# snap-research/MMVID

Hardware: AMD Instinct MI355X
Metric: video-tokens/sec training step, 8-frame 128px text-to-video (higher is better)
Workload: dtype bf16

## Files before the change

include/mmvid_hip.h:

```cpp
#ifndef MMVID_HIP_H
#define MMVID_HIP_H
#include <stdint.h>
#ifdef __cplusplus
extern "C" {
#endif

const char* mmvid_last_error(void);
int mmvid_abi_version(void);
int mmvid_device_count(void);

int mmvid_vq_sqnorm(const float* codebook, int n, int dim, float* ee, void* stream);
int mmvid_vq_argmin_l2(const float* z, const float* codebook, const float* ee, int64_t rows, int n, int dim,
                       int64_t* idx, float* dmin, void* stream);
int mmvid_gather_rows(const float* table, int64_t table_rows, const int64_t* idx, int64_t rows, int dim,
                      float* out_f32, void* out_bf16, void* stream);

int mmvid_gemm_bf16(int a_kmajor, int b_kmajor, int M, int N, int K, const void* A, int64_t lda, const void* B,
                    int64_t ldb, int batch, int64_t strideA, int64_t strideB, int64_t strideC, int splitk,
                    float alpha, const float* bias, const float* residual, int64_t ldr, const void* dact_pre,
                    void* save_pre, int64_t ldp, int act, int accumulate, float* out_f32, void* out_bf16,
                    int64_t ldc, float* out_colsum,
                    void* stream);

int mmvid_decode_trace(void* dev_buf);
int mmvid_decode_persistent_trace(void* dev_buf);

int mmvid_gemm_bf16_dw(int64_t M, int N, int K, const void* dY, int64_t ldy, const void* X, int64_t ldx, int splitk,
                       float* workspace, float* dW, int accumulate, void* stream);
int mmvid_gemm_dw_pick_splitk(int64_t M, int N, int K);
typedef struct {
    int N, K;
    const void* dY;
    int64_t ldy, strideY;
    const void* X;
    int64_t ldx, strideX;
    float* const* dW_list;
} mmvid_dw_kind_t;
int mmvid_gemm_bf16_dw_multi(int64_t M, int nkinds, const mmvid_dw_kind_t* kinds, int groups, int accumulate, void* stream);
int mmvid_gemm_bf16_dw_grouped(int64_t M, int N, int K, const void* dY, int64_t ldy, int64_t strideY, const void* X, int64_t ldx,
                               int64_t strideX, int groups, float* const* dW_list, int accumulate, void* stream);
double mmvid_gemm_dw_multi_fill(int nkinds, const mmvid_dw_kind_t* kinds, int groups);

int mmvid_layernorm_fwd(const float* x, int64_t ldx, int64_t rows, int E, const float* w, const float* b, float eps,
                        void* y_bf16, float* y_f32, int64_t ldy, float* mean, float* rstd, void* stream);
int mmvid_layernorm_bwd(const float* dy, int64_t lddy, const float* x, int64_t ldx, const float* mean,
                        const float* rstd, const float* w, int64_t rows, int E, float* dx, int64_t lddx,
                        int add_into_dx, void* dx_bf16, float* dw, float* db, float* dx_colsum, void* stream);
int mmvid_layernorm_bwd_ws(const float* dy, int64_t lddy, const float* x, int64_t ldx, const float* mean,
                           const float* rstd, const float* w, int64_t rows, int E, float* dx, int64_t lddx,
                           int add_into_dx, void* dx_bf16, float* dw, float* db, float* dx_colsum, float* workspace,
                           int64_t workspace_floats, void* stream);
int mmvid_layernorm_bwd_ex(const void* dy, int dy_is_bf16, int64_t lddy, const float* x, int64_t ldx, const float* mean,
                           const float* rstd, const float* w, int64_t rows, int E, float* dx, int64_t lddx, int add_into_dx,
                           void* dx_bf16, float* dw, float* db, float* dx_colsum, float* workspace, int64_t workspace_floats,
                           void* stream);
typedef struct {
    const float* partial;
    float *dw, *db, *dx_colsum;
} mmvid_ln_reduce_t;
int mmvid_layernorm_bwd_partial(const void* dy, int dy_is_bf16, int64_t lddy, const float* x, int64_t ldx, const float* mean,
                                const float* rstd, const float* w, int64_t rows, int E, float* dx, int64_t lddx, int add_into_dx,
                                void* dx_bf16, int want_dw, int want_db, int want_colsum, float* workspace,
                                int64_t workspace_floats, int* blocks_out, void* stream);
int mmvid_layernorm_bwd_reduce_multi(int n, const mmvid_ln_reduce_t* items, int blocks, int E, void* stream);
int mmvid_groupnorm_swish_nhwc(const void* x, int x_is_bf16, int N, int64_t hw, int C, const float* w,
                               const float* b, float eps, int swish, float* stats_scratch, int partial_blocks,
                               void* y_bf16, float* y_f32, void* stream);

int mmvid_attention_fwd(const void* qkv, int64_t ld, int B, int L, int H, int E, float scale, int mask_mode, int r0,
                        int c0, int r1, int c1, void* out, int64_t ldo, float* lse2, void* stream);
int mmvid_attention_bwd(const void* qkv, int64_t ld, const void* O, int64_t ldo, const void* dO, int64_t lddo,
                        const float* lse2, float* delta, int B, int L, int H, int E, float scale, int mask_mode,
                        int r0, int c0, int r1, int c1, void* dqkv, int64_t ldg, void* stream);
int mmvid_attention_bwd_bias(const void* qkv, int64_t ld, const void* O, int64_t ldo, const void* dO, int64_t lddo,
                             const float* lse2, float* delta, int B, int L, int H, int E, float scale, int mask_mode, int r0,
                             int c0, int r1, int c1, void* dqkv, int64_t ldg, float* dbias, void* stream);
int mmvid_assemble_sequence(const float* const* tables, const int64_t* table_rows, int ntables, const int64_t* ids,
                            const int32_t* seg, const float* pos, int64_t B, int L, int E, float* out, void* stream);
int mmvid_assemble_sequence_bwd(float* const* grad_tables, const int64_t* table_rows, int ntables,
                                const int64_t* ids, const int32_t* seg, const float* dx, int64_t B, int L, int E,
                                float* dpos, int accumulate_dpos, void* stream);
int mmvid_cross_entropy_fwd(const float* logits, int64_t ldl, const int64_t* target, const uint8_t* select,
                            int64_t rows, int V, float* lse, float* loss_sum, void* stream);
int mmvid_cross_entropy_bwd(const float* logits, int64_t ldl, const int64_t* target, const uint8_t* select,
                            const float* lse, const float* gscale, int64_t rows, int V, void* dlogits_bf16,
                            int64_t ldd, void* stream);
int mmvid_colsum_bf16(const void* dy, int64_t ld, int64_t M, int N, float* db, void* stream);
typedef struct {
    const float* w[3];
    float* gw[3];
    int32_t dst0, rows, naxes, src0;
    int32_t d[3];
    int32_t pad;
} mmvid_pos_segment_t;
int mmvid_pos_table_fwd(const mmvid_pos_segment_t* segs, int nseg, int L, int E, float* out, void* stream);
int mmvid_pos_table_bwd(const mmvid_pos_segment_t* segs, int nseg, int E, const float* g, void* stream);
int mmvid_lincomb3(const float* a, const float* b, const float* c, float wa, float wb, float wc, float* out, void* stream);
int mmvid_scale3(const float* g, float wa, float wb, float wc, float* ga, float* gb, float* gc, void* stream);
int mmvid_rows_pack(const float* W, int64_t V, int E, const int64_t* ids, int n, int64_t* uid, float* rows, void* stream);
int mmvid_rows_merge(float* W, int64_t V, int E, const int64_t* ids, const float* rows, int n, void* stream);

int mmvid_device_faults(int64_t* counts, int reset);

int mmvid_grad_sqnorm(const float* g, int64_t n, float* out_accum, void* stream);
int mmvid_adam_step(float* p, const float* g, float* m, float* v, void* shadow_bf16, int64_t n, float lr,
                    float beta1, float beta2, float eps, float weight_decay, int step, const float* step_dev,
                    float max_norm, const float* sqnorm, float grad_scale, void* stream);
int mmvid_grad_sqnorm_det(const float* g, int64_t n, float* partials, float* out_accum, void* stream);
int mmvid_adam_step_lr(float* p, const float* g, float* m, float* v, void* shadow_bf16, int64_t n, float lr,
                       const float* lr_dev, float beta1, float beta2, float eps, float weight_decay, int step,
                       const float* step_dev, float max_norm, const float* sqnorm, float grad_scale, void* stream);
int mmvid_grad_sqnorm_rows(const float* g, int64_t n, float* partials, float* out_accum, const uint8_t* row_flags,
                           int64_t table_lo, int64_t table_rows, int rowlen, void* stream);
int mmvid_adam_step_rows(float* p, const float* g, float* m, float* v, void* shadow_bf16, int64_t n, float lr,
                         const float* lr_dev, float beta1, float beta2, float eps, float weight_decay, int step,
                         const float* step_dev, float max_norm, const float* sqnorm, float grad_scale,
                         const uint8_t* row_flags, int64_t table_lo, int64_t table_rows, int rowlen, void* stream);
int mmvid_lr_schedule(const float* step_dev, int kind, float lr_min, float lr_max, int warmup_steps, int every,
                      float* lr_out, void* stream);
int mmvid_counter_add(float* counter, float value, void* stream);
int mmvid_cast_f32_to_bf16(const float* x, void* y, int64_t n, void* stream);

int mmvid_msm_masks(uint64_t seed, const float* step_dev, int B, int T, int f, const float* strategy_prob, float bern_lo,
                    float bern_hi, float pc_prob, uint8_t* mask1, float* not_fully_masked, int32_t* strategy_out,
                    void* stream);
int mmvid_msm_masks_inject(const int32_t* decisions, const uint8_t* bernoulli, int B, int T, int f, uint8_t* mask1,
                           float* not_fully_masked, void* stream);
int mmvid_warp_params_bytes(void);
int mmvid_vid_warp(uint64_t seed, const float* step_dev, const float* x, int B, int T, int C, int H, int W,
                   const float* strategy_prob, void* params_scratch, int draw_params, float* out, void* stream);
int mmvid_vid_warp_new_frames(uint64_t seed, const float* step_dev, const float* x, int B, int T, int C, int H, int W,
                              const float* strategy_prob, void* params_scratch, int draw_params, float* new_frames,
                              void* stream);
int mmvid_vid_warp_tokens(const int64_t* target_tok, const int64_t* new_frame_tok, const void* params, int B, int T, int n,
                          int64_t* out, void* stream);
int mmvid_frames_u8_to_f32(const uint8_t* frames_u8, int N, int H, int W, float* out, void* stream);
int mmvid_frames_to_u8(const float* img, int64_t N, int H, int W, uint8_t* out, void* stream);
int mmvid_frames_paste_u8(const float* img, const uint8_t* real, const uint8_t* given, int64_t N, int H, int W, int h, int w,
                          uint8_t* out, void* stream);
int mmvid_vid_warp_new_frames_u8(uint64_t seed, const float* step_dev, const uint8_t* x_u8, int B, int T, int H, int W,
                                 const float* strategy_prob, void* params_scratch, int draw_params, float* new_frames,
                                 void* stream);
int mmvid_vid_warp_draw(uint64_t seed, const float* step_dev, int B, int T, const float* strategy_prob, void* params_scratch,
                        void* stream);
int mmvid_token_rows_gather(const uint16_t* table, int64_t table_rows, const int64_t* frame_index, int64_t rows, int n,
                            int64_t* out, void* stream);
int mmvid_erase_tokens_choice(uint64_t seed, const float* step_dev, int nchoice, const float* cumprob, const int32_t* modes,
                              const int32_t* boxes, int frame0_full, int B, int Tv, int f, int64_t value, int64_t* tok,
                              void* stream);
int mmvid_random_erase_tokens(uint64_t seed, const float* step_dev, int B, int Tv, int f, float p, float scale_lo,
                              float scale_hi, float ratio_lo, float ratio_hi, int erase_half, int64_t value, int64_t* tok,
                              void* stream);

int mmvid_visual_color_jitter(uint64_t seed, const float* step_dev, float* x, int B, int Tv, int C, int H, int W, float p,
                              int first_frame, float* params_out, void* stream);

typedef struct {
    const float *ln1_w, *ln1_b, *ln2_w, *ln2_b;
    const void* in_w;
    const float* in_b;
    const void* out_w;
    const float* out_b;
    const void* fc_w;
    const float* fc_b;
    const void* pj_w;
    const float* pj_b;
    float *g_ln1_w, *g_ln1_b, *g_ln2_w, *g_ln2_b, *g_in_w, *g_in_b, *g_out_w, *g_out_b, *g_fc_w, *g_fc_b, *g_pj_w,
        *g_pj_b;
} mmvid_tower_layer_t;

typedef struct {
    int B, L, E, H, F, layers;
    int mask_mode, r0, c0, r1, c1;
    float ln_eps;
} mmvid_tower_cfg_t;

int mmvid_tower_workspace(const mmvid_tower_cfg_t* cfg, int64_t* saved_bytes, int64_t* scratch_bytes);
int mmvid_tower_forward(const mmvid_tower_cfg_t* cfg, const mmvid_tower_layer_t* layers, const float* x_in,
                        float* x_out, void* saved, void* scratch, void* stream);
int mmvid_tower_backward(const mmvid_tower_cfg_t* cfg, const mmvid_tower_layer_t* layers, float* g,
                         void* saved, void* scratch, void* stream);


int mmvid_tower_prefill(const mmvid_tower_cfg_t* cfg, const mmvid_tower_layer_t* layers, const float* x_in,
                        float* x_out, void* kv_cache, int Lmax, void* scratch, void* stream);
int mmvid_tower_decode(const mmvid_tower_cfg_t* cfg, const mmvid_tower_layer_t* layers, const float* x_in, float* x_out,
                       void* kv_cache, int Lmax, const int32_t* pos_dev, int pos, void* scratch, void* stream);
int mmvid_tower_decode_fused(const mmvid_tower_cfg_t* cfg, const mmvid_tower_layer_t* layers, const float* x_in,
                             float* x_out, void* kv_cache, int Lmax, const int32_t* pos_dev, int pos, void* scratch,
                             void* stream);
int mmvid_tower_decode_fused_slice(const mmvid_tower_cfg_t* cfg, const mmvid_tower_layer_t* layers, const float* x_in,
                                   float* x_out, void* kv_cache, int Lmax, int cache_batch, int32_t* pos_dev, int pos,
                                   int advance_pos, void* scratch, void* stream);
int mmvid_tower_decode_persistent_supported(const mmvid_tower_cfg_t* cfg, int Lmax);
int64_t mmvid_tower_decode_persistent_workspace_bytes(int B);
int mmvid_tower_decode_persistent(const mmvid_tower_cfg_t* cfg, const mmvid_tower_layer_t* layers, const float* x_in, float* x_out,
                                  void* kv_cache, int Lmax, int32_t* pos_dev, int pos, int advance_pos, void* workspace, void* stream);
typedef struct {
    int64_t* tok;
    const float* table;
    int64_t table_rows;
    const float* pos_rows;
    int32_t pos_off;
    int32_t record_pos0;
    int64_t* record;
    int64_t record_ld;
    const float *lnf_w, *lnf_b;
    const void* head_w;
    const float* head_b;
    const float* E;
    int64_t e_step_stride;
    int64_t tok_offset;
    float* logits_out;
    int32_t V, e_pos0;
    float lnf_eps, temperature;
} mmvid_decode_token_t;
int mmvid_artv_token_step_persistent(const mmvid_tower_cfg_t* cfg, const mmvid_tower_layer_t* layers, const mmvid_decode_token_t* t,
                                     float* x_out, void* kv_cache, int Lmax, int32_t* pos_dev, void* workspace, void* stream);
int mmvid_gemv_rows(const float* x, int64_t ldx, int NB, int K, const float* ln_w, const float* ln_b, float eps, const void* W,
                    const float* bias, int N, int act, const float* residual, int64_t ldr, int round_in, int round_out,
                    float* out, int64_t ldo, void* stream);
int mmvid_decode_embed(const int64_t* tok, const float* table, int64_t table_rows, const float* pos_rows,
                       const int32_t* pos_dev, int pos_off, int B, int E, float* x, void* stream);
int mmvid_decode_embed_record(const int64_t* tok, const float* table, int64_t table_rows, const float* pos_rows,
                              const int32_t* pos_dev, int pos_off, int B, int E, float* x, int64_t* record, int64_t record_ld,
                              int record_pos0, void* stream);
int mmvid_kv_store(const void* qkv, int64_t ldq, int B, int L, int E, const int32_t* pos_dev, int pos0, int Lmax,
                   void* cache, void* stream);
int mmvid_attention_decode(const void* qkv, int64_t ldq, const void* cache, int B, int Lmax, int H, int E,
                           const int32_t* pos_dev, int pos0, float scale, void* out, int64_t ldo, void* stream);

int mmvid_conv2d_nhwc(int mode, const void* x, int N, int Hin, int Win, int Cin, const void* w, const float* bias,
                      int Cout, const void* residual_bf16, const float* residual_f32, int clamp01, void* out_bf16,
                      float* out_f32, float* gn_partial, void* stream);
int mmvid_conv2d_nhwc_splitk(int mode, const void* x, int N, int Hin, int Win, int Cin, const void* w, const float* bias,
                             int Cout, const void* residual_bf16, const float* residual_f32, int clamp01, void* out_bf16,
                             float* out_f32, float* gn_partial, int splitk, float* workspace, void* stream);
int mmvid_conv3x3_strip_supported(int H, int W, int Cin, int Cout);
int mmvid_conv3x3_strip_nhwc(const void* x, int N, int H, int W, int Cin, const void* w, const float* bias, int Cout,
                             const void* residual_bf16, const float* residual_f32, void* out_bf16, float* out_f32,
                             float* gn_partial64, void* stream);
int mmvid_image_to_nhwc8(const float* img, int N, int H, int W, void* out_bf16, void* stream);
int mmvid_nhwc_to_nchw_f32(const float* x, int N, int H, int W, int C, int Cuse, float* out, void* stream);
int mmvid_spatial_attention(const void* q, const void* k, const void* v, int N, int HW, int C, float scale,
                            float* scores_scratch, void* out_bf16, void* stream);
int mmvid_spatial_attention_ld(const void* q, const void* k, const void* v, int64_t ld, int N, int HW, int C, float scale,
                               float* scores_scratch, void* out_bf16, void* stream);

int mmvid_sample_race(const float* logits, int64_t ld, const float* E, const float* noise_u, float temperature,
                      float logit_div, int64_t R, int V, int64_t tok_offset, int64_t* tok, float* y, void* stream);
int mmvid_sample_race_at(const float* logits, int64_t ld, const float* E, const int32_t* step_dev, int step0, int64_t e_step_stride,
                         const float* noise_u, float temperature, float logit_div, int64_t R, int V, int64_t tok_offset, int64_t* tok,
                         float* y, void* stream);
int mmvid_mp_select_keep(const float* Y, const float* E, const uint8_t* preserve, int b, int Bm, int TS, int k,
                         uint8_t* mask1, void* stream);
int mmvid_mp_select_keep_rows(const float* Y, const float* E, const uint8_t* given, const int32_t* k_rows, int b, int Bm, int TS,
                              uint8_t* mask1, void* stream);
int mmvid_mp_build_input(const float* control_emb, const float* image_emb, int64_t table_rows, const float* tpos,
                         const int64_t* I_tok, const uint8_t* mask1, int b, int Bm, int csl, int TS, int E, int64_t mask_id,
                         float* out, void* stream);
int mmvid_mp_update(const uint8_t* mask1, const float* Ynew, const int64_t* Inew, const float* rel_logit,
                    const float* vid_logit, int b, int Bm, int TS, int t, int dynamic, float* Y, int64_t* I_tok,
                    int64_t* Imax, float* Smax, int32_t* tmax, uint8_t* active, float* S_out, int32_t* jmax_out,
                    void* stream);
int mmvid_head_bce_fwd(const float* x, int64_t ldx, const int64_t* rows, int R, int E, const float* ln_w, const float* ln_b,
                       float eps, const float* w, const float* b, const float* label, const float* row_weight,
                       const float* den_from, int nden, float den_const, float* z, float* mean, float* rstd, float* loss,
                       void* stream);
int mmvid_head_bce_bwd(const float* x, int64_t ldx, const int64_t* rows, int R, int E, const float* ln_w, const float* ln_b,
                       const float* w, const float* z, const float* mean, const float* rstd, const float* label,
                       const float* row_weight, const float* den_from, int nden, float den_const, const float* gloss,
                       float* dx, int64_t lddx, float* dw, float* db, float* dln_w, float* dln_b, void* stream);
int mmvid_bert_build_ids(const int64_t* text, const int64_t* text_neg, const int64_t* visual_tok, const int64_t* target,
                         const int64_t* target_warp, const uint8_t* mask1, int B, int Ttxt, int Nvis, int TS,
                         int64_t pad_base, int64_t mask_id, int has_rel, int has_vid, int64_t* ids, uint8_t* select_full,
                         int64_t* target_full, float* select_count, void* stream);

int mmvid_gemm_f32(int b_kmajor, int M, int N, int K, const float* A, int64_t lda, const float* B, int64_t ldb,
                   int batch, int64_t strideA, int64_t strideB, int64_t strideC, float alpha, const float* bias,
                   const float* residual, float* C, int64_t ldc, void* stream);
int mmvid_conv2d_nhwc_f32(int mode, const float* x, int N, int Hin, int Win, int Cin, const float* w,
                          const float* bias, int Cout, const float* residual, int clamp01, float* out, void* stream);
int mmvid_image_to_nhwc4_f32(const float* img, int N, int H, int W, float* out, void* stream);
int mmvid_groupnorm_swish_nhwc_f32(const float* x, int N, int64_t hw, int C, const float* w, const float* b, float eps,
                                   int swish, float* stats_scratch, float* y, void* stream);
int mmvid_spatial_attention_f32(const float* q, const float* k, const float* v, int N, int HW, int C, float scale,
                                float* scratch, float* out, void* stream);

int mmvid_conv2d_nhwc_split3(int mode, const void* x_planes, int N, int Hin, int Win, int Cin, const void* w3, const float* bias,
                             int Cout, const float* residual_f32, int clamp01, float* out_f32, float* gn_partial, int splitk,
                             float* workspace, void* stream);
int mmvid_conv3x3_strip_nhwc_split3(const void* x_planes, int N, int H, int W, int Cin, const void* w3, const float* bias,
                                    int Cout, const float* residual_f32, float* out_f32, float* gn_partial64, void* out_planes,
                                    void* stream);
int mmvid_split_f32_bf16x2(const float* x, int64_t n, void* planes_bf16, void* stream);
int mmvid_image_to_nhwc8_split(const float* img, int N, int H, int W, void* planes_bf16, void* stream);
int mmvid_groupnorm_swish_nhwc_split(const float* x, int N, int64_t hw, int C, const float* w, const float* b, float eps,
                                     int swish, float* stats_scratch, int partial_blocks, void* planes_bf16, void* stream);
int mmvid_conv3x3_strip_nhwc_f16(const void* x_f16, int N, int H, int W, int Cin, const void* w_f16, const float* bias, int Cout,
                                 const float* residual_f32, float* out_f32, float* gn_partial64, void* out_planes, void* stream);
int mmvid_groupnorm_swish_nhwc_f16out(const float* x, int N, int64_t hw, int C, const float* w, const float* b, float eps,
                                      int swish, float* stats_scratch, int partial_blocks, void* y_f16, void* stream);

enum {
    MMVID_VQOP_IMG2NHWC8 = 0,
    MMVID_VQOP_CONV = 1,
    MMVID_VQOP_GROUPNORM = 2,
    MMVID_VQOP_CAST = 3,
    MMVID_VQOP_SPATIAL_ATTN = 4,
    MMVID_VQOP_VQ_ARGMIN = 5,
    MMVID_VQOP_GATHER = 6,
    MMVID_VQOP_NHWC2NCHW = 7,
    MMVID_VQOP_EXT_CAST = 8
};
#define MMVID_VQFLAG_STRICT 16
#define MMVID_VQFLAG_SPLIT 64
#define MMVID_VQFLAG_F16 128
typedef struct {
    int32_t op, mode;
    int32_t N, H, W, C;
    int32_t Cout, flags;
    int64_t in0, in1, in2;
    int64_t out_bf16, out_f32, scratch;
    const void* w;
    const float* b;
    const void* ext_in;
    void* ext_out;
    float eps;
    int32_t pad;
} mmvid_vqgan_op_t;
int mmvid_vqgan_run(const mmvid_vqgan_op_t* ops, int nops, void* arena, void* stream);

int mmvid_probe(int which, const void* in, void* out, void* stream);

// ... 86 lines not shown
```

mmvid_amd/_lib.py:

```python
import ctypes
import os
from ctypes import POINTER, Structure, c_char_p, c_float, c_int, c_int32, c_int64, c_uint8, c_uint64, c_void_p

HERE = os.path.dirname(os.path.abspath(__file__))
LIB_PATH = os.environ.get('MMVID_LIB') or os.path.join(HERE, 'libmmvid_hip.so')

P = c_void_p
I, I64, F, U64 = c_int, c_int64, c_float, c_uint64


class TowerLayer(Structure):
    _fields_ = [(n, P) for n in (
        'ln1_w', 'ln1_b', 'ln2_w', 'ln2_b', 'in_w', 'in_b', 'out_w', 'out_b', 'fc_w', 'fc_b', 'pj_w', 'pj_b',
        'g_ln1_w', 'g_ln1_b', 'g_ln2_w', 'g_ln2_b', 'g_in_w', 'g_in_b', 'g_out_w', 'g_out_b', 'g_fc_w', 'g_fc_b',
        'g_pj_w', 'g_pj_b')]


class TowerCfg(Structure):
    _fields_ = [('B', I), ('L', I), ('E', I), ('H', I), ('F', I), ('layers', I), ('mask_mode', I), ('r0', I),
                ('c0', I), ('r1', I), ('c1', I), ('ln_eps', F)]


class DecodeToken(Structure):
    _fields_ = [('tok', c_void_p), ('table', c_void_p), ('table_rows', c_int64), ('pos_rows', c_void_p), ('pos_off', c_int32),
                ('record_pos0', c_int32), ('record', c_void_p), ('record_ld', c_int64), ('lnf_w', c_void_p), ('lnf_b', c_void_p),
                ('head_w', c_void_p), ('head_b', c_void_p), ('E', c_void_p), ('e_step_stride', c_int64), ('tok_offset', c_int64),
                ('logits_out', c_void_p), ('V', c_int32), ('e_pos0', c_int32), ('lnf_eps', c_float), ('temperature', c_float)]


class PostLnLayer(Structure):
    _fields_ = [(n, P) for n in ('qkv_w', 'qkv_b', 'out_w', 'out_b', 'ln1_w', 'ln1_b', 'fc_w', 'fc_b', 'pj_w', 'pj_b', 'ln2_w', 'ln2_b')]


class PostLnCfg(Structure):
    _fields_ = [('B', I), ('L', I), ('E', I), ('H', I), ('F', I), ('layers', I), ('ln_eps', F)]


class Conv3dCfg(Structure):
    _fields_ = [(n, I) for n in ('N', 'T', 'H', 'W', 'Cin', 'Cout', 'kt', 'kh', 'kw', 'st', 'sh', 'sw', 'pt0', 'pt1', 'ph0', 'ph1',
                                 'pw0', 'pw1', 'relu', 'nseg')] + [('seg_end', I * 3), ('ldo', I * 3), ('c_off', I * 3), ('out', P * 3)]


class VqganOp(Structure):
    _fields_ = [('op', c_int32), ('mode', c_int32), ('N', c_int32), ('H', c_int32), ('W', c_int32), ('C', c_int32),
                ('Cout', c_int32), ('flags', c_int32), ('in0', I64), ('in1', I64), ('in2', I64), ('out_bf16', I64),
                ('out_f32', I64), ('scratch', I64), ('w', P), ('b', P), ('ext_in', P), ('ext_out', P), ('eps', F),
                ('pad', c_int32)]


SIGNATURES = {
    'mmvid_vq_sqnorm': [P, I, I, P, P],
    'mmvid_vq_argmin_l2': [P, P, P, I64, I, I, P, P, P],
    'mmvid_gather_rows': [P, I64, P, I64, I, P, P, P],
    'mmvid_gemm_bf16': [I, I, I, I, I, P, I64, P, I64, I, I64, I64, I64, I, F, P, P, I64, P, P, I64, I, I, P, P, I64, P, P],
    'mmvid_gemm_bf16_dw': [I64, I, I, P, I64, P, I64, I, P, P, I, P],
    'mmvid_gemm_dw_pick_splitk': [I64, I, I],
    'mmvid_gemm_bf16_dw_grouped': [I64, I, I, P, I64, I64, P, I64, I64, I, P, I, P],
    'mmvid_gemm_bf16_dw_multi': [I64, I, P, I, I, P],
    'mmvid_layernorm_fwd': [P, I64, I64, I, P, P, F, P, P, I64, P, P, P],
    'mmvid_layernorm_bwd': [P, I64, P, I64, P, P, P, I64, I, P, I64, I, P, P, P, P, P],
    'mmvid_layernorm_bwd_ws': [P, I64, P, I64, P, P, P, I64, I, P, I64, I, P, P, P, P, P, I64, P],
    'mmvid_layernorm_bwd_partial': [P, I, I64, P, I64, P, P, P, I64, I, P, I64, I, P, I, I, I, P, I64, P, P],
    'mmvid_layernorm_bwd_reduce_multi': [I, P, I, I, P],
    'mmvid_layernorm_bwd_ex': [P, I, I64, P, I64, P, P, P, I64, I, P, I64, I, P, P, P, P, P, I64, P],
    'mmvid_groupnorm_swish_nhwc': [P, I, I, I64, I, P, P, F, I, P, I, P, P, P],
    'mmvid_attention_fwd': [P, I64, I, I, I, I, F, I, I, I, I, I, P, I64, P, P],
    'mmvid_attention_bwd': [P, I64, P, I64, P, I64, P, P, I, I, I, I, F, I, I, I, I, I, P, I64, P],
    'mmvid_attention_bwd_bias': [P, I64, P, I64, P, I64, P, P, I, I, I, I, F, I, I, I, I, I, P, I64, P, P],
    'mmvid_assemble_sequence': [POINTER(P), POINTER(I64), I, P, P, P, I64, I, I, P, P],
    'mmvid_assemble_sequence_bwd': [POINTER(P), POINTER(I64), I, P, P, P, I64, I, I, P, I, P],
    'mmvid_cross_entropy_fwd': [P, I64, P, P, I64, I, P, P, P],
    'mmvid_cross_entropy_bwd': [P, I64, P, P, P, P, I64, I, P, I64, P],
    'mmvid_colsum_bf16': [P, I64, I64, I, P, P],
    'mmvid_grad_sqnorm': [P, I64, P, P],
    'mmvid_adam_step': [P, P, P, P, P, I64, F, F, F, F, F, I, P, F, P, F, P],
    'mmvid_cast_f32_to_bf16': [P, P, I64, P],
    'mmvid_tower_workspace': [POINTER(TowerCfg), POINTER(I64), POINTER(I64)],
    'mmvid_tower_forward': [POINTER(TowerCfg), POINTER(TowerLayer), P, P, P, P, P],
    'mmvid_tower_backward': [POINTER(TowerCfg), POINTER(TowerLayer), P, P, P, P],
    'mmvid_tower_prefill': [POINTER(TowerCfg), POINTER(TowerLayer), P, P, P, I, P, P],
    'mmvid_tower_decode': [POINTER(TowerCfg), POINTER(TowerLayer), P, P, P, I, P, I, P, P],
    'mmvid_tower_decode_fused': [POINTER(TowerCfg), POINTER(TowerLayer), P, P, P, I, P, I, P, P],
    'mmvid_tower_decode_persistent': [POINTER(TowerCfg), POINTER(TowerLayer), P, P, P, I, P, I, I, P, P],
    'mmvid_artv_token_step_persistent': [POINTER(TowerCfg), POINTER(TowerLayer), POINTER(DecodeToken), P, P, I, P, P, P],
    'mmvid_tower_decode_fused_slice': [POINTER(TowerCfg), POINTER(TowerLayer), P, P, P, I, I, P, I, I, P, P],
    'mmvid_gemv_rows': [P, I64, I, I, P, P, F, P, P, I, I, P, I64, I, I, P, I64, P],
    'mmvid_decode_embed': [P, P, I64, P, P, I, I, I, P, P],
    'mmvid_decode_embed_record': [P, P, I64, P, P, I, I, I, P, P, I64, I, P],
    'mmvid_kv_store': [P, I64, I, I, I, P, I, I, P, P],
    'mmvid_attention_decode': [P, I64, P, I, I, I, I, P, I, F, P, I64, P],
    'mmvid_conv2d_nhwc': [I, P, I, I, I, I, P, P, I, P, P, I, P, P, P, P],
    'mmvid_conv2d_nhwc_splitk': [I, P, I, I, I, I, P, P, I, P, P, I, P, P, P, I, P, P],
    'mmvid_conv3x3_strip_supported': [I, I, I, I],
    'mmvid_conv3x3_strip_nhwc': [P, I, I, I, I, P, P, I, P, P, P, P, P, P],
    'mmvid_image_to_nhwc8': [P, I, I, I, P, P],
    'mmvid_nhwc_to_nchw_f32': [P, I, I, I, I, I, P, P],
    'mmvid_spatial_attention': [P, P, P, I, I, I, F, P, P, P],
    'mmvid_spatial_attention_ld': [P, P, P, I64, I, I, I, F, P, P, P],
    'mmvid_conv2d_nhwc_split3': [I, P, I, I, I, I, P, P, I, P, I, P, P, I, P, P],
    'mmvid_conv3x3_strip_nhwc_split3': [P, I, I, I, I, P, P, I, P, P, P, P, P],
    'mmvid_conv3x3_strip_nhwc_f16': [P, I, I, I, I, P, P, I, P, P, P, P, P],
    'mmvid_split_f32_bf16x2': [P, I64, P, P],
    'mmvid_image_to_nhwc8_split': [P, I, I, I, P, P],
    'mmvid_groupnorm_swish_nhwc_split': [P, I, I64, I, P, P, F, I, P, I, P, P],
    'mmvid_groupnorm_swish_nhwc_f16out': [P, I, I64, I, P, P, F, I, P, I, P, P],
    'mmvid_decode_trace': [P],
    'mmvid_decode_persistent_trace': [P],
    'mmvid_vqgan_run': [POINTER(VqganOp), I, P, P],
    'mmvid_sample_race': [P, I64, P, P, F, F, I64, I, I64, P, P, P],
    'mmvid_sample_race_at': [P, I64, P, P, I, I64, P, F, F, I64, I, I64, P, P, P],
    'mmvid_mp_select_keep': [P, P, P, I, I, I, I, P, P],
    'mmvid_mp_build_input': [P, P, I64, P, P, P, I, I, I, I, I, I64, P, P],
    'mmvid_mp_update': [P, P, P, P, P, I, I, I, I, I, P, P, P, P, P, P, P, P, P],
    'mmvid_head_bce_fwd': [P, I64, P, I, I, P, P, F, P, P, P, P, P, I, F, P, P, P, P, P],
    'mmvid_head_bce_bwd': [P, I64, P, I, I, P, P, P, P, P, P, P, P, P, I, F, P, P, I64, P, P, P, P, P],
    'mmvid_bert_build_ids': [P, P, P, P, P, P, I, I, I, I, I64, I64, I, I, P, P, P, P, P],
    'mmvid_grad_sqnorm_det': [P, I64, P, P, P],
    'mmvid_adam_step_lr': [P, P, P, P, P, I64, F, P, F, F, F, F, I, P, F, P, F, P],
    'mmvid_lr_schedule': [P, I, F, F, I, I, P, P],
    'mmvid_grad_sqnorm_rows': [P, I64, P, P, P, I64, I64, I, P],
    'mmvid_adam_step_rows': [P, P, P, P, P, I64, F, P, F, F, F, F, I, P, F, P, F, P, I64, I64, I, P],
    'mmvid_counter_add': [P, F, P],
    'mmvid_msm_masks': [U64, P, I, I, I, P, F, F, F, P, P, P, P],
    'mmvid_msm_masks_inject': [P, P, I, I, I, P, P, P],
    'mmvid_vid_warp': [U64, P, P, I, I, I, I, I, P, P, I, P, P],
    'mmvid_vid_warp_new_frames': [U64, P, P, I, I, I, I, I, P, P, I, P, P],
    'mmvid_vid_warp_tokens': [P, P, P, I, I, I, P, P],
    'mmvid_frames_u8_to_f32': [P, I, I, I, P, P],
    'mmvid_vid_warp_new_frames_u8': [U64, P, P, I, I, I, I, P, P, I, P, P],
    'mmvid_vid_warp_draw': [U64, P, I, I, P, P, P],
    'mmvid_token_rows_gather': [P, I64, P, I64, I, P, P],
    'mmvid_erase_tokens_choice': [U64, P, I, P, P, P, I, I, I, I, I64, P, P],
    'mmvid_random_erase_tokens': [U64, P, I, I, I, F, F, F, F, F, I, I64, P, P],
    'mmvid_visual_color_jitter': [U64, P, P, I, I, I, I, I, F, I, P, P],
    'mmvid_gemm_f32': [I, I, I, I, P, I64, P, I64, I, I64, I64, I64, F, P, P, P, I64, P],
    'mmvid_conv2d_nhwc_f32': [I, P, I, I, I, I, P, P, I, P, I, P, P],
    'mmvid_image_to_nhwc4_f32': [P, I, I, I, P, P],
    'mmvid_groupnorm_swish_nhwc_f32': [P, I, I64, I, P, P, F, I, P, P, P],
    'mmvid_spatial_attention_f32': [P, P, P, I, I, I, F, P, P, P],
    'mmvid_probe': [I, P, P, P],
    'mmvid_prof_begin': [I],
    'mmvid_prof_enable': [I],
    'mmvid_graph_stats': [P],
    'mmvid_set_option': [c_char_p, I],
    'mmvid_get_option': [c_char_p, POINTER(I)],
    'mmvid_colsum_bf16_det': [P, I64, I64, I, P, P, I64, P],
    'mmvid_cross_entropy_fwd_det': [P, I64, P, P, I64, I, P, P, P, I64, P],
    'mmvid_assemble_sequence_bwd_det': [POINTER(P), POINTER(I64), I, P, P, P, I64, I, I, P, I, P, I64, P],
    'mmvid_gemm_bf16_det': [I, I, I, I, I, P, I64, P, I64, I, I64, I64, I64, I, F, P, P, I64, P, P, I64, I, I, P, P, I64, P, P, I64, P],
    'mmvid_attention_bwd_bias_det': [P, I64, P, I64, P, I64, P, P, I, I, I, I, F, I, I, I, I, I, P, I64, P, P, I64, P],
    'mmvid_device_faults': [P, I],
    'mmvid_pos_table_fwd': [P, I, I, I, P, P],
    'mmvid_pos_table_bwd': [P, I, I, P, P],
    'mmvid_lincomb3': [P, P, P, F, F, F, P, P],
    'mmvid_scale3': [P, F, F, F, P, P, P, P],
    'mmvid_prof_end': [P, P, P, P, I],
    'mmvid_rows_pack': [P, I64, I, P, I, P, P, P],
    'mmvid_rows_merge': [P, I64, I, P, P, I, P],
    'mmvid_clip_patchify': [P, I, I, I, I, I, P, P],
    'mmvid_clip_image_assemble': [P, P, P, P, P, F, I, I, I, P, P],
    'mmvid_clip_text_embed': [P, I, I, P, I64, P, I, P, P, P],
    'mmvid_clip_pool_project': [P, I, I, I, P, P, P, F, P, I, I, P, P],
    'mmvid_clip_pair_scores': [P, P, I, I, I, P, P],
    'mmvid_roberta_embed': [P, P, I, I, P, I64, P, I64, P, P, P, F, I, I64, P, P, P, P],
    'mmvid_attention_fwd_keylen': [P, I64, I, I, I, I, F, P, P, I64, P, P],
    'mmvid_postln_encoder_workspace': [POINTER(PostLnCfg), POINTER(I64)],
    'mmvid_postln_encoder_forward': [POINTER(PostLnCfg), POINTER(PostLnLayer), P, P, P, P, P, P],
    'mmvid_masked_mean_pool': [P, P, I, I, I, P, P],
    'mmvid_conv3d_ndhwc': [POINTER(Conv3dCfg), P, P, P, P],
    'mmvid_maxpool3d_ndhwc': [P, I, I, I, I, I, I, I, I, I, I, I, I, I, I, I, I, I, P, I, I, P],
    'mmvid_i3d_preprocess': [P, I, I, I, I, I, P, P],
    'mmvid_i3d_fold': [P, I, I, P, P],
    'mmvid_i3d_head': [P, I, I, I, P, P, I, P, P],
    'mmvid_frames_to_u8': [P, I64, I, I, P, P],
    'mmvid_mp_select_keep_rows': [P, P, P, P, I, I, I, P, P],
    'mmvid_frames_paste_u8': [P, P, P, I64, I, I, I, I, P, P],
}
OTHER = {'mmvid_last_error': ([], c_char_p), 'mmvid_abi_version': ([], I), 'mmvid_device_count': ([], I),
         'mmvid_warp_params_bytes': ([], I), 'mmvid_gemm_dw_multi_fill': ([I, P, I], ctypes.c_double),
         'mmvid_tower_decode_persistent_supported': ([POINTER(TowerCfg), I], I),
         'mmvid_tower_decode_persistent_workspace_bytes': ([I], I64),
         'mmvid_colsum_bf16_det_workspace_bytes': ([I64, I], I64), 'mmvid_cross_entropy_fwd_det_workspace_bytes': ([I64], I64),
         'mmvid_assemble_sequence_bwd_det_workspace_bytes': ([I64, I, I, I, POINTER(I64)], I64),
         'mmvid_gemm_bf16_det_workspace_bytes': ([I, I, I, I], I64),
         'mmvid_attention_bwd_bias_det_workspace_bytes': ([I, I, I], I64)}

class DwKind(ctypes.Structure):
    _fields_ = [('N', ctypes.c_int32), ('K', ctypes.c_int32), ('dY', ctypes.c_void_p), ('ldy', ctypes.c_int64), ('strideY', ctypes.c_int64),
                ('X', ctypes.c_void_p), ('ldx', ctypes.c_int64), ('strideX', ctypes.c_int64), ('dW_list', ctypes.c_void_p)]


class LnReduce(ctypes.Structure):
    _fields_ = [('partial', ctypes.c_void_p), ('dw', ctypes.c_void_p), ('db', ctypes.c_void_p), ('dx_colsum', ctypes.c_void_p)]


class PosSegment(ctypes.Structure):
    _fields_ = [('w', ctypes.c_void_p * 3), ('gw', ctypes.c_void_p * 3), ('dst0', ctypes.c_int32), ('rows', ctypes.c_int32),
                ('naxes', ctypes.c_int32), ('src0', ctypes.c_int32), ('d', ctypes.c_int32 * 3), ('pad', ctypes.c_int32)]


ABI_VERSION = 3
_lib = None


class MMVIDError(RuntimeError):
    pass


def load():
    global _lib
    if _lib is None:
        import torch
        if not os.path.exists(LIB_PATH):
            raise MMVIDError(f'{LIB_PATH} is missing: run `python -m mmvid_amd.build` (hipcc, gfx950). '
                             'There is no CPU/PyTorch fallback for the kernels.')
        lib = ctypes.CDLL(LIB_PATH)
        ver = getattr(lib, 'mmvid_abi_version', None)
        have = ver() if ver is not None else None
        if have != ABI_VERSION:
            raise MMVIDError(f'{LIB_PATH} has ABI version {have}, this package needs {ABI_VERSION}: '
                             'rebuild with `python -m mmvid_amd.build --force`')
        missing = []

        def bind(name, args, res):
            fn = getattr(lib, name, None)
            if fn is None:
                missing.append(name)
            else:
                fn.argtypes, fn.restype = args, res

        for name, args in SIGNATURES.items():
            bind(name, args, I)
        for name, (args, res) in OTHER.items():
            bind(name, args, res)
        if missing and not os.environ.get('MMVID_LIB'):
            raise MMVIDError(f'{LIB_PATH} lacks {missing[:4]}: rebuild with `python -m mmvid_amd.build --force`')
        lib._mmvid_missing = frozenset(missing)
        _lib = lib
    return _lib


def call(name, *args):
    lib = load()
    if name in lib._mmvid_missing:
        raise MMVIDError(f'{name} is not in {LIB_PATH} (an older build loaded through MMVID_LIB)')
    rc = getattr(lib, name)(*args)
    if rc != 0:
        raise MMVIDError(f'{name} failed (rc={rc}): {lib.mmvid_last_error().decode()}')


def is_deterministic():
    if 'mmvid_get_option' in load()._mmvid_missing:
        return False
    v = c_int(0)
    call('mmvid_get_option', b'deterministic', ctypes.byref(v))
    return v.value != 0


def set_deterministic(flag):
    prev = is_deterministic()
    call('mmvid_set_option', b'deterministic', int(bool(flag)))
    return prev


class deterministic:

    def __init__(self, flag=True):
        self.flag = bool(flag)

    def __enter__(self):
        self.prev = set_deterministic(self.flag)
        return self

    def __exit__(self, *exc):
        set_deterministic(self.prev)
        return False


FAULT_NAMES = ('embedding id outside its table', 'cross-entropy target outside [0, V)', 'token-table row outside its table', 'reserved')


def device_faults(reset=True):
    arr = (ctypes.c_int64 * 4)()
    call('mmvid_device_faults', arr, int(reset))
    return list(arr)


def check_device_faults():
    counts = device_faults(reset=True)
    bad = [f'{n} x {FAULT_NAMES[i]}' for i, n in enumerate(counts) if n]
    if bad:
        raise MMVIDError('kernels met out-of-range indices: ' + '; '.join(bad))
```

mmvid_amd/clip_tower.py:

```python
import ctypes
import os
import math

import torch
from torch import nn

from . import _lib, ops
from .functional import _note_params, _with_param_zeros

TOWER_SHAPES = {
    'openai_clip_visual': (768, 12, 12),
    'openai_clip_text': (512, 12, 8),
}
MATRIX_KEYS = ('attn.in_proj_weight', 'attn.out_proj.weight', 'mlp.c_fc.weight', 'mlp.c_proj.weight')


class _Holder(nn.Module):
    """Parameter container (no forward): gives parameters their reference names."""


def _linear_params(out_f, in_f, std):
    h = _Holder()
    h.weight = nn.Parameter(torch.randn(out_f, in_f) * std)
    h.bias = nn.Parameter(torch.zeros(out_f))
    return h


def _ln_params(e):
    h = _Holder()
    h.weight = nn.Parameter(torch.ones(e))
    h.bias = nn.Parameter(torch.zeros(e))
    return h


class ResidualAttentionBlockParams(_Holder):
    def __init__(self, width, layers):
        super().__init__()
        proj_std = (width**-0.5) * ((2 * layers)**-0.5)
        attn_std = width**-0.5
        fc_std = (2 * width)**-0.5
        self.attn = _Holder()
        self.attn.in_proj_weight = nn.Parameter(torch.randn(3 * width, width) * attn_std)
        self.attn.in_proj_bias = nn.Parameter(torch.zeros(3 * width))
        self.attn.out_proj = _linear_params(width, width, proj_std)
        self.ln_1 = _ln_params(width)
        self.mlp = _Holder()
        self.mlp.c_fc = _linear_params(4 * width, width, fc_std)
        self.mlp.c_proj = _linear_params(width, 4 * width, proj_std)
        self.ln_2 = _ln_params(width)


class _TowerParams(_Holder):
    def __init__(self, width, layers):
        super().__init__()
        self.resblocks = nn.ModuleList([ResidualAttentionBlockParams(width, layers) for _ in range(layers)])


class _TowerFn(torch.autograd.Function):
    @staticmethod
    def forward(ctx, x, tower, keep, *params):
        _note_params(ctx, (x, tower, keep) + params)
        ctx.tower = tower
        y, saved = tower._run_forward(x, keep=keep)
        ctx.saved_arena = saved
        ctx.shape = x.shape
        return y

    @staticmethod
    def backward(ctx, gy):
        g = gy.contiguous().clone()
        ctx.tower._run_backward(g, ctx.saved_arena, ctx.shape)
        ctx.saved_arena = None
        return _with_param_zeros(ctx, (g.view(ctx.shape), None, None) + (None, ) * (len(ctx.needs_input_grad) - 3))


class DecodeSession:

    def __init__(self, tower, kv_cache, first_pos, graph, fused=True):
        self.tower, self.cache, self.fused = tower, kv_cache, fused
        B, dev = kv_cache.shape[1], kv_cache.device
        self.cfg = tower._cfg(B, kv_cache.shape[2])
        self.layers, self._keep = tower._layer_structs(False)
        _, self.scratch = tower._workspace(self.cfg, dev, False)
        self.x = torch.zeros(B, tower.width, device=dev, dtype=torch.float32)
        self.y = torch.zeros_like(self.x)
        self.pos = torch.tensor([first_pos], dtype=torch.int32, device=dev)
        self.host_pos = int(first_pos)
        self.graph, self.want_graph, self.calls = None, graph, 0
        self._slice_cfgs = {}
        lib = _lib.load()
        self.persistent = bool(fused is True and os.environ.get('MMVID_DECODE_PERSISTENT', '1') != '0'
                               and lib.mmvid_tower_decode_persistent_supported(ctypes.byref(self.cfg), kv_cache.shape[2]))
        self.ws = torch.zeros(lib.mmvid_tower_decode_persistent_workspace_bytes(B) // 8, dtype=torch.int64, device=dev) if self.persistent else None

    def _enqueue(self):
        B, E = self.x.shape[0], self.x.shape[-1]
        if self.persistent:
            _lib.call('mmvid_tower_decode_persistent', ctypes.byref(self.cfg), self.layers, ops._p(self.x), ops._p(self.y),
                      ops._p(self.cache), self.cache.shape[2], ops._p(self.pos), 0, 1, ops._p(self.ws), ops._stream())
            return
        Lmax = self.cache.shape[2]
        if self.fused and E <= 768:
            per = 64 if E in (512, 768) else 16
            for b0 in range(0, B, per):
                nb = min(per, B - b0)
                cfg = self.cfg if nb == B else self._slice_cfgs.setdefault(nb, self.tower._cfg(nb, Lmax))
                _lib.call('mmvid_tower_decode_fused_slice', ctypes.byref(cfg), self.layers, self.x[b0:].data_ptr(), self.y[b0:].data_ptr(),
                          self.cache[0, b0].data_ptr(), Lmax, B, ops._p(self.pos), 0, int(b0 + per >= B), ops._p(self.scratch), ops._stream())
            return
        _lib.call('mmvid_tower_decode', ctypes.byref(self.cfg), self.layers, ops._p(self.x), ops._p(self.y),
                  ops._p(self.cache), Lmax, ops._p(self.pos), 0, ops._p(self.scratch), ops._stream())
        self.pos.add_(1)

    def token_step(self, tk):
        assert self.persistent
        _lib.call('mmvid_artv_token_step_persistent', ctypes.byref(self.cfg), self.layers, ctypes.byref(tk), ops._p(self.y), ops._p(self.cache),
                  self.cache.shape[2], ops._p(self.pos), ops._p(self.ws), ops._stream())
        self.host_pos += 1

    def failed(self):
        return bool(self.persistent and int(self.ws[1]) != 0)

    def fall_back(self, pos):
        self.persistent, self.graph = False, None
        self.fell_back = getattr(self, 'fell_back', 0) + 1
        self.pos.fill_(int(pos))
        self.host_pos = int(pos)

    def check(self):
        if self.failed():
            raise _lib.MMVIDError('persistent decode step: a poll timed out (the device was shared while it ran); results are invalid. '
                                  'Set MMVID_DECODE_PERSISTENT=0 to use the five-launch step.')

    @torch.no_grad()
    def step(self, x_new, verify=False):
        self.x.copy_(x_new)
        self.calls += 1
        if self.want_graph and self.graph is None and self.calls == 2:
            g = torch.cuda.CUDAGraph()
            side = torch.cuda.Stream()
            side.wait_stream(torch.cuda.current_stream())
            with torch.cuda.stream(side):
                with torch.cuda.graph(g, stream=side):
                    self._enqueue()
            torch.cuda.current_stream().wait_stream(side)
            self.graph = g
        if self.graph is not None:
            self.graph.replay()
        else:
            self._enqueue()
        if verify and self.persistent and self.failed():
            self.fall_back(self.host_pos)
            self._enqueue()
        self.host_pos += 1
        return self.y


class OpenAICLIPTransformer(nn.Module):
    def __init__(self, seq_len=0, which_model='openai_clip_text', model_path=None, causal=True, mask_type='causal',
                 mask_kwargs=None, layers=None, width=None, heads=None):
        super().__init__()
        if not which_model.startswith('openai_clip'):
            raise NotImplementedError(which_model)
        w, l, h = TOWER_SHAPES[which_model]
        self.width, self.layers, self.heads = width or w, layers or l, heads or h
        self.debug_keep_saved = False
        assert self.width == 64 * self.heads, 'head_dim must be 64 (CLIP towers)'
        self.context_length = seq_len
        self.causal = causal
        self.transformer = _TowerParams(self.width, self.layers)
        self.mask_spec = self.build_attention_mask(seq_len, mask_type, **(mask_kwargs or {})) if causal else None
        if model_path is not None:
            self.load_clip_checkpoint(model_path, which_model)
        self._shadow = None
        self._shadow_key = None
        self._scratch = None
        self._scratch_retired = []
        self.backward_chunk_layers = int(os.environ.get('MMVID_BWD_CHUNK', 0))
        self.on_layers_done = None

    @staticmethod
    def build_attention_mask(context_length, mask_type='causal', **kwargs):
        if mask_type == 'causal':
            return 'causal'
        if mask_type == 'mask_prev':
            idx = list(kwargs['index'])
            assert len(idx) <= 2, 'the kernels carry at most two restricted rows (BERT uses [ST1],[VID])'
            return ('rows', [(int(i), int(i)) for i in idx])
        raise NotImplementedError(mask_type)

    def dense_attention_mask(self, L=None):
        L = L or self.context_length
        if self.mask_spec is None:
            return None
        if self.mask_spec == 'causal':
            return torch.full((L, L), float('-inf')).triu_(1)
        m = torch.zeros(L, L)
        for r, c in self.mask_spec[1]:
            m[r, :c] = float('-inf')
        return m

    def load_clip_checkpoint(self, path, which_model):
        sd = torch.jit.load(path, map_location='cpu').state_dict()
        prefix = 'transformer.' if which_model == 'openai_clip_text' else 'visual.transformer.'
        own = {k[len(prefix):]: v.float() for k, v in sd.items() if k.startswith(prefix + 'resblocks.')}
        self.transformer.load_state_dict(own)

    def forward(self, x, **kwargs):
        assert x.dim() == 3 and x.shape[-1] == self.width
        keep = torch.is_grad_enabled() and (x.requires_grad or self._any_trainable())
        return _TowerFn.apply(x, self, keep, *self.parameters())

    def new_kv_cache(self, B, max_len, device):
        assert self.mask_spec == 'causal', 'incremental decoding needs the causal mask'
        return torch.empty(self.layers, B, max_len, 2 * self.width, device=device, dtype=torch.bfloat16)

    @torch.no_grad()
    def prefill(self, x, kv_cache):
        x = ops._chk(x.contiguous(), torch.float32, 'tower input')
        B, L, _ = x.shape
        cfg = self._cfg(B, L)
        layers, _keep = self._layer_structs(False)
        _, scratch = self._workspace(cfg, x.device, False)
        y = torch.empty_like(x)
        _lib.call('mmvid_tower_prefill', ctypes.byref(cfg), layers, ops._p(x), ops._p(y), ops._p(kv_cache),
                  kv_cache.shape[2], ops._p(scratch), ops._stream())
        return y

    @torch.no_grad()
    def decode_step(self, x_new, kv_cache, pos, pos_dev=None):
        x_new = ops._chk(x_new.contiguous(), torch.float32, 'tower input')
        B = x_new.shape[0]
        cfg = self._cfg(B, kv_cache.shape[2])
        layers, _keep = self._layer_structs(False)
        _, scratch = self._workspace(cfg, x_new.device, False)
        y = torch.empty_like(x_new)
        _lib.call('mmvid_tower_decode', ctypes.byref(cfg), layers, ops._p(x_new), ops._p(y), ops._p(kv_cache),
                  kv_cache.shape[2], ops._p(pos_dev), int(pos), ops._p(scratch), ops._stream())
        return y

    def decode_session(self, kv_cache, first_pos, graph=True, fused=True):
        return DecodeSession(self, kv_cache, first_pos, graph, fused)

    def _any_trainable(self):
        return any(p.requires_grad for p in self.parameters())

    def _matrix_params(self):
        for blk in self.transformer.resblocks:
            yield blk.attn.in_proj_weight
            yield blk.attn.out_proj.weight
            yield blk.mlp.c_fc.weight
            yield blk.mlp.c_proj.weight

    def attach_shadow(self, views):
        self._shadow = list(views)
        self.mark_shadow_fresh()

    def mark_shadow_fresh(self):
        self._shadow_key = tuple((p._version, p.data_ptr()) for p in self._matrix_params())

    def _sync_shadow(self):
        ps = list(self._matrix_params())
        key = tuple((p._version, p.data_ptr()) for p in ps)
        if self._shadow is None or self._shadow[0].device != ps[0].device:
            self._shadow = [torch.empty(p.shape, device=p.device, dtype=torch.bfloat16) for p in ps]
            self._shadow_key = None
        if key != self._shadow_key:
            for p, s in zip(ps, self._shadow):
                ops.cast_bf16(p.detach().contiguous(), s)
            self._shadow_key = key
        return self._shadow

    def _cfg(self, B, L):
        c = _lib.TowerCfg()
        c.B, c.L, c.E, c.H, c.F, c.layers = B, L, self.width, self.heads, 4 * self.width, self.layers
        c.mask_mode, c.r0, c.c0, c.r1, c.c1 = ops._mask_args(self.mask_spec)
        c.ln_eps = 1e-5
        return c

    def _layer_structs(self, with_grads):
        sh = self._sync_shadow()
        arr = (_lib.TowerLayer * self.layers)()
        keep = []

        def ptr(t):
            keep.append(t)
            return t.data_ptr()

        def gptr(p):
            if not with_grads or not p.requires_grad:
                return None
            if p.grad is None:
                p.grad = torch.zeros_like(p)
            return p.grad.data_ptr()

        for i, blk in enumerate(self.transformer.resblocks):
            a = arr[i]
            a.ln1_w, a.ln1_b = ptr(blk.ln_1.weight), ptr(blk.ln_1.bias)
            a.ln2_w, a.ln2_b = ptr(blk.ln_2.weight), ptr(blk.ln_2.bias)
            a.in_w, a.in_b = ptr(sh[4 * i]), ptr(blk.attn.in_proj_bias)
            a.out_w, a.out_b = ptr(sh[4 * i + 1]), ptr(blk.attn.out_proj.bias)
            a.fc_w, a.fc_b = ptr(sh[4 * i + 2]), ptr(blk.mlp.c_fc.bias)
            a.pj_w, a.pj_b = ptr(sh[4 * i + 3]), ptr(blk.mlp.c_proj.bias)
            a.g_ln1_w, a.g_ln1_b = gptr(blk.ln_1.weight), gptr(blk.ln_1.bias)
            a.g_ln2_w, a.g_ln2_b = gptr(blk.ln_2.weight), gptr(blk.ln_2.bias)
            a.g_in_w, a.g_in_b = gptr(blk.attn.in_proj_weight), gptr(blk.attn.in_proj_bias)
            a.g_out_w, a.g_out_b = gptr(blk.attn.out_proj.weight), gptr(blk.attn.out_proj.bias)
            a.g_fc_w, a.g_fc_b = gptr(blk.mlp.c_fc.weight), gptr(blk.mlp.c_fc.bias)
            a.g_pj_w, a.g_pj_b = gptr(blk.mlp.c_proj.weight), gptr(blk.mlp.c_proj.bias)
        return arr, keep

    def _workspace(self, cfg, device, keep):
        sb, cb = ctypes.c_int64(), ctypes.c_int64()
        _lib.call('mmvid_tower_workspace', ctypes.byref(cfg), ctypes.byref(sb), ctypes.byref(cb))
        if self._scratch is None or self._scratch.device != torch.device(device) or self._scratch.numel() < cb.value:
            if self._scratch is not None:
                self._scratch_retired.append(self._scratch)
            self._scratch = torch.empty(cb.value, device=device, dtype=torch.uint8)
        saved = torch.empty(sb.value, device=device, dtype=torch.uint8) if keep else None
        return saved, self._scratch

    def _run_forward(self, x, keep):
        x = ops._chk(x.contiguous(), torch.float32, 'tower input')
        B, L, _ = x.shape
        cfg = self._cfg(B, L)
        layers, _keep = self._layer_structs(False)
        saved, scratch = self._workspace(cfg, x.device, keep)
        y = torch.empty_like(x)
        _lib.call('mmvid_tower_forward', ctypes.byref(cfg), layers, ops._p(x), ops._p(y), ops._p(saved), ops._p(scratch),
                  ops._stream())
        if self.debug_keep_saved:
            self._last_saved = saved
        return y, saved

    def backward_chunks(self):
        if self.on_layers_done is None:
            return [(0, self.layers)]
        if self.backward_chunk_layers <= 0:
            return self._planned_chunks()
        step = self.backward_chunk_layers
        out, hi = [], self.layers
        while hi > 0:
            lo = max(0, hi - step)
            out.append((lo, hi))
            hi = lo
        return out

    def _planned_chunks(self):
        if getattr(self, '_chunk_plan', None) is None or self._chunk_plan[0] != self.layers:
            E = self.width
            F = 4 * E
            t = sum(-(-n // 256) * -(-k // 128) for n, k in ((3 * E, E), (E, E), (F, E), (E, F)))
            waste = lambda n: (-(-n * t // 256)) - n * t / 256.0
            best, plan = None, [(0, self.layers)]
            for a in range(3, self.layers - 2):
                w = waste(a) + waste(self.layers - a) + 0.02 * abs(a - 0.6 * self.layers)
                if best is None or w < best:
                    best, plan = w, [(self.layers - a, self.layers), (0, self.layers - a)]
            self._chunk_plan = (self.layers, plan)
        return self._chunk_plan[1]

    def _run_backward(self, g, saved, shape):
        if saved is None:
            raise _lib.MMVIDError('tower backward without saved activations (forward ran under no_grad)')
        B, L, _ = shape
        cfg = self._cfg(B, L)
        layers, _keep = self._layer_structs(True)
        _, scratch = self._workspace(cfg, g.device, False)
        sb = ctypes.c_int64()
        _lib.call('mmvid_tower_workspace', ctypes.byref(cfg), ctypes.byref(sb), None)
        if sb.value != saved.numel():
            raise _lib.MMVIDError(f'tower backward: the saved arena holds {saved.numel()} bytes, the current layout needs {sb.value} '
                                  '(the library changed between forward and backward)')
        per_layer = saved.numel() // self.layers
        for lo, hi in self.backward_chunks():
            sub = self._cfg(B, L)
            sub.layers = hi - lo
            lp = ctypes.cast(ctypes.byref(layers, lo * ctypes.sizeof(_lib.TowerLayer)), ctypes.POINTER(_lib.TowerLayer))
            _lib.call('mmvid_tower_backward', ctypes.byref(sub), lp, ops._p(g),
                      ctypes.c_void_p(saved.data_ptr() + lo * per_layer), ops._p(scratch), ops._stream())
            if self.on_layers_done is not None:
                self.on_layers_done(lo)
```

mmvid_amd/csrc/norm.hip:

```cpp
#include "../../include/mmvid_hip.h"
#include "common.h"
#include <type_traits>

namespace {

constexpr int LN_MAXV = 4;

__global__ __launch_bounds__(256) void layernorm_fwd_kernel(const float* __restrict__ x, long ldx, long rows, int E,
                                                            const float* __restrict__ w,
                                                            const float* __restrict__ b, float eps,
                                                            bf16_t* __restrict__ y_bf16, float* __restrict__ y_f32,
                                                            long ldy, float* __restrict__ mean_out,
                                                            float* __restrict__ rstd_out) {
    const long half = (rows + 1) >> 1;
    const long r0 = (long)blockIdx.x * 4 + (threadIdx.x >> 6);
    if (r0 >= half) return;
    const long rr[2] = {r0, r0 + half};
    const bool live1 = rr[1] < rows;
    const int lane = threadIdx.x & 63;
    const int nv = E >> 2;
    float4 v[2][LN_MAXV];
    float s[2] = {0.f, 0.f};
#pragma unroll
    for (int k = 0; k < 2; ++k) {
        const float4* xr = reinterpret_cast<const float4*>(x + (k == 0 || live1 ? rr[k] : rr[0]) * ldx);
#pragma unroll
        for (int i = 0; i < LN_MAXV; ++i) {
            const int c = lane + 64 * i;
            v[k][i] = c < nv ? xr[c] : make_float4(0, 0, 0, 0);
        }
    }
#pragma unroll
    for (int k = 0; k < 2; ++k)
#pragma unroll
        for (int i = 0; i < LN_MAXV; ++i) s[k] += (v[k][i].x + v[k][i].y) + (v[k][i].z + v[k][i].w);
    const float mean[2] = {wave_sum_fast(s[0]) / (float)E, wave_sum_fast(s[1]) / (float)E};
    float q[2] = {0.f, 0.f};
#pragma unroll
    for (int k = 0; k < 2; ++k)
#pragma unroll
        for (int i = 0; i < LN_MAXV; ++i) {
            const int c = lane + 64 * i;
            if (c < nv) {
                const float a = v[k][i].x - mean[k], b2 = v[k][i].y - mean[k], c2 = v[k][i].z - mean[k], d = v[k][i].w - mean[k];
                q[k] += (a * a + b2 * b2) + (c2 * c2 + d * d);
            }
        }
    const float rstd[2] = {rsqrtf(wave_sum_fast(q[0]) / (float)E + eps), rsqrtf(wave_sum_fast(q[1]) / (float)E + eps)};
#pragma unroll
    for (int k = 0; k < 2; ++k) {
        if (k == 1 && !live1) break;
        const long r = rr[k];
        if (lane == 0) {
            if (mean_out) mean_out[r] = mean[k];
            if (rstd_out) rstd_out[r] = rstd[k];
        }
#pragma unroll
        for (int i = 0; i < LN_MAXV; ++i) {
            const int c = lane + 64 * i;
            if (c < nv) {
                const float4 w4 = reinterpret_cast<const float4*>(w)[c];
                const float4 b4 = reinterpret_cast<const float4*>(b)[c];
                float4 o;
                o.x = (v[k][i].x - mean[k]) * rstd[k] * w4.x + b4.x;
                o.y = (v[k][i].y - mean[k]) * rstd[k] * w4.y + b4.y;
                o.z = (v[k][i].z - mean[k]) * rstd[k] * w4.z + b4.z;
                o.w = (v[k][i].w - mean[k]) * rstd[k] * w4.w + b4.w;
                if (y_f32) reinterpret_cast<float4*>(y_f32 + r * ldy)[c] = o;
                if (y_bf16) reinterpret_cast<uint2*>(y_bf16 + r * ldy)[c] = make_uint2(pack_bf2(o.x, o.y), pack_bf2(o.z, o.w));
            }
        }
    }
}

template <typename DY>
__global__ __launch_bounds__(256) void layernorm_bwd_kernel(const DY* __restrict__ dy, long lddy,
                                                            const float* __restrict__ x, long ldx,
                                                            const float* __restrict__ mean,
                                                            const float* __restrict__ rstd,
                                                            const float* __restrict__ w, long rows, int E,
                                                            float* __restrict__ dx, long lddx, int add,
                                                            bf16_t* __restrict__ dx_bf16,
                                                            float* __restrict__ dw, float* __restrict__ db,
                                                            float* __restrict__ dx_colsum, float* __restrict__ partial) {
    __shared__ float red[2][4][LN_MAXV * 64 * 4];
    const int lane = threadIdx.x & 63, wave = threadIdx.x >> 6;
    const int nv = E >> 2;
    float4 pw[LN_MAXV], pb[LN_MAXV], pc[LN_MAXV], w4[LN_MAXV];
#pragma unroll
    for (int i = 0; i < LN_MAXV; ++i) {
        pw[i] = pb[i] = pc[i] = make_float4(0, 0, 0, 0);
        const int c = lane + 64 * i;
        w4[i] = (c < nv) ? reinterpret_cast<const float4*>(w)[c] : make_float4(0, 0, 0, 0);
    }
    for (long r = (long)blockIdx.x * 4 + wave; r < rows; r += (long)gridDim.x * 4) {
        const float mu = mean[r], rs = rstd[r];
        float4 g[LN_MAXV], xh[LN_MAXV], prev[LN_MAXV];
        float s1 = 0.f, s2 = 0.f;
#pragma unroll
        for (int i = 0; i < LN_MAXV; ++i) {
            const int c = lane + 64 * i;
            if (c < nv) {
                prev[i] = add ? reinterpret_cast<const float4*>(dx + r * lddx)[c] : make_float4(0.f, 0.f, 0.f, 0.f);
                float4 d4;
                if constexpr (sizeof(DY) == 4) {
                    d4 = reinterpret_cast<const float4*>(dy + r * lddy)[c];
                } else {
                    const uint2 u = reinterpret_cast<const uint2*>(dy + r * lddy)[c];
                    d4 = make_float4(bf_lo(u.x), bf_hi(u.x), bf_lo(u.y), bf_hi(u.y));
                }
                const float4 x4 = reinterpret_cast<const float4*>(x + r * ldx)[c];
                xh[i] = make_float4((x4.x - mu) * rs, (x4.y - mu) * rs, (x4.z - mu) * rs, (x4.w - mu) * rs);
                g[i] = make_float4(d4.x * w4[i].x, d4.y * w4[i].y, d4.z * w4[i].z, d4.w * w4[i].w);
                s1 += (g[i].x + g[i].y) + (g[i].z + g[i].w);
                s2 += (g[i].x * xh[i].x + g[i].y * xh[i].y) + (g[i].z * xh[i].z + g[i].w * xh[i].w);
                pw[i].x += d4.x * xh[i].x, pw[i].y += d4.y * xh[i].y, pw[i].z += d4.z * xh[i].z, pw[i].w += d4.w * xh[i].w;
                pb[i].x += d4.x, pb[i].y += d4.y, pb[i].z += d4.z, pb[i].w += d4.w;
            }
        }
        const float m1 = wave_sum_fast(s1) / (float)E, m2 = wave_sum_fast(s2) / (float)E;
#pragma unroll
        for (int i = 0; i < LN_MAXV; ++i) {
            const int c = lane + 64 * i;
            if (c < nv) {
                float4 o;
                o.x = rs * (g[i].x - m1 - xh[i].x * m2);
                o.y = rs * (g[i].y - m1 - xh[i].y * m2);
                o.z = rs * (g[i].z - m1 - xh[i].z * m2);
                o.w = rs * (g[i].w - m1 - xh[i].w * m2);
                float4* d = reinterpret_cast<float4*>(dx + r * lddx) + c;
                o.x += prev[i].x, o.y += prev[i].y, o.z += prev[i].z, o.w += prev[i].w;
                *d = o;
                pc[i].x += o.x, pc[i].y += o.y, pc[i].z += o.z, pc[i].w += o.w;
                if (dx_bf16)
                    reinterpret_cast<uint2*>(dx_bf16 + r * lddx)[c] = make_uint2(pack_bf2(o.x, o.y), pack_bf2(o.z, o.w));
            }
        }
    }
    if (dw || db) {
#pragma unroll
        for (int i = 0; i < LN_MAXV; ++i) {
            const int c = lane + 64 * i;
            if (c < nv) {
                reinterpret_cast<float4*>(red[0][wave])[c] = pw[i];
                reinterpret_cast<float4*>(red[1][wave])[c] = pb[i];
            }
        }
        __syncthreads();
        for (int e = threadIdx.x; e < E; e += 256) {
            const float sw = (red[0][0][e] + red[0][1][e]) + (red[0][2][e] + red[0][3][e]);
            const float sb = (red[1][0][e] + red[1][1][e]) + (red[1][2][e] + red[1][3][e]);
            if (partial) {
                partial[((long)blockIdx.x * 3 + 0) * E + e] = sw;
                partial[((long)blockIdx.x * 3 + 1) * E + e] = sb;
            } else {
                if (dw) unsafeAtomicAdd(dw + e, sw);
                if (db) unsafeAtomicAdd(db + e, sb);
            }
        }
    }
    if (dx_colsum) {
        __syncthreads();
#pragma unroll
        for (int i = 0; i < LN_MAXV; ++i) {
            const int c = lane + 64 * i;
            if (c < nv) reinterpret_cast<float4*>(red[0][wave])[c] = pc[i];
        }
        __syncthreads();
        for (int e = threadIdx.x; e < E; e += 256) {
            const float sc = (red[0][0][e] + red[0][1][e]) + (red[0][2][e] + red[0][3][e]);
            if (partial)
                partial[((long)blockIdx.x * 3 + 2) * E + e] = sc;
            else
                unsafeAtomicAdd(dx_colsum + e, sc);
        }
    }
}

template <typename DY, int NVI>
__global__ __launch_bounds__(256) void layernorm_bwd_fast_kernel(const DY* __restrict__ dy, long lddy, const float* __restrict__ x,
                                                                 long ldx, const float* __restrict__ mean,
                                                                 const float* __restrict__ rstd, const float* __restrict__ w, long rows,
                                                                 float* __restrict__ dx, long lddx, int add,
                                                                 bf16_t* __restrict__ dx_bf16, float* __restrict__ dw,
                                                                 float* __restrict__ db, float* __restrict__ dx_colsum,
                                                                 float* __restrict__ partial) {
    constexpr int E = 256 * NVI;
    __shared__ float red[2][4][E];
    typedef typename std::conditional<sizeof(DY) == 4, float4, uint2>::type dy_raw_t;
    const int lane = threadIdx.x & 63, wave = __builtin_amdgcn_readfirstlane(threadIdx.x >> 6);
    float4 pw[NVI], pb[NVI], pc[NVI], w4[NVI];
#pragma unroll
    for (int i = 0; i < NVI; ++i) {
        pw[i] = pb[i] = pc[i] = make_float4(0, 0, 0, 0);
        w4[i] = reinterpret_cast<const float4*>(w)[lane + 64 * i];
    }
    struct RowIn {
        float4 prev[NVI], x4[NVI];
        dy_raw_t d[NVI];
        float mu, rs;
    };
    const long rstep = (long)gridDim.x * 4;
    auto load_row = [&](RowIn& in, long r) {
        in.mu = mean[r], in.rs = rstd[r];
#pragma unroll
        for (int i = 0; i < NVI; ++i) {
            const int c = lane + 64 * i;
            in.prev[i] = reinterpret_cast<const float4*>(dx + r * lddx)[c];
            in.d[i] = reinterpret_cast<const dy_raw_t*>(dy + r * lddy)[c];
            in.x4[i] = reinterpret_cast<const float4*>(x + r * ldx)[c];
        }
    };
    RowIn cur, nxt;
    long r = (long)blockIdx.x * 4 + wave;
    if (r < rows) load_row(nxt, r);
    for (; r < rows; r += rstep) {
        cur = nxt;
        load_row(nxt, r + rstep < rows ? r + rstep : r);
        const float mu = cur.mu, rs = cur.rs;
        float4 g[NVI], xh[NVI];
        float s1 = 0.f, s2 = 0.f;
#pragma unroll
        for (int i = 0; i < NVI; ++i) {
            float4 d4;
            if constexpr (sizeof(DY) == 4) {
                d4 = cur.d[i];
            } else {
                const uint2 u = cur.d[i];
                d4 = make_float4(bf_lo(u.x), bf_hi(u.x), bf_lo(u.y), bf_hi(u.y));
            }
            const float4 x4 = cur.x4[i];
            xh[i] = make_float4((x4.x - mu) * rs, (x4.y - mu) * rs, (x4.z - mu) * rs, (x4.w - mu) * rs);
            g[i] = make_float4(d4.x * w4[i].x, d4.y * w4[i].y, d4.z * w4[i].z, d4.w * w4[i].w);
            s1 += (g[i].x + g[i].y) + (g[i].z + g[i].w);
            s2 += (g[i].x * xh[i].x + g[i].y * xh[i].y) + (g[i].z * xh[i].z + g[i].w * xh[i].w);
            pw[i].x += d4.x * xh[i].x, pw[i].y += d4.y * xh[i].y, pw[i].z += d4.z * xh[i].z, pw[i].w += d4.w * xh[i].w;
            pb[i].x += d4.x, pb[i].y += d4.y, pb[i].z += d4.z, pb[i].w += d4.w;
        }
        const float m1 = wave_sum_fast(s1) / (float)E, m2 = wave_sum_fast(s2) / (float)E;
#pragma unroll
        for (int i = 0; i < NVI; ++i) {
            const int c = lane + 64 * i;
            float4 o;
            o.x = rs * (g[i].x - m1 - xh[i].x * m2);
            o.y = rs * (g[i].y - m1 - xh[i].y * m2);
            o.z = rs * (g[i].z - m1 - xh[i].z * m2);
            o.w = rs * (g[i].w - m1 - xh[i].w * m2);
            if (add) o.x += cur.prev[i].x, o.y += cur.prev[i].y, o.z += cur.prev[i].z, o.w += cur.prev[i].w;
            reinterpret_cast<float4*>(dx + r * lddx)[c] = o;
            pc[i].x += o.x, pc[i].y += o.y, pc[i].z += o.z, pc[i].w += o.w;
            if (dx_bf16) reinterpret_cast<uint2*>(dx_bf16 + r * lddx)[c] = make_uint2(pack_bf2(o.x, o.y), pack_bf2(o.z, o.w));
        }
    }
    if (dw || db) {
#pragma unroll
        for (int i = 0; i < NVI; ++i) {
            reinterpret_cast<float4*>(red[0][wave])[lane + 64 * i] = pw[i];
            reinterpret_cast<float4*>(red[1][wave])[lane + 64 * i] = pb[i];
        }
        __syncthreads();
        for (int e = threadIdx.x; e < E; e += 256) {
            const float sw = (red[0][0][e] + red[0][1][e]) + (red[0][2][e] + red[0][3][e]);
            const float sb = (red[1][0][e] + red[1][1][e]) + (red[1][2][e] + red[1][3][e]);
            if (partial) {
                partial[((long)blockIdx.x * 3 + 0) * E + e] = sw;
                partial[((long)blockIdx.x * 3 + 1) * E + e] = sb;
            } else {
                if (dw) unsafeAtomicAdd(dw + e, sw);
                if (db) unsafeAtomicAdd(db + e, sb);
            }
        }
    }
    if (dx_colsum) {
        __syncthreads();
#pragma unroll
        for (int i = 0; i < NVI; ++i) reinterpret_cast<float4*>(red[0][wave])[lane + 64 * i] = pc[i];
        __syncthreads();
        for (int e = threadIdx.x; e < E; e += 256) {
            const float sc = (red[0][0][e] + red[0][1][e]) + (red[0][2][e] + red[0][3][e]);
            if (partial)
                partial[((long)blockIdx.x * 3 + 2) * E + e] = sc;
            else
                unsafeAtomicAdd(dx_colsum + e, sc);
        }
    }
}

__global__ __launch_bounds__(1024) void layernorm_bwd_reduce_kernel(const float* __restrict__ partial, int nblocks, int E,
                                                                    float* __restrict__ dw, float* __restrict__ db,
                                                                    float* __restrict__ dx_colsum) {
    __shared__ float sh[32][33];
    const int which = blockIdx.y;
    float* out = which == 0 ? dw : (which == 1 ? db : dx_colsum);
    if (!out) return;
    const int lane = threadIdx.x & 31, rg = threadIdx.x >> 5;
    const int col = blockIdx.x * 32 + lane;
    float a = 0.f;
    if (col < E) {
        const float* src = partial + (long)which * E + col;
        int b = rg;
        for (; b + 15 * 32 < nblocks; b += 16 * 32) {
            float v[16];
#pragma unroll
            for (int i = 0; i < 16; ++i) v[i] = src[(long)(b + i * 32) * 3 * E];
#pragma unroll
            for (int i = 0; i < 16; ++i) a += v[i];
        }
        for (; b < nblocks; b += 32) a += src[(long)b * 3 * E];
    }
    sh[rg][lane] = a;
    __syncthreads();
    if (rg == 0 && col < E) {
        float t = 0.f;
#pragma unroll
        for (int i = 0; i < 32; ++i) t += sh[i][lane];
        out[col] += t;
    }
}

constexpr int LN_MULTI_MAX = 32;
struct LnReduceTable {
    mmvid_ln_reduce_t item[LN_MULTI_MAX];
};
__global__ __launch_bounds__(1024) void layernorm_bwd_reduce_multi_kernel(LnReduceTable t, int nblocks, int E) {
    __shared__ float sh[32][33];
    const int which = blockIdx.y;
    const float* partial = t.item[blockIdx.z].partial;
    float* out = which == 0 ? t.item[blockIdx.z].dw : (which == 1 ? t.item[blockIdx.z].db : t.item[blockIdx.z].dx_colsum);
    if (!out) return;
    const int lane = threadIdx.x & 31, rg = threadIdx.x >> 5;
    const int col = blockIdx.x * 32 + lane;
    float a = 0.f;
    if (col < E) {
        const float* src = partial + (long)which * E + col;
        int b = rg;
        for (; b + 15 * 32 < nblocks; b += 16 * 32) {
            float v[16];
#pragma unroll
            for (int i = 0; i < 16; ++i) v[i] = src[(long)(b + i * 32) * 3 * E];
#pragma unroll
            for (int i = 0; i < 16; ++i) a += v[i];
        }
        for (; b < nblocks; b += 32) a += src[(long)b * 3 * E];
    }
    sh[rg][lane] = a;
    __syncthreads();
    if (rg == 0 && col < E) {
        float s = 0.f;
#pragma unroll
        for (int i = 0; i < 32; ++i) s += sh[i][lane];
        out[col] += s;
    }
}

template <typename T>
__device__ __forceinline__ void load8(const T* p, float (&f)[8]);
template <>
__device__ __forceinline__ void load8<bf16_t>(const bf16_t* p, float (&f)[8]) {
    const uint4 u = *reinterpret_cast<const uint4*>(p);
    f[0] = bf_lo(u.x), f[1] = bf_hi(u.x), f[2] = bf_lo(u.y), f[3] = bf_hi(u.y);
    f[4] = bf_lo(u.z), f[5] = bf_hi(u.z), f[6] = bf_lo(u.w), f[7] = bf_hi(u.w);
// ... 139 lines not shown
        float a = 0.f;
        for (int r = 0; r < pstep; ++r) a += red[which][r * CB + ch];
        sh[which][ch] = a;
    }
    __syncthreads();
    const int cpg = C / 32;
    if (threadIdx.x < CB / cpg) {
        const int grp = threadIdx.x;
        float sm = 0.f, sq = 0.f;
        for (int e = 0; e < cpg; ++e) sm += sh[0][grp * cpg + e];
        for (int e = 0; e < cpg; ++e) sq += sh[1][grp * cpg + e];
        const float mu = sm / cnt;
        float var = sq / cnt - mu * mu;
        var = var < 0.f ? 0.f : var;
        const float rstd = rsqrtf(var + eps);
        for (int e = 0; e < cpg; ++e) {
            const int ch = grp * cpg + e;
            const float a = rstd * w[c0 + ch];
            ab[ch][0] = a, ab[ch][1] = b[c0 + ch] - mu * a;
        }
    }
    __syncthreads();
    float av[8], bv[8];
#pragma unroll
    for (int e = 0; e < 8; ++e) av[e] = ab[cc * 8 + e][0], bv[e] = ab[cc * 8 + e][1];
    for (long p = prow; p < hw; p += pstep) {
        float f[8], o[8];
        load8<T>(base + p * C, f);
#pragma unroll
        for (int e = 0; e < 8; ++e) {
            float v = f[e] * av[e] + bv[e];
            if (swish) v = v * __builtin_amdgcn_rcpf(1.0f + __builtin_amdgcn_exp2f(-1.4426950408889634f * v));
            o[e] = v;
        }
        const long at = ((long)n * hw + p) * C + c0 + cc * 8;
        if (y_bf16)
            *reinterpret_cast<uint4*>(y_bf16 + at) = make_uint4(pack_bf2(o[0], o[1]), pack_bf2(o[2], o[3]), pack_bf2(o[4], o[5]), pack_bf2(o[6], o[7]));
        if (y_f32) {
            float4* d = reinterpret_cast<float4*>(y_f32 + at);
            d[0] = make_float4(o[0], o[1], o[2], o[3]);
            d[1] = make_float4(o[4], o[5], o[6], o[7]);
        }
    }
}

__global__ __launch_bounds__(256) void groupnorm_finalize_f64_kernel(const float* __restrict__ partial, int nblk, int N, int C,
                                                                     double cnt, float eps, float* __restrict__ mr) {
    const int item = blockIdx.x * 4 + (threadIdx.x >> 6);
    if (item >= N * 32) return;
    const int lane = threadIdx.x & 63;
    const int n = item >> 5, grp = item & 31;
    double sm = 0.0, sq = 0.0;
    for (int k = lane; k < nblk; k += 64) {
        const float2 v = *reinterpret_cast<const float2*>(partial + (((long)n * nblk + k) * 32 + grp) * 2);
        sm += (double)v.x, sq += (double)v.y;
    }
    for (int o = 32; o > 0; o >>= 1) sm += __shfl_xor(sm, o, 64), sq += __shfl_xor(sq, o, 64);
    const double mu = sm / cnt;
    double var = sq / cnt - mu * mu;
    var = var < 0.0 ? 0.0 : var;
    const double rstd = 1.0 / sqrt(var + (double)eps);
    const int cpg = C >> 5;
    if (lane < cpg) *reinterpret_cast<float2*>(mr + ((long)n * C + grp * cpg + lane) * 2) = make_float2((float)mu, (float)rstd);
}

template <bool F16>
__global__ __launch_bounds__(256) void groupnorm_apply_split_kernel(const float* __restrict__ x, long hw, int C,
                                                                    const float* __restrict__ mr, const float* __restrict__ w,
                                                                    const float* __restrict__ b, int swish,
                                                                    bf16_t* __restrict__ planes, long total_chunks) {
    const long t = (long)blockIdx.x * 256 + threadIdx.x;
    if (t >= total_chunks) return;
    const int cchunks = C >> 3;
    const int cc = (int)(t % cchunks);
    const long pix = t / cchunks;
    const int n = (int)(pix / hw);
    float f[8], wv[8], bv[8];
    load8<float>(x + pix * C + cc * 8, f);
    load8<float>(w + cc * 8, wv);
    load8<float>(b + cc * 8, bv);
    const float4* q = reinterpret_cast<const float4*>(mr + ((long)n * C + cc * 8) * 2);
    const float4 q0 = q[0], q1 = q[1], q2 = q[2], q3 = q[3];
    const float mu[8] = {q0.x, q0.z, q1.x, q1.z, q2.x, q2.z, q3.x, q3.z};
    const float rs[8] = {q0.y, q0.w, q1.y, q1.w, q2.y, q2.w, q3.y, q3.w};
    uint32_t h[4], l[4];
    float o[8];
#pragma unroll
    for (int e = 0; e < 8; ++e) {
        float v = ((f[e] - mu[e]) * rs[e]) * wv[e] + bv[e];
        if (swish) v = v * (1.0f / (1.0f + expf(-v)));
        o[e] = v;
    }
    if constexpr (F16) {
#pragma unroll
        for (int e = 0; e < 4; ++e) {
            typedef __attribute__((ext_vector_type(2))) _Float16 h2_t;
            const h2_t p2 = {(_Float16)o[2 * e], (_Float16)o[2 * e + 1]};
            h[e] = __builtin_bit_cast(uint32_t, p2);
        }
        *reinterpret_cast<uint4*>(planes + t * 8) = make_uint4(h[0], h[1], h[2], h[3]);
        return;
    }
#pragma unroll
    for (int e = 0; e < 4; ++e) {
        h[e] = pack_bf2(o[2 * e], o[2 * e + 1]);
        l[e] = pack_bf2(o[2 * e] - bf_lo(h[e]), o[2 * e + 1] - bf_hi(h[e]));
    }
    *reinterpret_cast<uint4*>(planes + t * 8) = make_uint4(h[0], h[1], h[2], h[3]);
    *reinterpret_cast<uint4*>(planes + (total_chunks + t) * 8) = make_uint4(l[0], l[1], l[2], l[3]);
}

}

extern "C" int mmvid_layernorm_fwd(const float* x, int64_t ldx, int64_t rows, int E, const float* w, const float* b,
                                   float eps, void* y_bf16, float* y_f32, int64_t ldy, float* mean, float* rstd,
                                   void* stream) {
    MMVID_REQUIRE(x && w && b && (y_bf16 || y_f32), "layernorm_fwd: null pointer");
    MMVID_REQUIRE(E % 4 == 0 && E <= 64 * 4 * LN_MAXV && ldx % 4 == 0 && ldy % 4 == 0,
                  "layernorm_fwd: E=%d must be a multiple of 4 and <= %d; row strides multiples of 4", E,
                  64 * 4 * LN_MAXV);
    if (rows == 0) return MMVID_OK;
    hipLaunchKernelGGL(layernorm_fwd_kernel, dim3(cdiv((rows + 1) / 2, 4)), dim3(256), 0, (hipStream_t)stream, x, (long)ldx,
                       (long)rows, E, w, b, eps, (bf16_t*)y_bf16, y_f32, (long)ldy, mean, rstd);
    MMVID_LAUNCH_CHECK("layernorm_fwd");
    return MMVID_OK;
}

extern "C" int mmvid_layernorm_bwd_ws(const float* dy, int64_t lddy, const float* x, int64_t ldx, const float* mean,
                                      const float* rstd, const float* w, int64_t rows, int E, float* dx, int64_t lddx,
                                      int add_into_dx, void* dx_bf16, float* dw, float* db, float* dx_colsum,
                                      float* workspace, int64_t workspace_floats, void* stream);
extern "C" int mmvid_layernorm_bwd_ex(const void* dy, int dy_is_bf16, int64_t lddy, const float* x, int64_t ldx, const float* mean,
                                      const float* rstd, const float* w, int64_t rows, int E, float* dx, int64_t lddx,
                                      int add_into_dx, void* dx_bf16, float* dw, float* db, float* dx_colsum,
                                      float* workspace, int64_t workspace_floats, void* stream);

extern "C" int mmvid_layernorm_bwd(const float* dy, int64_t lddy, const float* x, int64_t ldx, const float* mean,
                                   const float* rstd, const float* w, int64_t rows, int E, float* dx, int64_t lddx,
                                   int add_into_dx, void* dx_bf16, float* dw, float* db, float* dx_colsum,
                                   void* stream) {
    return mmvid_layernorm_bwd_ws(dy, lddy, x, ldx, mean, rstd, w, rows, E, dx, lddx, add_into_dx, dx_bf16, dw, db, dx_colsum,
                                  nullptr, 0, stream);
}

extern "C" int mmvid_layernorm_bwd_ws(const float* dy, int64_t lddy, const float* x, int64_t ldx, const float* mean,
                                      const float* rstd, const float* w, int64_t rows, int E, float* dx, int64_t lddx,
                                      int add_into_dx, void* dx_bf16, float* dw, float* db, float* dx_colsum,
                                      float* workspace, int64_t workspace_floats, void* stream) {
    return mmvid_layernorm_bwd_ex(dy, 0, lddy, x, ldx, mean, rstd, w, rows, E, dx, lddx, add_into_dx, dx_bf16, dw, db, dx_colsum,
                                  workspace, workspace_floats, stream);
}

static int layernorm_bwd_impl(const void* dy, int dy_is_bf16, int64_t lddy, const float* x, int64_t ldx, const float* mean,
                              const float* rstd, const float* w, int64_t rows, int E, float* dx, int64_t lddx, int add_into_dx,
                              void* dx_bf16, float* dw, float* db, float* dx_colsum, float* workspace, int64_t workspace_floats,
                              int* blocks_out, void* stream) {
    MMVID_REQUIRE(dy && x && mean && rstd && w && dx, "layernorm_bwd: null pointer");
    MMVID_REQUIRE(E % 4 == 0 && E <= 64 * 4 * LN_MAXV && lddy % 4 == 0 && ldx % 4 == 0 && lddx % 4 == 0,
                  "layernorm_bwd: bad E/strides");
    if (rows == 0) return MMVID_OK;
    int blocks = cdiv(rows, 4);
    const bool any_red = dw || db || dx_colsum;
    float* partial = nullptr;
    if (workspace && any_red) {
        int cap = (int)(workspace_floats / (3 * (int64_t)E));
        if (cap > 2048) cap = 2048;
        if (cap >= 64) {
            if (blocks > cap) blocks = cap;
            partial = workspace;
        }
    }
    MMVID_REQUIRE(partial || !any_red || !mmvid_option(MMVID_OPT_DETERMINISTIC),
                  "layernorm_bwd: deterministic mode refuses the atomic dw / db / dx_colsum sums: pass a workspace of at least 64 * 3 * E "
                  "floats (mmvid_layernorm_bwd_ws / mmvid_layernorm_bwd_ex / mmvid_layernorm_bwd_partial)");
    if (!partial) {
        if (blocks > 512) blocks = 512;
    }
    float* const a_dw = partial ? (dw ? dw : workspace) : dw;
    float* const a_db = partial ? (db ? db : workspace) : db;
    float* const a_cs = partial ? (dx_colsum ? dx_colsum : nullptr) : dx_colsum;
    if (E == 768 || E == 512) {
#define MMVID_LN_FAST(DYT, NVI)                                                                                                            \
    hipLaunchKernelGGL((layernorm_bwd_fast_kernel<DYT, NVI>), dim3(blocks), dim3(256), 0, (hipStream_t)stream, (const DYT*)dy, (long)lddy, x, \
                       (long)ldx, mean, rstd, w, (long)rows, dx, (long)lddx, add_into_dx, (bf16_t*)dx_bf16, a_dw, a_db, a_cs, partial)
        if (dy_is_bf16) {
            if (E == 768) MMVID_LN_FAST(bf16_t, 3); else MMVID_LN_FAST(bf16_t, 2);
        } else {
            if (E == 768) MMVID_LN_FAST(float, 3); else MMVID_LN_FAST(float, 2);
        }
#undef MMVID_LN_FAST
    } else if (dy_is_bf16)
        hipLaunchKernelGGL(layernorm_bwd_kernel<bf16_t>, dim3(blocks), dim3(256), 0, (hipStream_t)stream, (const bf16_t*)dy, (long)lddy, x,
                           (long)ldx, mean, rstd, w, (long)rows, E, dx, (long)lddx, add_into_dx, (bf16_t*)dx_bf16,
                           partial ? (dw ? dw : workspace) : dw, partial ? (db ? db : workspace) : db,
                           partial ? (dx_colsum ? dx_colsum : nullptr) : dx_colsum, partial);
    else
        hipLaunchKernelGGL(layernorm_bwd_kernel<float>, dim3(blocks), dim3(256), 0, (hipStream_t)stream, (const float*)dy, (long)lddy, x,
                           (long)ldx, mean, rstd, w, (long)rows, E, dx, (long)lddx, add_into_dx, (bf16_t*)dx_bf16,
                           partial ? (dw ? dw : workspace) : dw, partial ? (db ? db : workspace) : db,
                           partial ? (dx_colsum ? dx_colsum : nullptr) : dx_colsum, partial);
    if (blocks_out) {
        MMVID_REQUIRE(partial || !any_red, "layernorm_bwd_partial: needs a workspace of at least 64 * 3 * E floats");
        *blocks_out = blocks;
    } else if (partial) {
        hipLaunchKernelGGL(layernorm_bwd_reduce_kernel, dim3(cdiv(E, 32), 3), dim3(1024), 0, (hipStream_t)stream, partial, blocks, E,
                           dw, db, dx_colsum);
    }
    MMVID_LAUNCH_CHECK("layernorm_bwd");
    return MMVID_OK;
}

extern "C" int mmvid_layernorm_bwd_ex(const void* dy, int dy_is_bf16, int64_t lddy, const float* x, int64_t ldx, const float* mean,
                                      const float* rstd, const float* w, int64_t rows, int E, float* dx, int64_t lddx,
                                      int add_into_dx, void* dx_bf16, float* dw, float* db, float* dx_colsum,
                                      float* workspace, int64_t workspace_floats, void* stream) {
    return layernorm_bwd_impl(dy, dy_is_bf16, lddy, x, ldx, mean, rstd, w, rows, E, dx, lddx, add_into_dx, dx_bf16, dw, db, dx_colsum,
                              workspace, workspace_floats, nullptr, stream);
}

extern "C" int mmvid_layernorm_bwd_partial(const void* dy, int dy_is_bf16, int64_t lddy, const float* x, int64_t ldx, const float* mean,
                                           const float* rstd, const float* w, int64_t rows, int E, float* dx, int64_t lddx,
                                           int add_into_dx, void* dx_bf16, int want_dw, int want_db, int want_colsum,
                                           float* workspace, int64_t workspace_floats, int* blocks_out, void* stream) {
    MMVID_REQUIRE(workspace && blocks_out, "layernorm_bwd_partial: null workspace / blocks_out");
    return layernorm_bwd_impl(dy, dy_is_bf16, lddy, x, ldx, mean, rstd, w, rows, E, dx, lddx, add_into_dx, dx_bf16,
                              want_dw ? workspace : nullptr, want_db ? workspace : nullptr, want_colsum ? workspace : nullptr, workspace,
                              workspace_floats, blocks_out, stream);
}

extern "C" int mmvid_layernorm_bwd_reduce_multi(int n, const mmvid_ln_reduce_t* items, int blocks, int E, void* stream) {
    MMVID_REQUIRE(n >= 0 && (n == 0 || items) && blocks > 0 && E > 0, "layernorm_bwd_reduce_multi: bad arguments");
    for (int i0 = 0; i0 < n; i0 += LN_MULTI_MAX) {
        const int m = n - i0 < LN_MULTI_MAX ? n - i0 : LN_MULTI_MAX;
        LnReduceTable t;
        for (int i = 0; i < LN_MULTI_MAX; ++i) {
            if (i < m) {
                MMVID_REQUIRE(items[i0 + i].partial, "layernorm_bwd_reduce_multi: entry %d has no partial rows", i0 + i);
                t.item[i] = items[i0 + i];
            } else {
                t.item[i].partial = nullptr, t.item[i].dw = t.item[i].db = t.item[i].dx_colsum = nullptr;
            }
        }
        hipLaunchKernelGGL(layernorm_bwd_reduce_multi_kernel, dim3(cdiv(E, 32), 3, m), dim3(1024), 0, (hipStream_t)stream, t, blocks, E);
    }
    MMVID_LAUNCH_CHECK("layernorm_bwd_reduce_multi");
    return MMVID_OK;
}

extern "C" int mmvid_groupnorm_swish_nhwc(const void* x, int x_is_bf16, int N, int64_t hw, int C, const float* w,
                                          const float* b, float eps, int swish, float* stats_scratch,
                                          int partial_blocks, void* y_bf16, float* y_f32, void* stream) {
    MMVID_REQUIRE(x && w && b && stats_scratch && (y_bf16 || y_f32), "groupnorm: null pointer");
    MMVID_REQUIRE(C % 32 == 0 && C <= 512 && 256 % (C / 8) == 0, "groupnorm: C=%d unsupported", C);
    MMVID_REQUIRE(partial_blocks >= 0 && partial_blocks <= cdiv(hw, 64), "groupnorm: partial_blocks %d", partial_blocks);
    if (N == 0 || hw == 0) return MMVID_OK;
    hipStream_t s = (hipStream_t)stream;
    const int pix_per_block = 256;
    int nblk = partial_blocks;
    float* ab = stats_scratch;
    float* partial = stats_scratch + (long)N * C * 2;
    const long chunks = (long)N * hw * (C / 8);
    if (partial_blocks == 0 && hw <= pix_per_block && (C & (C - 1)) == 0) {
        if (x_is_bf16)
            hipLaunchKernelGGL(groupnorm_small_fused_kernel<bf16_t>, dim3(N, C < 64 ? 1 : C / 64), dim3(256), 0, s, (const bf16_t*)x, (long)hw, C,
                               (float)hw * (float)(C / 32), eps, w, b, swish, (bf16_t*)y_bf16, y_f32);
        else
            hipLaunchKernelGGL(groupnorm_small_fused_kernel<float>, dim3(N, C < 64 ? 1 : C / 64), dim3(256), 0, s, (const float*)x, (long)hw, C,
                               (float)hw * (float)(C / 32), eps, w, b, swish, (bf16_t*)y_bf16, y_f32);
        MMVID_LAUNCH_CHECK("groupnorm");
        return MMVID_OK;
    }
    if (partial_blocks == 0) {
        nblk = cdiv(hw, pix_per_block);
        dim3 g1(nblk, N);
        if (x_is_bf16)
            hipLaunchKernelGGL(groupnorm_stats_kernel<bf16_t>, g1, dim3(256), 0, s, (const bf16_t*)x, (long)hw, C,
                               pix_per_block, partial);
        else
            hipLaunchKernelGGL(groupnorm_stats_kernel<float>, g1, dim3(256), 0, s, (const float*)x, (long)hw, C,
                               pix_per_block, partial);
    }
    hipLaunchKernelGGL(groupnorm_finalize_kernel, dim3(cdiv((long)N * 32, 4)), dim3(256), 0, s, partial, nblk, N, C,
                       (float)hw * (float)(C / 32), eps, w, b, ab);
    if (x_is_bf16)
        hipLaunchKernelGGL(groupnorm_apply_kernel<bf16_t>, dim3(cdiv(chunks, 256)), dim3(256), 0, s,
                           (const bf16_t*)x, (long)hw, C, ab, swish, (bf16_t*)y_bf16, y_f32, chunks);
    else
        hipLaunchKernelGGL(groupnorm_apply_kernel<float>, dim3(cdiv(chunks, 256)), dim3(256), 0, s, (const float*)x,
                           (long)hw, C, ab, swish, (bf16_t*)y_bf16, y_f32, chunks);
    MMVID_LAUNCH_CHECK("groupnorm");
    return MMVID_OK;
}

static int groupnorm_split_launch(const float* x, int N, int64_t hw, int C, const float* w, const float* b, float eps, int swish,
                                  float* stats_scratch, int partial_blocks, void* planes_bf16, void* stream, bool f16);

extern "C" int mmvid_groupnorm_swish_nhwc_split(const float* x, int N, int64_t hw, int C, const float* w, const float* b, float eps,
                                                int swish, float* stats_scratch, int partial_blocks, void* planes_bf16, void* stream) {
    return groupnorm_split_launch(x, N, hw, C, w, b, eps, swish, stats_scratch, partial_blocks, planes_bf16, stream, false);
}
extern "C" int mmvid_groupnorm_swish_nhwc_f16out(const float* x, int N, int64_t hw, int C, const float* w, const float* b, float eps,
                                                 int swish, float* stats_scratch, int partial_blocks, void* y_f16, void* stream) {
    return groupnorm_split_launch(x, N, hw, C, w, b, eps, swish, stats_scratch, partial_blocks, y_f16, stream, true);
}

static int groupnorm_split_launch(const float* x, int N, int64_t hw, int C, const float* w, const float* b, float eps, int swish,
                                  float* stats_scratch, int partial_blocks, void* planes_bf16, void* stream, bool f16) {
    MMVID_REQUIRE(x && w && b && stats_scratch && planes_bf16, "groupnorm_split: null pointer");
    MMVID_REQUIRE(C % 32 == 0 && C <= 512 && 256 % (C / 8) == 0, "groupnorm_split: C=%d unsupported", C);
    MMVID_REQUIRE(partial_blocks >= 0 && partial_blocks <= cdiv(hw, 64), "groupnorm_split: partial_blocks %d", partial_blocks);
    if (N == 0 || hw == 0) return MMVID_OK;
    hipStream_t s = (hipStream_t)stream;
    const int pix_per_block = 256;
    int nblk = partial_blocks;
    float* mr = stats_scratch;
    float* partial = stats_scratch + (long)N * C * 2;
    if (partial_blocks == 0) {
        nblk = cdiv(hw, pix_per_block);
        hipLaunchKernelGGL(groupnorm_stats_kernel<float>, dim3(nblk, N), dim3(256), 0, s, x, (long)hw, C, pix_per_block, partial);
    }
    hipLaunchKernelGGL(groupnorm_finalize_f64_kernel, dim3(cdiv((long)N * 32, 4)), dim3(256), 0, s, partial, nblk, N, C,
                       (double)hw * (double)(C / 32), eps, mr);
    const long chunks = (long)N * hw * (C / 8);
    if (f16)
        hipLaunchKernelGGL(groupnorm_apply_split_kernel<true>, dim3(cdiv(chunks, 256)), dim3(256), 0, s, x, (long)hw, C, mr, w, b, swish,
                           (bf16_t*)planes_bf16, chunks);
    else
        hipLaunchKernelGGL(groupnorm_apply_split_kernel<false>, dim3(cdiv(chunks, 256)), dim3(256), 0, s, x, (long)hw, C, mr, w, b, swish,
                           (bf16_t*)planes_bf16, chunks);
    MMVID_LAUNCH_CHECK("groupnorm_split");
    return MMVID_OK;
}
```

mmvid_amd/csrc/optim.hip:

```cpp
#include "../../include/mmvid_hip.h"
#include "common.h"

namespace {

__global__ __launch_bounds__(256) void grad_sqnorm_kernel(const float* __restrict__ g, long n,
                                                          float* __restrict__ out) {
    float a = 0.f;
    const long stride = (long)gridDim.x * 256 * 4;
    for (long i = ((long)blockIdx.x * 256 + threadIdx.x) * 4; i < n; i += stride) {
        if (i + 3 < n) {
            const float4 v = *reinterpret_cast<const float4*>(g + i);
            a += (v.x * v.x + v.y * v.y) + (v.z * v.z + v.w * v.w);
        } else {
            for (long k = i; k < n; ++k) a += g[k] * g[k];
        }
    }
    a = wave_sum(a);
    __shared__ float sh[4];
    if ((threadIdx.x & 63) == 0) sh[threadIdx.x >> 6] = a;
    __syncthreads();
    if (threadIdx.x == 0) unsafeAtomicAdd(out, (sh[0] + sh[1]) + (sh[2] + sh[3]));
}

struct AdamArgs {
    float lr, beta1, beta2, eps, weight_decay, bc1, bc2_sqrt, max_norm, grad_scale;
};
struct LazyRows {
    const unsigned char* flags;
    long lo, hi;
    int rowlen;
};
__device__ __forceinline__ bool lazy_skip(const LazyRows& z, long i) {
    return z.flags && i >= z.lo && i < z.hi && z.flags[(i - z.lo) / z.rowlen] == 0;
}

__global__ __launch_bounds__(256) void adam_kernel(float* __restrict__ p, const float* __restrict__ g,
                                                   float* __restrict__ m, float* __restrict__ v,
                                                   bf16_t* __restrict__ shadow, long n, AdamArgs a,
                                                   const float* __restrict__ sqnorm,
                                                   const float* __restrict__ step_dev,
                                                   const float* __restrict__ lr_dev, LazyRows z) {
    if (lr_dev) a.lr = *lr_dev;
    if (step_dev) {
        const float t = *step_dev;
        a.bc1 = 1.0f - powf(a.beta1, t);
        a.bc2_sqrt = sqrtf(1.0f - powf(a.beta2, t));
    }
    float coef = a.grad_scale;
    if (sqnorm && a.max_norm > 0.f) {
        const float c = a.max_norm / (sqrtf(*sqnorm) * a.grad_scale + 1e-6f);
        coef *= c < 1.f ? c : 1.f;
    }
    const float step = a.lr / a.bc1;
    const long stride = (long)gridDim.x * 256 * 4;
    for (long i = ((long)blockIdx.x * 256 + threadIdx.x) * 4; i < n; i += stride) {
        if (lazy_skip(z, i)) continue;
        if (i + 3 < n) {
            float4 pp = *reinterpret_cast<float4*>(p + i);
            const float4 gg = *reinterpret_cast<const float4*>(g + i);
            float4 mm = *reinterpret_cast<float4*>(m + i), vv = *reinterpret_cast<float4*>(v + i);
            float pe[4] = {pp.x, pp.y, pp.z, pp.w}, ge[4] = {gg.x, gg.y, gg.z, gg.w};
            float me[4] = {mm.x, mm.y, mm.z, mm.w}, ve[4] = {vv.x, vv.y, vv.z, vv.w};
#pragma unroll
            for (int e = 0; e < 4; ++e) {
                float gr = ge[e] * coef + a.weight_decay * pe[e];
                me[e] = a.beta1 * me[e] + (1.f - a.beta1) * gr;
                ve[e] = a.beta2 * ve[e] + (1.f - a.beta2) * gr * gr;
                pe[e] -= step * me[e] / (sqrtf(ve[e]) / a.bc2_sqrt + a.eps);
            }
            *reinterpret_cast<float4*>(p + i) = make_float4(pe[0], pe[1], pe[2], pe[3]);
            *reinterpret_cast<float4*>(m + i) = make_float4(me[0], me[1], me[2], me[3]);
            *reinterpret_cast<float4*>(v + i) = make_float4(ve[0], ve[1], ve[2], ve[3]);
            if (shadow) *reinterpret_cast<uint2*>(shadow + i) = make_uint2(pack_bf2(pe[0], pe[1]), pack_bf2(pe[2], pe[3]));
        } else {
            for (long k = i; k < n; ++k) {
                float gr = g[k] * coef + a.weight_decay * p[k];
                float mk = a.beta1 * m[k] + (1.f - a.beta1) * gr;
                float vk = a.beta2 * v[k] + (1.f - a.beta2) * gr * gr;
                float pk = p[k] - step * mk / (sqrtf(vk) / a.bc2_sqrt + a.eps);
                p[k] = pk, m[k] = mk, v[k] = vk;
                if (shadow) shadow[k] = f2bf(pk);
            }
        }
    }
}

__global__ __launch_bounds__(256) void cast_bf16_kernel(const float* __restrict__ x, bf16_t* __restrict__ y, long n) {
    const long stride = (long)gridDim.x * 256 * 4;
    for (long i = ((long)blockIdx.x * 256 + threadIdx.x) * 4; i < n; i += stride) {
        if (i + 3 < n) {
            const float4 v = *reinterpret_cast<const float4*>(x + i);
            *reinterpret_cast<uint2*>(y + i) = make_uint2(pack_bf2(v.x, v.y), pack_bf2(v.z, v.w));
        } else {
            for (long k = i; k < n; ++k) y[k] = f2bf(x[k]);
        }
    }
}

static int grid_for(long n) {
    long b = (n + 1023) / 1024;
    if (b > 2048) b = 2048;
    if (b < 1) b = 1;
    return (int)b;
}

}

extern "C" int mmvid_grad_sqnorm(const float* g, int64_t n, float* out_accum, void* stream) {
    MMVID_REQUIRE(g && out_accum && n >= 0, "grad_sqnorm: bad arguments");
    MMVID_REQUIRE(((uintptr_t)g & 15) == 0, "grad_sqnorm: buffer must be 16-byte aligned");
    if (n == 0) return MMVID_OK;
    hipLaunchKernelGGL(grad_sqnorm_kernel, dim3(grid_for(n)), dim3(256), 0, (hipStream_t)stream, g, (long)n, out_accum);
    MMVID_LAUNCH_CHECK("grad_sqnorm");
    return MMVID_OK;
}

__global__ __launch_bounds__(256) void grad_sqnorm_partial_kernel(const float* __restrict__ g, long n, float* __restrict__ part,
                                                                  LazyRows z) {
    float a = 0.f;
    const long stride = (long)gridDim.x * 256 * 4;
    for (long i = ((long)blockIdx.x * 256 + threadIdx.x) * 4; i < n; i += stride) {
        if (lazy_skip(z, i)) continue;
        if (i + 3 < n) {
            const float4 v = *reinterpret_cast<const float4*>(g + i);
            a += (v.x * v.x + v.y * v.y) + (v.z * v.z + v.w * v.w);
        } else {
            for (long k = i; k < n; ++k) a += g[k] * g[k];
        }
    }
    a = wave_sum(a);
    __shared__ float sh[4];
    if ((threadIdx.x & 63) == 0) sh[threadIdx.x >> 6] = a;
    __syncthreads();
    if (threadIdx.x == 0) part[blockIdx.x] = (sh[0] + sh[1]) + (sh[2] + sh[3]);
}
__global__ __launch_bounds__(256) void sum_partials_kernel(const float* __restrict__ part, int nb, float* __restrict__ out) {
    __shared__ float sh[256];
    float a = 0.f;
    for (int i = threadIdx.x; i < nb; i += 256) a += part[i];
    sh[threadIdx.x] = a;
    __syncthreads();
    for (int o = 128; o > 0; o >>= 1) {
        if ((int)threadIdx.x < o) sh[threadIdx.x] += sh[threadIdx.x + o];
        __syncthreads();
    }
    if (threadIdx.x == 0) out[0] += sh[0];
}

static int make_lazy(LazyRows& z, const uint8_t* flags, int64_t lo, int64_t rows, int rowlen, int64_t n) {
    z.flags = nullptr, z.lo = z.hi = 0, z.rowlen = 1;
    if (!flags) return MMVID_OK;
    MMVID_REQUIRE(lo >= 0 && rows >= 0 && rowlen > 0 && rowlen % 4 == 0 && lo % 4 == 0 && lo + rows * rowlen <= n,
                  "lazy rows: the table [%lld, +%lld x %d) must lie inside the buffer and be 4-element aligned", (long long)lo,
                  (long long)rows, rowlen);
    z.flags = flags, z.lo = lo, z.hi = lo + rows * rowlen, z.rowlen = rowlen;
    return MMVID_OK;
}

extern "C" int mmvid_grad_sqnorm_det(const float* g, int64_t n, float* partials, float* out_accum, void* stream) {
    return mmvid_grad_sqnorm_rows(g, n, partials, out_accum, nullptr, 0, 0, 0, stream);
}

extern "C" int mmvid_grad_sqnorm_rows(const float* g, int64_t n, float* partials, float* out_accum, const uint8_t* row_flags,
                                      int64_t table_lo, int64_t table_rows, int rowlen, void* stream) {
    MMVID_REQUIRE(g && partials && out_accum && n >= 0, "grad_sqnorm_det: bad arguments");
    MMVID_REQUIRE(((uintptr_t)g & 15) == 0, "grad_sqnorm_det: buffer must be 16-byte aligned");
    if (n == 0) return MMVID_OK;
    LazyRows z;
    if (int rc = make_lazy(z, row_flags, table_lo, table_rows, rowlen, n)) return rc;
    const int nb = grid_for(n);
    hipLaunchKernelGGL(grad_sqnorm_partial_kernel, dim3(nb), dim3(256), 0, (hipStream_t)stream, g, (long)n, partials, z);
    hipLaunchKernelGGL(sum_partials_kernel, dim3(1), dim3(256), 0, (hipStream_t)stream, partials, nb, out_accum);
    MMVID_LAUNCH_CHECK("grad_sqnorm_det");
    return MMVID_OK;
}

extern "C" int mmvid_adam_step_lr(float* p, const float* g, float* m, float* v, void* shadow_bf16, int64_t n, float lr,
                                  const float* lr_dev, float beta1, float beta2, float eps, float weight_decay, int step,
                                  const float* step_dev, float max_norm, const float* sqnorm, float grad_scale, void* stream);

extern "C" int mmvid_adam_step(float* p, const float* g, float* m, float* v, void* shadow_bf16, int64_t n, float lr,
                               float beta1, float beta2, float eps, float weight_decay, int step,
                               const float* step_dev, float max_norm, const float* sqnorm, float grad_scale,
                               void* stream) {
    return mmvid_adam_step_lr(p, g, m, v, shadow_bf16, n, lr, nullptr, beta1, beta2, eps, weight_decay, step, step_dev, max_norm,
                              sqnorm, grad_scale, stream);
}

extern "C" int mmvid_adam_step_lr(float* p, const float* g, float* m, float* v, void* shadow_bf16, int64_t n, float lr,
                                  const float* lr_dev, float beta1, float beta2, float eps, float weight_decay, int step,
                                  const float* step_dev, float max_norm, const float* sqnorm, float grad_scale, void* stream) {
    return mmvid_adam_step_rows(p, g, m, v, shadow_bf16, n, lr, lr_dev, beta1, beta2, eps, weight_decay, step, step_dev, max_norm,
                                sqnorm, grad_scale, nullptr, 0, 0, 0, stream);
}

extern "C" int mmvid_adam_step_rows(float* p, const float* g, float* m, float* v, void* shadow_bf16, int64_t n, float lr,
                                    const float* lr_dev, float beta1, float beta2, float eps, float weight_decay, int step,
                                    const float* step_dev, float max_norm, const float* sqnorm, float grad_scale,
                                    const uint8_t* row_flags, int64_t table_lo, int64_t table_rows, int rowlen, void* stream) {
    MMVID_REQUIRE(p && g && m && v && n >= 0 && (step >= 1 || step_dev), "adam_step: bad arguments");
    MMVID_REQUIRE(!row_flags || weight_decay == 0.f, "adam_step: lazy rows are exact only without weight decay");
    LazyRows z;
    if (int rc = make_lazy(z, row_flags, table_lo, table_rows, rowlen, n)) return rc;
    MMVID_REQUIRE((((uintptr_t)p | (uintptr_t)g | (uintptr_t)m | (uintptr_t)v) & 15) == 0 && ((uintptr_t)shadow_bf16 & 7) == 0,
                  "adam_step: buffers must be 16-byte aligned");
    if (n == 0) return MMVID_OK;
    AdamArgs a;
    a.lr = lr, a.beta1 = beta1, a.beta2 = beta2, a.eps = eps, a.weight_decay = weight_decay;
    a.bc1 = 1.0f - powf(beta1, (float)(step >= 1 ? step : 1));
    a.bc2_sqrt = sqrtf(1.0f - powf(beta2, (float)(step >= 1 ? step : 1)));
    a.max_norm = max_norm, a.grad_scale = grad_scale;
    hipLaunchKernelGGL(adam_kernel, dim3(grid_for(n)), dim3(256), 0, (hipStream_t)stream, p, g, m, v, (bf16_t*)shadow_bf16,
                       (long)n, a, sqnorm, step_dev, lr_dev, z);
    MMVID_LAUNCH_CHECK("adam_step");
    return MMVID_OK;
}

extern "C" int mmvid_cast_f32_to_bf16(const float* x, void* y, int64_t n, void* stream) {
    MMVID_REQUIRE(x && y && n >= 0, "cast_f32_to_bf16: bad arguments");
    MMVID_REQUIRE(((uintptr_t)x & 15) == 0 && ((uintptr_t)y & 7) == 0, "cast_f32_to_bf16: alignment");
    if (n == 0) return MMVID_OK;
    hipLaunchKernelGGL(cast_bf16_kernel, dim3(grid_for(n)), dim3(256), 0, (hipStream_t)stream, x, (bf16_t*)y, (long)n);
    MMVID_LAUNCH_CHECK("cast_f32_to_bf16");
    return MMVID_OK;
}
```

mmvid_amd/csrc/tower.hip:

```cpp
#include "../../include/mmvid_hip.h"
#include "common.h"
#include <vector>

#include "graphs.h"

namespace {

inline int64_t align256(int64_t x) { return (x + 255) & ~(int64_t)255; }
constexpr int kMaxSplitK = 16;
constexpr int kLnBwdBlocks = 512;

struct Dims {
    int B, L, E, H, F, layers;
    int64_t M;
};
Dims dims_of(const mmvid_tower_cfg_t& c) {
    Dims d;
    d.B = c.B, d.L = c.L, d.E = c.E, d.H = c.H, d.F = c.F, d.layers = c.layers;
    d.M = (int64_t)c.B * c.L;
    return d;
}

struct SavedLayer {
    int64_t x_in, x_mid, mean1, rstd1, mean2, rstd2, h1, qkv, o, lse2, h2, pre, act, k_gpj, k_dpre, k_gout, k_dqkv, k_ln1, k_ln2, total;
};
SavedLayer saved_layout(const Dims& d) {
    SavedLayer s;
    int64_t off = 0;
    auto take = [&](int64_t bytes) {
        int64_t o = off;
        off += align256(bytes);
        return o;
    };
    s.x_in = take(d.M * d.E * 4);
    s.x_mid = take(d.M * d.E * 4);
    s.mean1 = take(d.M * 4), s.rstd1 = take(d.M * 4), s.mean2 = take(d.M * 4), s.rstd2 = take(d.M * 4);
    s.h1 = take(d.M * d.E * 2);
    s.qkv = take(d.M * 3 * d.E * 2);
    s.o = take(d.M * d.E * 2);
    s.lse2 = take((int64_t)d.B * d.H * d.L * 4);
    s.h2 = take(d.M * d.E * 2);
    s.pre = take(d.M * d.F * 2);
    s.act = take(d.M * d.F * 2);
    const int64_t keep = 1;
    s.k_gpj = take(keep * d.M * d.E * 2), s.k_dpre = take(keep * d.M * d.F * 2);
    s.k_gout = take(keep * d.M * d.E * 2), s.k_dqkv = take(keep * d.M * 3 * d.E * 2);
    s.k_ln1 = take(keep * (int64_t)kLnBwdBlocks * 3 * d.E * 4), s.k_ln2 = take(keep * (int64_t)kLnBwdBlocks * 3 * d.E * 4);
    s.total = off;
    return s;
}

struct Scratch {
    int64_t delta, d_h, d_o, splitk_ws, infer, total;
};
Scratch scratch_layout(const Dims& d) {
    Scratch s;
    int64_t off = 0;
    auto take = [&](int64_t bytes) {
        int64_t o = off;
        off += align256(bytes);
        return o;
    };
    s.delta = take((int64_t)d.B * d.H * d.L * 4);
    s.d_h = take(d.M * d.E * 2);
    s.d_o = take(d.M * d.E * 2);
    s.splitk_ws = take((int64_t)kMaxSplitK * d.F * d.E * 4);
    s.infer = take(saved_layout(d).total);
    s.total = off;
    return s;
}

int64_t det_slab_bytes(const Dims& d) {
    const int64_t a = mmvid_gemm_bf16_det_workspace_bytes((int)d.M, d.F, 1, 1);
    const int64_t b = mmvid_attention_bwd_bias_det_workspace_bytes(d.B, d.L, d.E);
    const int64_t c = mmvid_colsum_bf16_det_workspace_bytes(d.M, d.E);
    return a > b ? (a > c ? a : c) : (b > c ? b : c);
}

#define TRY(call)                   \
    do {                            \
        int rc__ = (call);          \
        if (rc__ != 0) return rc__; \
    } while (0)

int check_cfg(const mmvid_tower_cfg_t* c) {
    MMVID_REQUIRE(c, "tower: null config");
    MMVID_REQUIRE(c->B > 0 && c->L > 0 && c->layers > 0, "tower: bad B/L/layers");
    MMVID_REQUIRE(c->E == c->H * 64 && c->E % 8 == 0 && c->F % 8 == 0 && c->E <= 1024,
                  "tower: need E == 64*H <= 1024 and F %% 8 == 0 (E=%d H=%d F=%d)", c->E, c->H, c->F);
    return 0;
}

int linear_fwd(int64_t M, int N, int K, const void* X, const void* W, const float* bias, const float* residual,
               void* save_pre, int act, float* out_f32, void* out_bf16, void* st) {
    return mmvid_gemm_bf16(0, 0, (int)M, N, K, X, K, W, K, 1, 0, 0, 0, 1, 1.0f, bias, residual, N, nullptr, save_pre, N,
                           act, 0, out_f32, out_bf16, N, nullptr, st);
}
int linear_dx(int64_t M, int N, int K, const void* dY, const void* W, const void* dact_pre, float* out_f32,
              void* out_bf16, void* st, float* out_colsum = nullptr, void* det_ws = nullptr, int64_t det_bytes = 0) {
    if (out_colsum && det_ws)
        return mmvid_gemm_bf16_det(0, 1, (int)M, K, N, dY, N, W, K, 1, 0, 0, 0, 1, 1.0f, nullptr, nullptr, 0, dact_pre, nullptr, K,
                                   0, 0, out_f32, out_bf16, K, out_colsum, det_ws, det_bytes, st);
    return mmvid_gemm_bf16(0, 1, (int)M, K, N, dY, N, W, K, 1, 0, 0, 0, 1, 1.0f, nullptr, nullptr, 0, dact_pre, nullptr, K,
                           0, 0, out_f32, out_bf16, K, out_colsum, st);
}
int linear_dw(int64_t M, int N, int K, const void* dY, const void* X, float* dW, float* db, float* ws, void* st) {
    if (dW) {
        const int sk = mmvid_gemm_dw_pick_splitk(M, N, K);
        TRY(mmvid_gemm_bf16_dw(M, N, K, dY, N, X, K, sk, ws, dW, 1, st));
    }
    if (db) TRY(mmvid_colsum_bf16(dY, N, M, N, db, st));
    return 0;
}

}

extern "C" int mmvid_tower_workspace(const mmvid_tower_cfg_t* cfg, int64_t* saved_bytes, int64_t* scratch_bytes) {
    TRY(check_cfg(cfg));
    const Dims d = dims_of(*cfg);
    if (saved_bytes) *saved_bytes = saved_layout(d).total * d.layers;
    if (scratch_bytes) *scratch_bytes = scratch_layout(d).total;
    return MMVID_OK;
}

static int tower_forward_enqueue(const mmvid_tower_cfg_t* cfg, const mmvid_tower_layer_t* layers, const float* x_in,
                                 float* x_out, void* saved, void* scratch, void* stream, void* kv_cache = nullptr,
                                 int kv_lmax = 0);
static int tower_backward_enqueue(const mmvid_tower_cfg_t* cfg, const mmvid_tower_layer_t* layers, float* g,
                                  void* saved, void* scratch, void* stream);

static uint64_t tower_key(uint64_t seed, const mmvid_tower_cfg_t* cfg, const mmvid_tower_layer_t* layers, const void* a,
                          const void* b, const void* c, const void* d, const void* stream) {
    uint64_t k = mmvid_hash_bytes(cfg, sizeof(*cfg), 0xcbf29ce484222325ull ^ seed);
    k = mmvid_hash_bytes(layers, sizeof(mmvid_tower_layer_t) * (size_t)cfg->layers, k);
    return mmvid_hash_ptr(stream, mmvid_hash_ptr(d, mmvid_hash_ptr(c, mmvid_hash_ptr(b, mmvid_hash_ptr(a, k)))));
}

extern "C" int mmvid_tower_forward(const mmvid_tower_cfg_t* cfg, const mmvid_tower_layer_t* layers,
                                   const float* x_in, float* x_out, void* saved, void* scratch, void* stream) {
    TRY(check_cfg(cfg));
    MMVID_REQUIRE(layers && x_in && x_out && scratch, "tower_forward: null pointer");
    const uint64_t key = tower_key(2, cfg, layers, x_in, x_out, saved, scratch, stream);
    return mmvid_run_cached(key, (hipStream_t)stream, [=](hipStream_t s) {
        return tower_forward_enqueue(cfg, layers, x_in, x_out, saved, scratch, (void*)s);
    });
}

static int tower_forward_enqueue(const mmvid_tower_cfg_t* cfg, const mmvid_tower_layer_t* layers, const float* x_in,
                                 float* x_out, void* saved, void* scratch, void* stream, void* kv_cache, int kv_lmax) {
    const Dims d = dims_of(*cfg);
    const SavedLayer sl = saved_layout(d);
    const Scratch sc = scratch_layout(d);
    char* scr = (char*)scratch;
    const float scale = 0.125f;
    const float* x = x_in;
    for (int i = 0; i < d.layers; ++i) {
        const mmvid_tower_layer_t& ly = layers[i];
        char* sv = saved ? (char*)saved + (int64_t)i * sl.total : scr + sc.infer;
        float* xin_s = (float*)(sv + sl.x_in);
        float* xmid = (float*)(sv + sl.x_mid);
        if (saved && i == 0) {
            if (hipMemcpyAsync(xin_s, x_in, d.M * d.E * 4, hipMemcpyDeviceToDevice, (hipStream_t)stream) != hipSuccess) {
                mmvid_set_error("tower_forward: memcpy failed");
                return MMVID_ERR_HIP;
            }
            x = xin_s;
        }
        float* xnext;
        if (i == d.layers - 1)
            xnext = x_out;
        else if (saved)
            xnext = (float*)((char*)saved + (int64_t)(i + 1) * sl.total + sl.x_in);
        else
            xnext = x_out;
        TRY(mmvid_layernorm_fwd(x, d.E, d.M, d.E, ly.ln1_w, ly.ln1_b, cfg->ln_eps, sv + sl.h1, nullptr, d.E,
                                (float*)(sv + sl.mean1), (float*)(sv + sl.rstd1), stream));
        TRY(linear_fwd(d.M, 3 * d.E, d.E, sv + sl.h1, ly.in_w, ly.in_b, nullptr, nullptr, 0, nullptr, sv + sl.qkv, stream));
        if (kv_cache)
            TRY(mmvid_kv_store(sv + sl.qkv, 3 * d.E, d.B, d.L, d.E, nullptr, 0, kv_lmax,
                               (char*)kv_cache + (int64_t)i * d.B * kv_lmax * 2 * d.E * 2, stream));
        TRY(mmvid_attention_fwd(sv + sl.qkv, 3 * d.E, d.B, d.L, d.H, d.E, scale, cfg->mask_mode, cfg->r0, cfg->c0, cfg->r1,
                                cfg->c1, sv + sl.o, d.E, (float*)(sv + sl.lse2), stream));
        TRY(linear_fwd(d.M, d.E, d.E, sv + sl.o, ly.out_w, ly.out_b, x, nullptr, 0, xmid, nullptr, stream));
        TRY(mmvid_layernorm_fwd(xmid, d.E, d.M, d.E, ly.ln2_w, ly.ln2_b, cfg->ln_eps, sv + sl.h2, nullptr, d.E,
                                (float*)(sv + sl.mean2), (float*)(sv + sl.rstd2), stream));
        TRY(linear_fwd(d.M, d.F, d.E, sv + sl.h2, ly.fc_w, ly.fc_b, nullptr, saved ? sv + sl.pre : nullptr, 1, nullptr,
                       sv + sl.act, stream));
        TRY(linear_fwd(d.M, d.E, d.F, sv + sl.act, ly.pj_w, ly.pj_b, xmid, nullptr, 0, xnext, nullptr, stream));
        x = xnext;
    }
    return MMVID_OK;
}

extern "C" int mmvid_tower_backward(const mmvid_tower_cfg_t* cfg, const mmvid_tower_layer_t* layers, float* g,
                                    void* saved, void* scratch, void* stream) {
    TRY(check_cfg(cfg));
    MMVID_REQUIRE(layers && g && saved && scratch, "tower_backward: null pointer");
    const uint64_t key = tower_key(mmvid_option(MMVID_OPT_DETERMINISTIC) ? 5 : 3, cfg, layers, g, saved, scratch, nullptr, stream);
    return mmvid_run_cached(key, (hipStream_t)stream, [=](hipStream_t s) {
        return tower_backward_enqueue(cfg, layers, g, saved, scratch, (void*)s);
    });
}

static int tower_backward_enqueue(const mmvid_tower_cfg_t* cfg, const mmvid_tower_layer_t* layers, float* g, void* saved,
                                  void* scratch, void* stream) {
    const Dims d = dims_of(*cfg);
    const SavedLayer sl = saved_layout(d);
    const Scratch sc = scratch_layout(d);
    char* scr = (char*)scratch;
    char* keep = (char*)saved;
    struct { int64_t g_pj, d_pre, g_out, dqkv, total; } kl = {sl.k_gpj, sl.k_dpre, sl.k_gout, sl.k_dqkv, sl.total};
    const float scale = 0.125f;
    void* d_h = scr + sc.d_h;
    float* ws = (float*)(scr + sc.splitk_ws);
    void* det_ws = nullptr;
    const int64_t det_bytes = det_slab_bytes(d);
    if (mmvid_option(MMVID_OPT_DETERMINISTIC)) {
        MMVID_REQUIRE(det_bytes <= sc.total - sc.infer, "tower_backward: the deterministic slabs do not fit the scratch arena");
        det_ws = scr + sc.infer;
    }
    const int64_t ln_ws_floats = (int64_t)kLnBwdBlocks * 3 * d.E;
    std::vector<mmvid_ln_reduce_t> ln_items;
    int ln_blocks = 0;
    for (int i = d.layers - 1; i >= 0; --i) {
        const mmvid_tower_layer_t& ly = layers[i];
        const char* sv = (const char*)saved + (int64_t)i * sl.total;
        char* kp = keep + (int64_t)i * kl.total;
        void* g_pj = kp + kl.g_pj;
        if (i == d.layers - 1) {
            TRY(mmvid_cast_f32_to_bf16(g, g_pj, d.M * d.E, stream));
            if (ly.g_pj_b && det_ws) TRY(mmvid_colsum_bf16_det(g_pj, d.E, d.M, d.E, ly.g_pj_b, det_ws, det_bytes, stream));
            if (ly.g_pj_b && !det_ws) TRY(mmvid_colsum_bf16(g_pj, d.E, d.M, d.E, ly.g_pj_b, stream));
        }
        TRY(linear_dx(d.M, d.E, d.F, g_pj, ly.pj_w, sv + sl.pre, nullptr, kp + kl.d_pre, stream, ly.g_fc_b, det_ws, det_bytes));
        TRY(linear_dx(d.M, d.F, d.E, kp + kl.d_pre, ly.fc_w, nullptr, nullptr, d_h, stream));
        {
            mmvid_ln_reduce_t r = {(const float*)(kp + sl.k_ln2), ly.g_ln2_w, ly.g_ln2_b, ly.g_out_b};
            int nb = 0;
            TRY(mmvid_layernorm_bwd_partial(d_h, 1, d.E, (const float*)(sv + sl.x_mid), d.E, (const float*)(sv + sl.mean2),
                                            (const float*)(sv + sl.rstd2), ly.ln2_w, d.M, d.E, g, d.E, 1, kp + kl.g_out, r.dw != nullptr,
                                            r.db != nullptr, r.dx_colsum != nullptr, (float*)(kp + sl.k_ln2), ln_ws_floats, &nb, stream));
            if (r.dw || r.db || r.dx_colsum) ln_items.push_back(r), ln_blocks = nb;
        }
        TRY(linear_dx(d.M, d.E, d.E, kp + kl.g_out, ly.out_w, nullptr, nullptr, scr + sc.d_o, stream));
        if (det_ws)
            TRY(mmvid_attention_bwd_bias_det(sv + sl.qkv, 3 * d.E, sv + sl.o, d.E, scr + sc.d_o, d.E, (const float*)(sv + sl.lse2),
                                             (float*)(scr + sc.delta), d.B, d.L, d.H, d.E, scale, cfg->mask_mode, cfg->r0, cfg->c0,
                                             cfg->r1, cfg->c1, kp + kl.dqkv, 3 * d.E, ly.g_in_b, det_ws, det_bytes, stream));
        else
            TRY(mmvid_attention_bwd_bias(sv + sl.qkv, 3 * d.E, sv + sl.o, d.E, scr + sc.d_o, d.E, (const float*)(sv + sl.lse2),
                                         (float*)(scr + sc.delta), d.B, d.L, d.H, d.E, scale, cfg->mask_mode, cfg->r0, cfg->c0,
                                         cfg->r1, cfg->c1, kp + kl.dqkv, 3 * d.E, ly.g_in_b, stream));
        TRY(linear_dx(d.M, 3 * d.E, d.E, kp + kl.dqkv, ly.in_w, nullptr, nullptr, d_h, stream));
        {
            mmvid_ln_reduce_t r = {(const float*)(kp + sl.k_ln1), ly.g_ln1_w, ly.g_ln1_b, i > 0 ? layers[i - 1].g_pj_b : nullptr};
            int nb = 0;
            TRY(mmvid_layernorm_bwd_partial(d_h, 1, d.E, (const float*)(sv + sl.x_in), d.E, (const float*)(sv + sl.mean1),
                                            (const float*)(sv + sl.rstd1), ly.ln1_w, d.M, d.E, g, d.E, 1,
                                            i > 0 ? (void*)(keep + (int64_t)(i - 1) * kl.total + kl.g_pj) : nullptr, r.dw != nullptr,
                                            r.db != nullptr, r.dx_colsum != nullptr, (float*)(kp + sl.k_ln1), ln_ws_floats, &nb, stream));
            if (r.dw || r.db || r.dx_colsum) ln_items.push_back(r), ln_blocks = nb;
        }
    }
    if (!ln_items.empty()) TRY(mmvid_layernorm_bwd_reduce_multi((int)ln_items.size(), ln_items.data(), ln_blocks, d.E, stream));
    struct Kind {
        int N, K;
        int64_t dy_off, x_off;
        float* mmvid_tower_layer_t::*gw;
    };
    const Kind kinds[4] = {{d.E, d.F, kl.g_pj, sl.act, &mmvid_tower_layer_t::g_pj_w},
                           {d.F, d.E, kl.d_pre, sl.h2, &mmvid_tower_layer_t::g_fc_w},
                           {d.E, d.E, kl.g_out, sl.o, &mmvid_tower_layer_t::g_out_w},
                           {3 * d.E, d.E, kl.dqkv, sl.h1, &mmvid_tower_layer_t::g_in_w}};
    std::vector<float*> outs((size_t)d.layers * 4);
    mmvid_dw_kind_t kd[4];
    int nk = 0;
    for (const Kind& k : kinds) {
        float** o = outs.data() + (size_t)nk * d.layers;
        bool any = false;
        for (int i = 0; i < d.layers; ++i) o[i] = layers[i].*(k.gw), any = any || o[i];
        if (!any) continue;
        kd[nk].N = k.N, kd[nk].K = k.K;
        kd[nk].dY = keep + k.dy_off, kd[nk].ldy = k.N, kd[nk].strideY = kl.total / 2;
        kd[nk].X = (const char*)saved + k.x_off, kd[nk].ldx = k.K, kd[nk].strideX = sl.total / 2;
        kd[nk].dW_list = o;
        ++nk;
    }
    if (nk == 0) return MMVID_OK;
    if (mmvid_gemm_dw_multi_fill(nk, kd, d.layers) >= 0.7) return mmvid_gemm_bf16_dw_multi(d.M, nk, kd, d.layers, 1, stream);
    for (int k = 0; k < nk; ++k)
        for (int i = d.layers - 1; i >= 0; --i)
            TRY(linear_dw(d.M, kd[k].N, kd[k].K, (const char*)kd[k].dY + (int64_t)i * kl.total, (const char*)kd[k].X + (int64_t)i * sl.total,
                          kd[k].dW_list[i], nullptr, ws, stream));
    return MMVID_OK;
}

extern "C" int mmvid_tower_prefill(const mmvid_tower_cfg_t* cfg, const mmvid_tower_layer_t* layers, const float* x_in,
                                   float* x_out, void* kv_cache, int Lmax, void* scratch, void* stream) {
    TRY(check_cfg(cfg));
    MMVID_REQUIRE(layers && x_in && x_out && kv_cache && scratch, "tower_prefill: null pointer");
    MMVID_REQUIRE(cfg->mask_mode == 1 && cfg->L <= Lmax, "tower_prefill: needs the causal mask and L (%d) <= Lmax (%d)", cfg->L,
                  Lmax);
    return tower_forward_enqueue(cfg, layers, x_in, x_out, nullptr, scratch, stream, kv_cache, Lmax);
}

extern "C" int mmvid_tower_decode(const mmvid_tower_cfg_t* cfg, const mmvid_tower_layer_t* layers, const float* x_in,
                                  float* x_out, void* kv_cache, int Lmax, const int32_t* pos_dev, int pos, void* scratch,
                                  void* stream) {
    TRY(check_cfg(cfg));
    MMVID_REQUIRE(layers && x_in && x_out && kv_cache && scratch, "tower_decode: null pointer");
    MMVID_REQUIRE(cfg->mask_mode == 1, "tower_decode: incremental decoding needs the causal mask");
    const int B = cfg->B, E = cfg->E, F = cfg->F, H = cfg->H;
    char* p = (char*)scratch;
    auto take = [&](int64_t bytes) {
        char* o = p;
        p += align256(bytes);
        return o;
    };
    void* h = take((int64_t)B * E * 2);
    void* qkv = take((int64_t)B * 3 * E * 2);
    void* o = take((int64_t)B * E * 2);
    float* xmid = (float*)take((int64_t)B * E * 4);
    void* act = take((int64_t)B * F * 2);
    float* xa = (float*)take((int64_t)B * E * 4);
    float* xb = (float*)take((int64_t)B * E * 4);
    const float* x = x_in;
    for (int i = 0; i < cfg->layers; ++i) {
        const mmvid_tower_layer_t& ly = layers[i];
        void* cache = (char*)kv_cache + (int64_t)i * B * Lmax * 2 * E * 2;
        float* xnext = (i == cfg->layers - 1) ? x_out : ((i & 1) ? xb : xa);
        TRY(mmvid_layernorm_fwd(x, E, B, E, ly.ln1_w, ly.ln1_b, cfg->ln_eps, h, nullptr, E, nullptr, nullptr, stream));
        TRY(linear_fwd(B, 3 * E, E, h, ly.in_w, ly.in_b, nullptr, nullptr, 0, nullptr, qkv, stream));
        TRY(mmvid_kv_store(qkv, 3 * E, B, 1, E, pos_dev, pos, Lmax, cache, stream));
        TRY(mmvid_attention_decode(qkv, 3 * E, cache, B, Lmax, H, E, pos_dev, pos, 0.125f, o, E, stream));
        TRY(linear_fwd(B, E, E, o, ly.out_w, ly.out_b, x, nullptr, 0, xmid, nullptr, stream));
        TRY(mmvid_layernorm_fwd(xmid, E, B, E, ly.ln2_w, ly.ln2_b, cfg->ln_eps, h, nullptr, E, nullptr, nullptr, stream));
        TRY(linear_fwd(B, F, E, h, ly.fc_w, ly.fc_b, nullptr, nullptr, 1, nullptr, act, stream));
        TRY(linear_fwd(B, E, F, act, ly.pj_w, ly.pj_b, xmid, nullptr, 0, xnext, nullptr, stream));
        x = xnext;
    }
    return MMVID_OK;
}
```

mmvid_amd/engine.py:

```python
import os

import torch
import torch.distributed as dist

from . import _lib, ops

ALIGN = 128


def _round_up(x, m):
    return (x + m - 1) // m * m


class WarmupLR:

    def __init__(self, warmup_min_lr=1e-6, warmup_max_lr=1e-4, warmup_num_steps=5000, every=1):
        self.min_lr, self.max_lr = float(warmup_min_lr), float(warmup_max_lr)
        self.warmup = max(2, int(warmup_num_steps))
        self.every = max(1, int(every))

    def lr_at(self, iteration):
        import math
        ns = iteration // self.every
        if ns == 0:
            return self.max_lr
        k = ns - 1
        gamma = math.log(k + 1) / math.log(self.warmup) if k < self.warmup else 1.0
        return self.min_lr + (self.max_lr - self.min_lr) * gamma


class FlatTrainer:
    def __init__(self, model, lr=1e-4, betas=(0.9, 0.999), eps=1e-8, weight_decay=0.0, max_grad_norm=1.0,
                 process_group=None, bucket_mb=64, order=None, lr_schedule=None, force_exchange=False, sparse_tables=True,
                 lazy_rows=True, exchange=None):
        self.model = model
        self.exchange = os.environ.get('MMVID_EXCHANGE', exchange or 'allreduce')
        assert self.exchange in ('allreduce', 'direct'), self.exchange
        self._direct_buf = None
        self.sparse_tables = bool(sparse_tables) and os.environ.get('MMVID_SPARSE_TABLES', '1') != '0'
        self.lr_schedule = lr_schedule
        self.force_exchange = bool(force_exchange) and dist.is_available() and dist.is_initialized()
        self.exchange_enabled = True
        params = [(n, p) for n, p in model.named_parameters() if p.requires_grad]
        if order is not None:
            params = order(params)
        self.names = [n for n, _ in params]
        self.params = [p for _, p in params]
        dev = self.params[0].device
        offs, tot = [], 0
        for p in self.params:
            offs.append(tot)
            tot += _round_up(p.numel(), ALIGN)
        self.offsets, self.numel = offs, tot
        self.P = torch.zeros(tot, device=dev, dtype=torch.float32)
        self.G = torch.zeros(tot, device=dev, dtype=torch.float32)
        self.M = torch.zeros(tot, device=dev, dtype=torch.float32)
        self.V = torch.zeros(tot, device=dev, dtype=torch.float32)
        self.S = torch.zeros(tot, device=dev, dtype=torch.bfloat16) if dev.type == 'cuda' else None
        for p, o in zip(self.params, offs):
            n = p.numel()
            self.P[o:o + n].copy_(p.detach().reshape(-1))
            p.data = self.P[o:o + n].view(p.shape)
            p.grad = self.G[o:o + n].view(p.shape)
        if self.S is not None:
            ops.cast_bf16(self.P, self.S)
            self._attach_shadows()
        self.lr, self.betas, self.eps, self.wd, self.max_norm = lr, betas, eps, weight_decay, max_grad_norm
        self.step_count = 0
        self.pg = process_group
        self.world = dist.get_world_size(process_group) if (dist.is_available() and dist.is_initialized()) else 1
        self.bucket_elems = max(ALIGN, int(bucket_mb * (1 << 20) / 4) // ALIGN * ALIGN)
        self._sq = torch.zeros(1, device=dev, dtype=torch.float32)
        self._sq_partials = torch.zeros(2048, device=dev, dtype=torch.float32) if dev.type == 'cuda' else None
        self._step_dev = torch.zeros(1, device=dev, dtype=torch.float32) if dev.type == 'cuda' else None
        self._lr_dev = torch.full((1, ), float(lr), device=dev, dtype=torch.float32) if dev.type == 'cuda' else None
        self._comm_stream = torch.cuda.Stream(device=dev) if dev.type == 'cuda' else None
        self._works = []
        self._sent_from = tot
        self._layer_start = {}
        for n, o in zip(self.names, offs):
            if n.startswith('transformer.transformer.resblocks.'):
                i = int(n.split('.')[3])
                self._layer_start[i] = min(o, self._layer_start.get(i, tot))
        tw = getattr(model, 'transformer', None)
        if tw is not None and hasattr(tw, 'on_layers_done') and self._layer_start and (self.world > 1 or self.force_exchange):
            tw.on_layers_done = self.layers_done
        self._init_lazy_rows(lazy_rows and os.environ.get('MMVID_LAZY_ROWS', '1') != '0')

    def _init_lazy_rows(self, enabled):
        self._lazy = None
        fn = getattr(self.model, 'sparse_grad_rows', None)
        if not enabled or fn is None or self.S is None or self.wd != 0.0:
            return
        names = [n for n in fn() if n in self.names]
        if len(names) != 1:
            return
        i = self.names.index(names[0])
        p = self.params[i]
        if p.dim() != 2 or p.shape[1] % 4 != 0:
            return
        dev = p.device
        self._lazy = {'name': names[0], 'lo': self.offsets[i], 'rows': p.shape[0], 'rowlen': p.shape[1],
                      'flags': torch.zeros(p.shape[0], device=dev, dtype=torch.uint8),
                      'dirty': None, 'dirty_n': 0, 'all_dirty': True}

    def _lazy_arg(self):
        z = self._lazy
        return None if z is None else (z['flags'], z['lo'], z['rows'], z['rowlen'])

    def _lazy_mark(self, ids):
        z = self._lazy
        if z is None:
            return
        if ids is None:
            z['flags'].fill_(1)
            z['all_dirty'] = True
            return
        ids = ids.reshape(-1).clamp_min(0)
        z['flags'].index_fill_(0, ids, 1)
        if z['all_dirty']:
            return
        n = ids.numel()
        if z['dirty'] is None or z['dirty_n'] + n > z['dirty'].numel():
            if z['dirty'] is not None and z['dirty_n'] > 0 or torch.cuda.is_current_stream_capturing():
                z['all_dirty'] = True
                return
            z['dirty'] = torch.zeros(max(4 * n, 1024), device=ids.device, dtype=torch.int64)
            z['dirty_n'] = 0
        z['dirty'][z['dirty_n']:z['dirty_n'] + n].copy_(ids)
        z['dirty_n'] += n

    def _shadow_view(self, p):
        i = next(k for k, q in enumerate(self.params) if q is p)
        o = self.offsets[i]
        return self.S[o:o + p.numel()].view(p.shape)

    def _attach_shadows(self):
        m = self.model
        self._tower_shadow_attached = False
        tw = getattr(m, 'transformer', None)
        if tw is not None and hasattr(tw, 'attach_shadow') and all(p.requires_grad for p in tw._matrix_params()):
            tw.attach_shadow([self._shadow_view(p) for p in tw._matrix_params()])
            self._tower_shadow_attached = True
        if hasattr(m, 'attach_head_shadow') and hasattr(m, 'head_shadow_targets'):
            for lin in m.head_shadow_targets():
                if lin.weight.requires_grad:
                    m.attach_head_shadow(lin, self._shadow_view(lin.weight))

    def _check_bindings(self):
        for p, o in zip(self.params, self.offsets):
            if p.data_ptr() != self.P.data_ptr() + 4 * o:
                raise RuntimeError('a parameter no longer lives in FlatTrainer.P (moved by .to() / load_state_dict(assign=True)); '
                                   'rebuild the trainer after moving the model')
            if p.grad is None or p.grad.data_ptr() != self.G.data_ptr() + 4 * o:
                stray = p.grad
                p.grad = self.G[o:o + p.numel()].view(p.shape)
                if stray is not None:
                    p.grad.add_(stray)
                    if self._lazy is not None and o == self._lazy['lo']:
                        self._lazy_mark(None)

    def state_dict(self):
        state = {}
        for i, (p, o) in enumerate(zip(self.params, self.offsets)):
            n = p.numel()
            state[i] = {'step': torch.tensor(float(self.step_count)), 'exp_avg': self.M[o:o + n].view(p.shape).clone(),
                        'exp_avg_sq': self.V[o:o + n].view(p.shape).clone()}
        group = {'lr': self.lr, 'betas': self.betas, 'eps': self.eps, 'weight_decay': self.wd, 'amsgrad': False,
                 'params': list(range(len(self.params)))}
        out = {'state': state, 'param_groups': [group], 'names': list(self.names)}
        fe = getattr(self.model, 'frontend', None)
        if fe is not None and hasattr(fe, 'state_dict'):
            out['frontend'] = fe.state_dict()
        return out

    def load_state_dict(self, sd):
        if 'names' in sd:
            names = list(sd['names'])
        else:
            names = [n for n, p in self.model.named_parameters() if p.requires_grad]
        if sorted(names) != sorted(self.names):
            raise ValueError('optimizer state was saved for a different set of parameters: '
                             f'{sorted(set(names) ^ set(self.names))[:6]} ...')
        at = {n: i for i, n in enumerate(self.names)}
        steps, loaded = set(), []
        for j, name in enumerate(names):
            st = sd['state'].get(j, sd['state'].get(str(j)))
            if st is None:
                continue
            i = at[name]
            p, o, n = self.params[i], self.offsets[i], self.params[i].numel()
            for k in ('exp_avg', 'exp_avg_sq'):
                if tuple(st[k].shape) != tuple(p.shape):
                    raise ValueError(f'optimizer state entry {j} ({name}): {k} has shape {tuple(st[k].shape)}, the parameter '
                                     f'{tuple(p.shape)}')
            loaded.append((o, n, st))
            steps.add(int(float(st['step'])))
        if len(steps) > 1:
            raise ValueError('per-parameter step counts differ')
        for o, n, st in loaded:
            self.M[o:o + n].copy_(st['exp_avg'].reshape(-1))
            self.V[o:o + n].copy_(st['exp_avg_sq'].reshape(-1))
        if steps:
            self.step_count = steps.pop()
            if self._step_dev is not None:
                self._step_dev.fill_(float(self.step_count))
        g = sd['param_groups'][0]
        self.lr, self.betas, self.eps, self.wd = g['lr'], tuple(g['betas']), g['eps'], g['weight_decay']
        fe = getattr(self.model, 'frontend', None)
        if fe is not None and 'frontend' in sd and hasattr(fe, 'load_state_dict'):
            fe.load_state_dict(sd['frontend'])
        z = getattr(self, '_lazy', None)
        if z is not None:
            lo, hi = z['lo'], z['lo'] + z['rows'] * z['rowlen']
            live = (self.M[lo:hi].view(z['rows'], -1).abs().amax(1) > 0) | (self.V[lo:hi].view(z['rows'], -1).amax(1) > 0)
            z['flags'].copy_(live.to(torch.uint8) | z['flags'])

    def refresh_shadows(self):
        if self.S is not None:
            ops.cast_bf16(self.P, self.S)
            self._attach_shadows()

    def zero_grad(self):
        z = self._lazy
        if z is not None:
            pending = getattr(self.model, 'table_grad_pending', None)
            if pending is None:
                pending = not getattr(self, '_stepped_since_zero', True)
            if pending or getattr(self.model, '_text_id_overflow', False):
                z['all_dirty'] = True
        self._stepped_since_zero = False
        if z is None or z['all_dirty']:
            self.G.zero_()
        else:
            lo, hi = z['lo'], z['lo'] + z['rows'] * z['rowlen']
            self.G[:lo].zero_()
            self.G[hi:].zero_()
            if z['dirty_n']:
                self.G[lo:hi].view(z['rows'], z['rowlen']).index_fill_(0, z['dirty'][:z['dirty_n']], 0.0)
        if z is not None:
            z['all_dirty'], z['dirty_n'] = False, 0
            if hasattr(self.model, 'table_grad_pending'):
                self.model.table_grad_pending = False
        reset = getattr(self.model, 'reset_sparse_grad_rows', None)
        if reset is not None:
            reset()

    def _sparse_ranges(self):
        fn = getattr(self.model, 'sparse_grad_rows', None)
        if not self.sparse_tables or fn is None:
            return []
        out = []
        for name, ids in fn().items():
            if name in self.names and ids is not None:
                i = self.names.index(name)
                out.append((self.offsets[i], self.offsets[i] + _round_up(self.params[i].numel(), ALIGN)))
        return sorted(out)

    def _send(self, lo, hi):
        if (self.world == 1 and not self.force_exchange) or hi <= lo or not self.exchange_enabled:
            return
        pieces, at = [], lo
        for a, b in self._sparse_ranges():
            if b <= at or a >= hi:
                continue
            if a > at:
                pieces.append((at, a))
            at = max(at, b)
        if at < hi:
            pieces.append((at, hi))
        if self._comm_stream is not None:
            self._comm_stream.wait_stream(torch.cuda.current_stream())
        for plo, phi in pieces:
            for s in range(plo, phi, self.bucket_elems):
                e = min(s + self.bucket_elems, phi)
                if self._comm_stream is not None:
                    with torch.cuda.stream(self._comm_stream):
                        self._reduce_message(s, e)
                else:
                    self._reduce_message(s, e)

    def _reduce_message(self, s, e):
        if self.exchange == 'allreduce' or self.world == 1 or (e - s) % self.world != 0:
            self._works.append(dist.all_reduce(self.G[s:e], op=dist.ReduceOp.SUM, group=self.pg, async_op=True))
            return
        n, w = e - s, self.world
        if self._direct_buf is None or self._direct_buf.numel() < n + n // w:
            self._direct_buf = torch.empty(self.bucket_elems + self.bucket_elems // w + w, device=self.G.device, dtype=torch.float32)
        recv = self._direct_buf[:n].view(w, n // w)
        shard = self._direct_buf[n:n + n // w]
        msg = self.G[s:e]
        nccl = dist.get_backend(self.pg) == 'nccl'
        if nccl:
            dist.all_to_all_single(recv.view(-1), msg, group=self.pg)
        else:
            me, parts = self._rank(), msg.view(w, n // w)
            recv[me].copy_(parts[me])
            reqs = [dist.P2POp(dist.isend, parts[j].contiguous(), j, self.pg) for j in range(w) if j != me] + \
                   [dist.P2POp(dist.irecv, recv[j], j, self.pg) for j in range(w) if j != me]
            for r in dist.batch_isend_irecv(reqs):
                r.wait()
        torch.sum(recv, dim=0, out=shard)
        if nccl:
            dist.all_gather_into_tensor(msg, shard, group=self.pg)
        else:
            dist.all_gather(list(msg.view(w, n // w).unbind(0)), shard, group=self.pg)

    def _gather(self, t):
        out = torch.empty((self.world * t.shape[0], ) + tuple(t.shape[1:]), device=t.device, dtype=t.dtype)
        if dist.get_backend(self.pg) == 'nccl':
            dist.all_gather_into_tensor(out, t, group=self.pg)
        else:
            dist.all_gather(list(out.chunk(self.world, 0)), t, group=self.pg)
        return out

    def _exchange_sparse(self):
        fn = getattr(self.model, 'sparse_grad_rows', None)
        if not self.sparse_tables or fn is None or not self.exchange_enabled:
            return
        rank = self._rank()
        for name, ids in fn().items():
            if name not in self.names or ids is None:
                continue
            W = self.params[self.names.index(name)].grad
            uid, rows = self.pack_rows(W, ids)
            all_ids = self._gather(uid)
            self.merge_rows(W, all_ids, self._gather(rows), rank, uid.shape[0])
            if self._lazy is not None and self._lazy['name'] == name:
                self._lazy_mark(all_ids)

    def _rank(self):
        return dist.get_rank(self.pg)

    @staticmethod
    def pack_rows(W, ids):
        ids = ids.reshape(-1)
        if W.is_cuda and ids.numel() <= 4096 and W.dtype == torch.float32 and W.is_contiguous():
            uid = torch.empty_like(ids)
            rows = torch.empty(ids.numel(), W.shape[1], device=W.device, dtype=W.dtype)
            _lib.call('mmvid_rows_pack', ops._p(W), W.shape[0], W.shape[1], ops._p(ids.contiguous()), ids.numel(), ops._p(uid), ops._p(rows),
                      ops._stream())
            return uid, rows
        srt, _ = torch.sort(ids)
        first = torch.ones_like(srt, dtype=torch.bool)
        first[1:] = srt[1:] != srt[:-1]
        uid = torch.where(first, srt, torch.full_like(srt, -1))
        rows = W.index_select(0, srt) * first.unsqueeze(1).to(W.dtype)
        return uid, rows

    @staticmethod
    def merge_rows(W, all_ids, all_rows, rank, n):
        if W.is_cuda and W.dtype == torch.float32 and W.is_contiguous():
            for r in range(all_ids.shape[0] // n):
                if r != rank:
                    _lib.call('mmvid_rows_merge', ops._p(W), W.shape[0], W.shape[1], ops._p(all_ids[r * n:(r + 1) * n]),
                              ops._p(all_rows[r * n:(r + 1) * n]), n, ops._stream())
            return
        own = torch.zeros(all_ids.shape[0], dtype=torch.bool, device=all_ids.device)
        own[rank * n:(rank + 1) * n] = True
        valid = (all_ids >= 0) & ~own
        W.index_add_(0, all_ids.clamp_min(0), all_rows * valid.unsqueeze(1).to(W.dtype))

    def layers_done(self, first_layer):
        lo = self._layer_start.get(first_layer)
        if lo is None or lo >= self._sent_from:
            return
        self._send(lo, self._sent_from)
        self._sent_from = lo

    def after_failed_capture(self):
        if self._comm_stream is not None:
            self._comm_stream = torch.cuda.Stream(device=self.G.device)
        self._works = []
        self._sent_from = self.numel

    def allreduce_grads(self):
        if self.world > 1 or self.force_exchange:
            self._send(0, self._sent_from)
            if self._comm_stream is not None:
                with torch.cuda.stream(self._comm_stream):
                    self._exchange_sparse()
            else:
                self._exchange_sparse()
            for w in self._works:
                w.wait()
            self._works = []
            if self._comm_stream is not None:
                torch.cuda.current_stream().wait_stream(self._comm_stream)
        self._sent_from = self.numel

    def step(self):
        self._check_bindings()
        self.allreduce_grads()
        if self._lazy is not None:
            ids = self.model.sparse_grad_rows().get(self._lazy['name'])
            dense_exchange = (self.world > 1 or self.force_exchange) and self.exchange_enabled and not self.sparse_tables
            self._lazy_mark(None if dense_exchange else ids)
            if hasattr(self.model, 'table_grad_pending'):
                self.model.table_grad_pending = False
        self._stepped_since_zero = True
        self.step_count += 1
        gscale = 1.0 / self.world
        self._sq.zero_()
        lr_dev = None
        if self._step_dev is not None:
            if self.lr_schedule is not None:
                sc = self.lr_schedule
                ops.lr_schedule(self._step_dev, 1, sc.min_lr, sc.max_lr, sc.warmup, sc.every, self._lr_dev)
                lr_dev = self._lr_dev
            ops.counter_add(self._step_dev, 1.0)
        ops.grad_sqnorm(self.G, self._sq, partials=self._sq_partials, lazy=self._lazy_arg())
        ops.adam_step(self.P, self.G, self.M, self.V, self.S, self.step_count, self.lr, self.betas, self.eps, self.wd,
                      self.max_norm, self._sq, gscale, step_dev=self._step_dev, lr_dev=lr_dev, lazy=self._lazy_arg())
        tw = getattr(self.model, 'transformer', None)
        if tw is not None and hasattr(tw, 'mark_shadow_fresh') and getattr(self, '_tower_shadow_attached', False):
            tw.mark_shadow_fresh()

    def grad_norm(self):
        return float(self.G.norm()) / self.world


class GraphedStep:

    def __init__(self, trainer, fn, example_inputs, warmup=2):
        self.trainer, self.fn = trainer, fn
        self.static = {k: v.clone() for k, v in example_inputs.items()}
        self.graph, self.capture_error = None, None
        self.deterministic = _lib.is_deterministic()
        side = torch.cuda.Stream()
        side.wait_stream(torch.cuda.current_stream())
        with torch.cuda.stream(side):
            for _ in range(warmup):
                self._step()
        torch.cuda.current_stream().wait_stream(side)
        torch.cuda.synchronize()
        saved = (trainer.step_count, trainer._step_dev.clone(), self._frontend_steps())
        graph = torch.cuda.CUDAGraph()
        mode = 'thread_local' if (dist.is_available() and dist.is_initialized()) else 'global'
        try:
            with torch.cuda.graph(graph, capture_error_mode=mode):
                self.loss = self._step()
            self.graph = graph
        except Exception as e:
            self.capture_error = f'{type(e).__name__}: {e}'.splitlines()[0][:200]
            try:
                torch.cuda.synchronize()
            except Exception:
                pass
            trainer.after_failed_capture()
        trainer.step_count = saved[0]
        trainer._step_dev.copy_(saved[1])
        self._frontend_steps(saved[2])

    def _frontend_steps(self, restore=None):
        fe = getattr(self.trainer.model, 'frontend', None)
        if fe is None or fe.step is None:
            return None
        if restore is not None:
            fe.step.copy_(restore)
            return None
        return fe.step.clone()

    def _step(self):
        self.trainer.zero_grad()
        loss = self.fn(**self.static)
        loss.backward()
        self.trainer.step()
        return loss.detach()

    def __call__(self, **inputs):
        if _lib.is_deterministic() != self.deterministic:
            raise RuntimeError(f'this GraphedStep was captured with deterministic={self.deterministic} and is called with '
                               f'deterministic={_lib.is_deterministic()}: a replay would run the other mode\'s kernels; switch back '
                               '(mmvid_amd.set_deterministic) or capture a new GraphedStep')
        for k, v in inputs.items():
            self.static[k].copy_(v, non_blocking=True)
        if self.graph is None:
            return self._step()
        self.graph.replay()
        self.trainer.step_count += 1
        return self.loss


_CAPTURABLE = {}


def collectives_capturable(device):
    if not (dist.is_available() and dist.is_initialized()):
        return True
    if dist.get_backend() != 'nccl':
        return False
    key = (dist.get_world_size(), str(device))
    if key in _CAPTURABLE:
        return _CAPTURABLE[key]

    def vote(ok):
        flag = torch.tensor([1 if ok else 0], device=device, dtype=torch.int32)
        dist.all_reduce(flag, op=dist.ReduceOp.MIN)
        return bool(int(flag.item()))

    pg = None
    try:
        pg = dist.new_group(backend='nccl')
    except Exception:
        pg = None
    ok = vote(pg is not None)
    if ok:
        t = torch.zeros(64, device=device)
        try:
            dist.all_reduce(t, group=pg)
            torch.cuda.synchronize()
        except Exception:
            ok = False
        ok = vote(ok)
    if ok:
        try:
            g = torch.cuda.CUDAGraph()
            with torch.cuda.graph(g, capture_error_mode='thread_local'):
                dist.all_reduce(t, group=pg)
            g.replay()
            torch.cuda.synchronize()
        except Exception:
            ok = False
            try:
                torch.cuda.synchronize()
            except Exception:
                pass
        ok = vote(ok)
    _CAPTURABLE[key] = ok
    return ok


def backward_order(params):
    def key(item):
        n = item[0]
        if n.startswith('transformer.transformer.resblocks.'):
            return (1, int(n.split('.')[3]))
        if n.startswith('to_logits'):
            return (2, 0)
        return (0, 0)

    return sorted(params, key=key)


def broadcast_parameters(model, src=0, group=None):
    if not (dist.is_available() and dist.is_initialized()):
        return
    for t in list(model.parameters()) + list(model.buffers()):
        dist.broadcast(t.data, src=src, group=group)
```

mmvid_amd/ops.py:

```python
import ctypes

import torch

from . import _lib
from ._lib import call

bf16, f32, i64 = torch.bfloat16, torch.float32, torch.int64


def _stream():
    return ctypes.c_void_p(torch.cuda.current_stream().cuda_stream)


def _p(t):
    if t is None:
        return None
    return ctypes.c_void_p(t.data_ptr())


_DET_WS = {}


def _det_ws(op, device, nbytes):
    key = (op, str(device), int(nbytes))
# ... 240 lines not shown
    rf = residual if (residual is not None and residual.dtype == f32) else None
    gp = ctypes.c_void_p(gn_stats.data_ptr() + N * Cout * 2 * 4) if gn_stats is not None else None
    call('mmvid_conv3x3_strip_nhwc', _p(x), N, H, W, Cin, _p(w), _p(bias), Cout, _p(rb), _p(rf),
         _p(out) if out_dtype == bf16 else _p(o16), _p(out) if out_dtype == f32 else None, gp, _stream())
    return (out, o16) if o16 is not None else out


def groupnorm_swish(x, w, b, eps=1e-6, swish=True, out_dtype=bf16, stats=None, stats_block=128):
    N, H, W, C = x.shape
    assert x.is_contiguous() and x.dtype in (bf16, f32)
    blocks = 0
    if stats is None:
        stats = gn_stats_buffer(N, H * W, C, x.device)
    else:
        assert (H * W) % stats_block == 0
        blocks = H * W // stats_block
    y = torch.empty(x.shape, device=x.device, dtype=out_dtype)
    call('mmvid_groupnorm_swish_nhwc', _p(x), int(x.dtype == bf16), N, H * W, C, _p(w), _p(b), float(eps), int(swish),
         _p(stats), blocks, _p(y) if out_dtype == bf16 else None, _p(y) if out_dtype == f32 else None, _stream())
    return y


def _mask_args(mask):
    if mask is None:
        return 0, -1, 0, -1, 0
    if mask == 'causal':
        return 1, -1, 0, -1, 0
    kind, rows = mask
    assert kind == 'rows' and len(rows) <= 2
    rows = list(rows) + [(-1, 0)] * (2 - len(rows))
    return 2, rows[0][0], rows[0][1], rows[1][0], rows[1][1]


def attention_fwd(qkv, B, L, H, mask=None, scale=0.125):
    _chk(qkv, bf16, 'qkv')
    E = H * 64
    out = torch.empty(B * L, E, device=qkv.device, dtype=bf16)
    lse2 = torch.empty(B, H, L, device=qkv.device, dtype=f32)
    call('mmvid_attention_fwd', _p(qkv), 3 * E, B, L, H, E, float(scale), *_mask_args(mask), _p(out), E, _p(lse2),
         _stream())
    return out, lse2


def attention_bwd(qkv, out, dout, lse2, B, L, H, mask=None, scale=0.125, dbias=None):
    E = H * 64
    delta = torch.empty(B, H, L, device=qkv.device, dtype=f32)
    dqkv = torch.empty_like(qkv)
    if dbias is not None and _lib.is_deterministic():
        ws = _det_ws('attention_bwd_bias', qkv.device, _lib.load().mmvid_attention_bwd_bias_det_workspace_bytes(B, L, E))
        call('mmvid_attention_bwd_bias_det', _p(qkv), 3 * E, _p(out), E, _p(dout), E, _p(lse2), _p(delta), B, L, H, E, float(scale),
             *_mask_args(mask), _p(dqkv), 3 * E, _p(dbias), _p(ws), ws.numel(), _stream())
        return dqkv
    call('mmvid_attention_bwd_bias', _p(qkv), 3 * E, _p(out), E, _p(dout), E, _p(lse2), _p(delta), B, L, H, E, float(scale),
         *_mask_args(mask), _p(dqkv), 3 * E, _p(dbias) if dbias is not None else None, _stream())
    return dqkv


def _ptr_array(tensors):
    arr = (ctypes.c_void_p * len(tensors))(*[t.data_ptr() if t is not None else 0 for t in tensors])
    return ctypes.cast(arr, ctypes.POINTER(ctypes.c_void_p)), arr


def assemble_sequence(tables, ids, seg, pos):
    B, L = ids.shape
    E = pos.shape[-1]
    for t in tables:
        _chk(t, f32, 'table')
    _chk(ids, i64, 'ids'), _chk(pos, f32, 'pos')
    assert seg.dtype == torch.int32 and seg.is_cuda
    out = torch.empty(B, L, E, device=ids.device, dtype=f32)
    tp, keep = _ptr_array(tables)
    rows = (ctypes.c_int64 * len(tables))(*[t.shape[0] for t in tables])
    call('mmvid_assemble_sequence', tp, rows, len(tables), _p(ids), _p(seg), _p(pos), B, L, E, _p(out), _stream())
    return out


def assemble_sequence_bwd(grad_tables, table_rows, ids, seg, dx, dpos=None, accumulate_dpos=False):
    B, L = ids.shape
    E = dx.shape[-1]
    _chk(dx, f32, 'dx')
    tp, keep = _ptr_array(grad_tables)
    rows = (ctypes.c_int64 * len(grad_tables))(*table_rows)
    if _lib.is_deterministic():
        nb = _lib.load().mmvid_assemble_sequence_bwd_det_workspace_bytes(B, L, E, len(grad_tables), rows)
        if nb < 0:
            raise _lib.MMVIDError('assemble_sequence_bwd: tables / batch too large for the deterministic form (2^31 destinations)')
        ws = _det_ws('assemble_sequence_bwd', dx.device, nb)
        call('mmvid_assemble_sequence_bwd_det', tp, rows, len(grad_tables), _p(ids), _p(seg), _p(dx), B, L, E, _p(dpos),
             int(accumulate_dpos), _p(ws), ws.numel(), _stream())
        return
    call('mmvid_assemble_sequence_bwd', tp, rows, len(grad_tables), _p(ids), _p(seg), _p(dx), B, L, E, _p(dpos),
         int(accumulate_dpos), _stream())


def cross_entropy_fwd(logits, target, select):
    _chk(logits, f32, 'logits'), _chk(target, i64, 'target')
    rows, V = logits.shape
    lse = torch.empty(rows, device=logits.device, dtype=f32)
    loss = torch.zeros(1, device=logits.device, dtype=f32)
    if _lib.is_deterministic():
        ws = _det_ws('cross_entropy_fwd', logits.device, rows * 4)
        call('mmvid_cross_entropy_fwd_det', _p(logits), V, _p(target), _p(select), rows, V, _p(lse), _p(loss), _p(ws), ws.numel(),
             _stream())
        return lse, loss
    call('mmvid_cross_entropy_fwd', _p(logits), V, _p(target), _p(select), rows, V, _p(lse), _p(loss), _stream())
    return lse, loss


def cross_entropy_bwd(logits, target, select, lse, gscale):
    rows, V = logits.shape
    d = torch.empty(rows, V, device=logits.device, dtype=bf16)
    call('mmvid_cross_entropy_bwd', _p(logits), V, _p(target), _p(select), _p(lse), _p(gscale), rows, V, _p(d), V,
         _stream())
    return d


def colsum_bf16(dy, db):
    M, N = dy.shape
    if _lib.is_deterministic():
        ws = _det_ws('colsum_bf16', dy.device, _lib.load().mmvid_colsum_bf16_det_workspace_bytes(M, N))
        call('mmvid_colsum_bf16_det', _p(dy), N, M, N, _p(db), _p(ws), ws.numel(), _stream())
        return
    call('mmvid_colsum_bf16', _p(dy), N, M, N, _p(db), _stream())


def grad_sqnorm(g, out, partials=None, lazy=None):
    _chk(g, f32, 'g'), _chk(out, f32, 'out')
    if lazy is not None:
        assert partials is not None
        fl, lo, rows, rowlen = lazy
        call('mmvid_grad_sqnorm_rows', _p(g), g.numel(), _p(partials), _p(out), _p(_chk(fl, torch.uint8, 'row_flags')), int(lo), int(rows),
             int(rowlen), _stream())
    elif partials is not None:
        call('mmvid_grad_sqnorm_det', _p(g), g.numel(), _p(partials), _p(out), _stream())
    else:
        call('mmvid_grad_sqnorm', _p(g), g.numel(), _p(out), _stream())


def adam_step(p, g, m, v, shadow, step, lr, betas=(0.9, 0.999), eps=1e-8, weight_decay=0.0, max_norm=0.0,
              sqnorm=None, grad_scale=1.0, step_dev=None, lr_dev=None, lazy=None):
    for t, n in ((p, 'p'), (g, 'g'), (m, 'm'), (v, 'v')):
        _chk(t, f32, n)
    fl, lo, rows, rowlen = lazy if lazy is not None else (None, 0, 0, 0)
    call('mmvid_adam_step_rows', _p(p), _p(g), _p(m), _p(v), _p(shadow), p.numel(), float(lr), _p(lr_dev), float(betas[0]),
         float(betas[1]), float(eps), float(weight_decay), int(step), _p(step_dev), float(max_norm), _p(sqnorm),
         float(grad_scale), _p(fl), int(lo), int(rows), int(rowlen), _stream())


def lr_schedule(step_dev, kind, lr_min, lr_max, warmup, every, lr_out):
    call('mmvid_lr_schedule', _p(step_dev), int(kind), float(lr_min), float(lr_max), int(warmup), int(every), _p(lr_out),
         _stream())


def counter_add(counter, value=1.0):
    call('mmvid_counter_add', _p(counter), float(value), _stream())


def cast_bf16(x, out=None):
    _chk(x, f32, 'x')
    if out is None:
        out = torch.empty(x.shape, device=x.device, dtype=bf16)
    call('mmvid_cast_f32_to_bf16', _p(x), _p(out), x.numel(), _stream())
    return out


def conv2d_nhwc(x, w, bias, mode, residual=None, clamp01=False, out_dtype=bf16, gn_stats=None, splitk=1):
    _chk(x, bf16, 'x'), _chk(w, bf16, 'w')
    N, H, W, Cin = x.shape
    Cout = w.shape[0]
    Ho, Wo = (H // 2, W // 2) if mode == 1 else ((2 * H, 2 * W) if mode == 2 else (H, W))
    out = torch.empty(N, Ho, Wo, Cout, device=x.device, dtype=out_dtype)
    rb = residual if (residual is not None and residual.dtype == bf16) else None
    rf = residual if (residual is not None and residual.dtype == f32) else None
    gp = None
    if gn_stats is not None:
        gp = ctypes.c_void_p(gn_stats.data_ptr() + N * Cout * 2 * 4)
    ws = torch.empty(splitk * N * Ho * Wo * Cout, device=x.device, dtype=f32) if splitk > 1 else None
    call('mmvid_conv2d_nhwc_splitk', mode, _p(x), N, H, W, Cin, _p(w), _p(bias), Cout, _p(rb), _p(rf), int(clamp01),
         _p(out) if out_dtype == bf16 else None, _p(out) if out_dtype == f32 else None, gp, int(splitk), _p(ws), _stream())
    return out


def split_planes(x):
    _chk(x, f32, 'x')
    out = torch.empty((2, ) + tuple(x.shape), device=x.device, dtype=bf16)
    call('mmvid_split_f32_bf16x2', _p(x.contiguous()), x.numel(), _p(out), _stream())
    return out


def split_weights(w):
    hi = w.to(bf16)
    lo = (w - hi.float()).to(bf16)
    return torch.stack([hi, hi, lo], 1).contiguous()


def conv2d_nhwc_split3(x_planes, w3, bias, mode, residual=None, clamp01=False, splitk=1, strip=False, planes_out=None):
    _chk(x_planes, bf16, 'x_planes'), _chk(w3, bf16, 'w3')
    _, N, H, W, Cin = x_planes.shape
    Cout = w3.shape[0]
    Ho, Wo = (H // 2, W // 2) if mode == 1 else ((2 * H, 2 * W) if mode == 2 else (H, W))
    out = torch.empty(N, Ho, Wo, Cout, device=x_planes.device, dtype=f32)
    if strip:
        assert mode == 0 and not clamp01 and splitk == 1
        call('mmvid_conv3x3_strip_nhwc_split3', _p(x_planes), N, H, W, Cin, _p(w3), _p(bias), Cout, _p(residual), _p(out), None, _p(planes_out),
             _stream())
        return out
    ws = torch.empty(splitk * N * Ho * Wo * Cout, device=out.device, dtype=f32) if splitk > 1 else None
    call('mmvid_conv2d_nhwc_split3', mode, _p(x_planes), N, H, W, Cin, _p(w3), _p(bias), Cout, _p(residual), int(clamp01), _p(out),
         None, int(splitk), _p(ws), _stream())
    return out


def groupnorm_swish_split(x, w, b, eps=1e-6, swish=True):
    _chk(x, f32, 'x')
    N, H, W, C = x.shape
    out = torch.empty(2, N, H, W, C, device=x.device, dtype=bf16)
    st = torch.empty(N * (2 * C + 64 * ((H * W + 63) // 64)), device=x.device, dtype=f32)
    call('mmvid_groupnorm_swish_nhwc_split', _p(x), N, H * W, C, _p(w), _p(b), float(eps), int(swish), _p(st), 0, _p(out), _stream())
    return out


def groupnorm_swish_f16(x, w, b, eps=1e-6, swish=True):
    _chk(x, f32, 'x')
    N, H, W, C = x.shape
    out = torch.empty(N, H, W, C, device=x.device, dtype=torch.float16)
    st = torch.empty(N * (2 * C + 64 * ((H * W + 63) // 64)), device=x.device, dtype=f32)
    call('mmvid_groupnorm_swish_nhwc_f16out', _p(x), N, H * W, C, _p(w), _p(b), float(eps), int(swish), _p(st), 0, _p(out), _stream())
    return out


def conv3x3_strip_f16(x, w, bias, residual=None, planes_out=None):
    _chk(x, torch.float16, 'x'), _chk(w, torch.float16, 'w')
    N, H, W, Cin = x.shape
    Cout = w.shape[0]
    out = torch.empty(N, H, W, Cout, device=x.device, dtype=f32)
    call('mmvid_conv3x3_strip_nhwc_f16', _p(x), N, H, W, Cin, _p(w), _p(bias), Cout, _p(residual), _p(out), None, _p(planes_out), _stream())
    return out


def image_to_nhwc8(img):
    _chk(img, f32, 'img')
    N, C, H, W = img.shape
    assert C == 3
    out = torch.empty(N, H, W, 8, device=img.device, dtype=bf16)
    call('mmvid_image_to_nhwc8', _p(img), N, H, W, _p(out), _stream())
    return out


def nhwc_to_nchw(x, c_use=None):
    _chk(x, f32, 'x')
    N, H, W, C = x.shape
    c_use = c_use or C
    out = torch.empty(N, c_use, H, W, device=x.device, dtype=f32)
    call('mmvid_nhwc_to_nchw_f32', _p(x), N, H, W, C, c_use, _p(out), _stream())
    return out


def spatial_attention(q, k, v):
    N, HW, C = q.shape
    scratch = torch.empty(N * HW * HW * 3 // 2 + 16, device=q.device, dtype=f32)
    out = torch.empty_like(q)
    call('mmvid_spatial_attention', _p(q), _p(k), _p(v), N, HW, C, float(C)**-0.5, _p(scratch), _p(out), _stream())
    return out


u8 = torch.uint8


def exponential_like(shape, device):
    return torch.empty(shape, device=device, dtype=f32).exponential_()


def sample_race(logits, E, noise_u=None, temperature=0.0, logit_div=1.0, tok_offset=0, want_y=True, tok_out=None, step_dev=None, step0=0):
    _chk(E, f32, 'E')
    assert logits.dtype == f32 and logits.is_cuda and logits.stride(1) == 1
    R, V = logits.shape
    assert E.shape[-2:] == (R, V) and E.is_contiguous() and (E.dim() == 2 or (E.dim() == 3 and step_dev is not None))
    if tok_out is not None:
        _chk(tok_out, i64, 'tok_out')
        assert tok_out.shape == (R, )
    tok = tok_out if tok_out is not None else torch.empty(R, device=logits.device, dtype=i64)
    y = torch.empty(R, device=logits.device, dtype=f32) if want_y else None
    if noise_u is not None:
        _chk(noise_u, f32, 'noise_u')
    call('mmvid_sample_race_at', _p(logits), logits.stride(0), _p(E), _p(step_dev) if step_dev is not None else None, int(step0), R * V,
         _p(noise_u), float(temperature), float(logit_div), R, V, int(tok_offset), _p(tok), _p(y), _stream())
    return tok, y


def mp_select_keep(Y, E, preserve, k):
    _chk(Y, f32, 'Y'), _chk(E, f32, 'E')
    b, Bm, TS = E.shape
    mask1 = torch.empty(b, Bm, TS, device=Y.device, dtype=u8)
    if torch.is_tensor(k) or (preserve is not None and preserve.dim() == 2):
        if not torch.is_tensor(k) or preserve is None or preserve.dim() != 2:
            raise ValueError('mp_select_keep: the per-video form takes preserve [b, TS] uint8 AND k int32 [b] on the device')
        _chk(preserve, u8, 'preserve'), _chk(k, torch.int32, 'k')
        assert tuple(preserve.shape) == (b, TS) and tuple(k.shape) == (b, ), (tuple(preserve.shape), tuple(k.shape), (b, TS))
        call('mmvid_mp_select_keep_rows', _p(Y), _p(E), _p(preserve), _p(k), b, Bm, TS, _p(mask1), _stream())
        return mask1
    call('mmvid_mp_select_keep', _p(Y), _p(E), _p(preserve), b, Bm, TS, int(k), _p(mask1), _stream())
    return mask1


def mp_build_input(control_emb, image_emb, tpos, I_tok, mask1, Bm, mask_id):
    _chk(control_emb, f32, 'control_emb'), _chk(image_emb, f32, 'image_emb'), _chk(tpos, f32, 'tpos'), _chk(I_tok, i64, 'I_tok')
# ... 81 lines not shown
```

Baseline: 211,900.

## Skip zeroing tower weight gradients by writing them on first backward pass

```diff
diff --git a/include/mmvid_hip.h b/include/mmvid_hip.h
--- a/include/mmvid_hip.h
+++ b/include/mmvid_hip.h
@@ -62,6 +62,10 @@
                                 const float* rstd, const float* w, int64_t rows, int E, float* dx, int64_t lddx, int add_into_dx,
                                 void* dx_bf16, int want_dw, int want_db, int want_colsum, float* workspace,
                                 int64_t workspace_floats, int* blocks_out, void* stream);
+int mmvid_layernorm_bwd_partial_src(const void* dy, int dy_is_bf16, int64_t lddy, const float* x, int64_t ldx, const float* mean,
+                                    const float* rstd, const float* w, int64_t rows, int E, const float* dx_src, float* dx,
+                                    int64_t lddx, int add_into_dx, void* dx_bf16, int want_dw, int want_db, int want_colsum,
+                                    float* workspace, int64_t workspace_floats, int* blocks_out, void* stream);
 int mmvid_layernorm_bwd_reduce_multi(int n, const mmvid_ln_reduce_t* items, int blocks, int E, void* stream);
 int mmvid_groupnorm_swish_nhwc(const void* x, int x_is_bf16, int N, int64_t hw, int C, const float* w,
                                const float* b, float eps, int swish, float* stats_scratch, int partial_blocks,
@@ -120,6 +124,7 @@
                       float* lr_out, void* stream);
 int mmvid_counter_add(float* counter, float value, void* stream);
 int mmvid_cast_f32_to_bf16(const float* x, void* y, int64_t n, void* stream);
+int mmvid_zero_ranges(float* g, int64_t n, const int64_t* table, int n_ranges, void* stream);
 
 int mmvid_msm_masks(uint64_t seed, const float* step_dev, int B, int T, int f, const float* strategy_prob, float bern_lo,
                     float bern_hi, float pc_prob, uint8_t* mask1, float* not_fully_masked, int32_t* strategy_out,
@@ -180,6 +185,9 @@
                         float* x_out, void* saved, void* scratch, void* stream);
 int mmvid_tower_backward(const mmvid_tower_cfg_t* cfg, const mmvid_tower_layer_t* layers, float* g,
                          void* saved, void* scratch, void* stream);
+#define MMVID_TOWER_DW_FIRST_WRITE 1u
+int mmvid_tower_backward_ex(const mmvid_tower_cfg_t* cfg, const mmvid_tower_layer_t* layers, const float* g_in, float* g,
+                            void* saved, void* scratch, unsigned flags, void* stream);
 
 
 int mmvid_tower_prefill(const mmvid_tower_cfg_t* cfg, const mmvid_tower_layer_t* layers, const float* x_in,
diff --git a/mmvid_amd/_lib.py b/mmvid_amd/_lib.py
--- a/mmvid_amd/_lib.py
+++ b/mmvid_amd/_lib.py
@@ -61,6 +61,7 @@
     'mmvid_layernorm_bwd': [P, I64, P, I64, P, P, P, I64, I, P, I64, I, P, P, P, P, P],
     'mmvid_layernorm_bwd_ws': [P, I64, P, I64, P, P, P, I64, I, P, I64, I, P, P, P, P, P, I64, P],
     'mmvid_layernorm_bwd_partial': [P, I, I64, P, I64, P, P, P, I64, I, P, I64, I, P, I, I, I, P, I64, P, P],
+    'mmvid_layernorm_bwd_partial_src': [P, I, I64, P, I64, P, P, P, I64, I, P, P, I64, I, P, I, I, I, P, I64, P, P],
     'mmvid_layernorm_bwd_reduce_multi': [I, P, I, I, P],
     'mmvid_layernorm_bwd_ex': [P, I, I64, P, I64, P, P, P, I64, I, P, I64, I, P, P, P, P, P, I64, P],
     'mmvid_groupnorm_swish_nhwc': [P, I, I, I64, I, P, P, F, I, P, I, P, P, P],
@@ -78,6 +79,8 @@
     'mmvid_tower_workspace': [POINTER(TowerCfg), POINTER(I64), POINTER(I64)],
     'mmvid_tower_forward': [POINTER(TowerCfg), POINTER(TowerLayer), P, P, P, P, P],
     'mmvid_tower_backward': [POINTER(TowerCfg), POINTER(TowerLayer), P, P, P, P],
+    'mmvid_tower_backward_ex': [POINTER(TowerCfg), POINTER(TowerLayer), P, P, P, P, ctypes.c_uint, P],
+    'mmvid_zero_ranges': [P, I64, P, I, P],
     'mmvid_tower_prefill': [POINTER(TowerCfg), POINTER(TowerLayer), P, P, P, I, P, P],
     'mmvid_tower_decode': [POINTER(TowerCfg), POINTER(TowerLayer), P, P, P, I, P, I, P, P],
     'mmvid_tower_decode_fused': [POINTER(TowerCfg), POINTER(TowerLayer), P, P, P, I, P, I, P, P],
@@ -199,6 +202,7 @@
                 ('naxes', ctypes.c_int32), ('src0', ctypes.c_int32), ('d', ctypes.c_int32 * 3), ('pad', ctypes.c_int32)]
 
 
+TOWER_DW_FIRST_WRITE = 1
 ABI_VERSION = 3
 _lib = None
 
diff --git a/mmvid_amd/clip_tower.py b/mmvid_amd/clip_tower.py
--- a/mmvid_amd/clip_tower.py
+++ b/mmvid_amd/clip_tower.py
@@ -68,8 +68,7 @@
 
     @staticmethod
     def backward(ctx, gy):
-        g = gy.contiguous().clone()
-        ctx.tower._run_backward(g, ctx.saved_arena, ctx.shape)
+        g = ctx.tower._run_backward(gy.contiguous(), ctx.saved_arena, ctx.shape)
         ctx.saved_arena = None
         return _with_param_zeros(ctx, (g.view(ctx.shape), None, None) + (None, ) * (len(ctx.needs_input_grad) - 3))
 
@@ -178,6 +177,8 @@
         self._scratch_retired = []
         self.backward_chunk_layers = int(os.environ.get('MMVID_BWD_CHUNK', 0))
         self.on_layers_done = None
+        self._dw_fresh = None
+        self.use_backward_ex = os.environ.get('MMVID_TOWER_BACKWARD_EX', '1') != '0'
 
     @staticmethod
     def build_attention_mask(context_length, mask_type='causal', **kwargs):
@@ -251,6 +252,27 @@
             yield blk.attn.out_proj.weight
             yield blk.mlp.c_fc.weight
             yield blk.mlp.c_proj.weight
+
+    def first_write_params(self):
+        return list(self._matrix_params())
+
+    def expect_first_write(self, ptrs):
+        self._dw_fresh = None if ptrs is None else tuple(ptrs)
+
+    def first_write_pending(self):
+        return self._dw_fresh is not None
+
+    def _take_first_write(self):
+        if self._dw_fresh is None:
+            return False
+        ps = self.first_write_params()
+        if len(ps) != len(self._dw_fresh):
+            return False
+        for p, ptr in zip(ps, self._dw_fresh):
+            have = p.grad.data_ptr() if (p.requires_grad and p.grad is not None) else None
+            if have != ptr:
+                return False
+        return True
 
     def attach_shadow(self, views):
         self._shadow = list(views)
@@ -360,24 +382,42 @@
             self._chunk_plan = (self.layers, plan)
         return self._chunk_plan[1]
 
-    def _run_backward(self, g, saved, shape):
+    def _run_backward(self, gy, saved, shape):
         if saved is None:
             raise _lib.MMVIDError('tower backward without saved activations (forward ran under no_grad)')
         B, L, _ = shape
         cfg = self._cfg(B, L)
         layers, _keep = self._layer_structs(True)
-        _, scratch = self._workspace(cfg, g.device, False)
+        _, scratch = self._workspace(cfg, gy.device, False)
+        gy = ops._chk(gy, torch.float32, 'tower output gradient')
+        ex = self.use_backward_ex and 'mmvid_tower_backward_ex' not in _lib.load()._mmvid_missing
+        g = torch.empty_like(gy) if ex else gy.clone()
         sb = ctypes.c_int64()
         _lib.call('mmvid_tower_workspace', ctypes.byref(cfg), ctypes.byref(sb), None)
         if sb.value != saved.numel():
             raise _lib.MMVIDError(f'tower backward: the saved arena holds {saved.numel()} bytes, the current layout needs {sb.value} '
                                   '(the library changed between forward and backward)')
         per_layer = saved.numel() // self.layers
+        take = self._take_first_write()
+        flags = _lib.TOWER_DW_FIRST_WRITE if (take and ex) else 0
+        if take:
+            self._dw_fresh = None
+            if not ex:
+                for p in self.first_write_params():
+                    if p.requires_grad:
+                        p.grad.zero_()
+        g_in = gy
         for lo, hi in self.backward_chunks():
             sub = self._cfg(B, L)
             sub.layers = hi - lo
             lp = ctypes.cast(ctypes.byref(layers, lo * ctypes.sizeof(_lib.TowerLayer)), ctypes.POINTER(_lib.TowerLayer))
-            _lib.call('mmvid_tower_backward', ctypes.byref(sub), lp, ops._p(g),
-                      ctypes.c_void_p(saved.data_ptr() + lo * per_layer), ops._p(scratch), ops._stream())
+            if ex:
+                _lib.call('mmvid_tower_backward_ex', ctypes.byref(sub), lp, ops._p(g_in), ops._p(g),
+                          ctypes.c_void_p(saved.data_ptr() + lo * per_layer), ops._p(scratch), flags, ops._stream())
+                g_in = None
+            else:
+                _lib.call('mmvid_tower_backward', ctypes.byref(sub), lp, ops._p(g),
+                          ctypes.c_void_p(saved.data_ptr() + lo * per_layer), ops._p(scratch), ops._stream())
             if self.on_layers_done is not None:
                 self.on_layers_done(lo)
+        return g
diff --git a/mmvid_amd/csrc/norm.hip b/mmvid_amd/csrc/norm.hip
--- a/mmvid_amd/csrc/norm.hip
+++ b/mmvid_amd/csrc/norm.hip
@@ -79,7 +79,7 @@
                                                             const float* __restrict__ mean,
                                                             const float* __restrict__ rstd,
                                                             const float* __restrict__ w, long rows, int E,
-                                                            float* __restrict__ dx, long lddx, int add,
+                                                            const float* dx_src, float* dx, long lddx, int add,
                                                             bf16_t* __restrict__ dx_bf16,
                                                             float* __restrict__ dw, float* __restrict__ db,
                                                             float* __restrict__ dx_colsum, float* __restrict__ partial) {
@@ -101,7 +101,7 @@
         for (int i = 0; i < LN_MAXV; ++i) {
             const int c = lane + 64 * i;
             if (c < nv) {
-                prev[i] = add ? reinterpret_cast<const float4*>(dx + r * lddx)[c] : make_float4(0.f, 0.f, 0.f, 0.f);
+                prev[i] = add ? reinterpret_cast<const float4*>(dx_src + r * lddx)[c] : make_float4(0.f, 0.f, 0.f, 0.f);
                 float4 d4;
                 if constexpr (sizeof(DY) == 4) {
                     d4 = reinterpret_cast<const float4*>(dy + r * lddy)[c];
@@ -181,7 +181,7 @@
 __global__ __launch_bounds__(256) void layernorm_bwd_fast_kernel(const DY* __restrict__ dy, long lddy, const float* __restrict__ x,
                                                                  long ldx, const float* __restrict__ mean,
                                                                  const float* __restrict__ rstd, const float* __restrict__ w, long rows,
-                                                                 float* __restrict__ dx, long lddx, int add,
+                                                                 const float* dx_src, float* dx, long lddx, int add,
                                                                  bf16_t* __restrict__ dx_bf16, float* __restrict__ dw,
                                                                  float* __restrict__ db, float* __restrict__ dx_colsum,
                                                                  float* __restrict__ partial) {
@@ -206,7 +206,7 @@
 #pragma unroll
         for (int i = 0; i < NVI; ++i) {
             const int c = lane + 64 * i;
-            in.prev[i] = reinterpret_cast<const float4*>(dx + r * lddx)[c];
+            in.prev[i] = reinterpret_cast<const float4*>(dx_src + r * lddx)[c];
             in.d[i] = reinterpret_cast<const dy_raw_t*>(dy + r * lddy)[c];
             in.x4[i] = reinterpret_cast<const float4*>(x + r * ldx)[c];
         }
@@ -652,13 +652,14 @@
 }
 
 static int layernorm_bwd_impl(const void* dy, int dy_is_bf16, int64_t lddy, const float* x, int64_t ldx, const float* mean,
-                              const float* rstd, const float* w, int64_t rows, int E, float* dx, int64_t lddx, int add_into_dx,
+                              const float* rstd, const float* w, int64_t rows, int E, const float* dx_src, float* dx, int64_t lddx, int add_into_dx,
                               void* dx_bf16, float* dw, float* db, float* dx_colsum, float* workspace, int64_t workspace_floats,
                               int* blocks_out, void* stream) {
     MMVID_REQUIRE(dy && x && mean && rstd && w && dx, "layernorm_bwd: null pointer");
     MMVID_REQUIRE(E % 4 == 0 && E <= 64 * 4 * LN_MAXV && lddy % 4 == 0 && ldx % 4 == 0 && lddx % 4 == 0,
                   "layernorm_bwd: bad E/strides");
     if (rows == 0) return MMVID_OK;
+    if (!dx_src) dx_src = dx;
     int blocks = cdiv(rows, 4);
     const bool any_red = dw || db || dx_colsum;
     float* partial = nullptr;
@@ -682,7 +683,7 @@
     if (E == 768 || E == 512) {
 #define MMVID_LN_FAST(DYT, NVI)                                                                                                            \
     hipLaunchKernelGGL((layernorm_bwd_fast_kernel<DYT, NVI>), dim3(blocks), dim3(256), 0, (hipStream_t)stream, (const DYT*)dy, (long)lddy, x, \
-                       (long)ldx, mean, rstd, w, (long)rows, dx, (long)lddx, add_into_dx, (bf16_t*)dx_bf16, a_dw, a_db, a_cs, partial)
+                       (long)ldx, mean, rstd, w, (long)rows, dx_src, dx, (long)lddx, add_into_dx, (bf16_t*)dx_bf16, a_dw, a_db, a_cs, partial)
         if (dy_is_bf16) {
             if (E == 768) MMVID_LN_FAST(bf16_t, 3); else MMVID_LN_FAST(bf16_t, 2);
         } else {
@@ -691,12 +692,12 @@
 #undef MMVID_LN_FAST
     } else if (dy_is_bf16)
         hipLaunchKernelGGL(layernorm_bwd_kernel<bf16_t>, dim3(blocks), dim3(256), 0, (hipStream_t)stream, (const bf16_t*)dy, (long)lddy, x,
-                           (long)ldx, mean, rstd, w, (long)rows, E, dx, (long)lddx, add_into_dx, (bf16_t*)dx_bf16,
+                           (long)ldx, mean, rstd, w, (long)rows, E, dx_src, dx, (long)lddx, add_into_dx, (bf16_t*)dx_bf16,
                            partial ? (dw ? dw : workspace) : dw, partial ? (db ? db : workspace) : db,
                            partial ? (dx_colsum ? dx_colsum : nullptr) : dx_colsum, partial);
     else
         hipLaunchKernelGGL(layernorm_bwd_kernel<float>, dim3(blocks), dim3(256), 0, (hipStream_t)stream, (const float*)dy, (long)lddy, x,
-                           (long)ldx, mean, rstd, w, (long)rows, E, dx, (long)lddx, add_into_dx, (bf16_t*)dx_bf16,
+                           (long)ldx, mean, rstd, w, (long)rows, E, dx_src, dx, (long)lddx, add_into_dx, (bf16_t*)dx_bf16,
                            partial ? (dw ? dw : workspace) : dw, partial ? (db ? db : workspace) : db,
                            partial ? (dx_colsum ? dx_colsum : nullptr) : dx_colsum, partial);
     if (blocks_out) {
@@ -714,7 +715,7 @@
                                       const float* rstd, const float* w, int64_t rows, int E, float* dx, int64_t lddx,
                                       int add_into_dx, void* dx_bf16, float* dw, float* db, float* dx_colsum,
                                       float* workspace, int64_t workspace_floats, void* stream) {
-    return layernorm_bwd_impl(dy, dy_is_bf16, lddy, x, ldx, mean, rstd, w, rows, E, dx, lddx, add_into_dx, dx_bf16, dw, db, dx_colsum,
+    return layernorm_bwd_impl(dy, dy_is_bf16, lddy, x, ldx, mean, rstd, w, rows, E, nullptr, dx, lddx, add_into_dx, dx_bf16, dw, db, dx_colsum,
                               workspace, workspace_floats, nullptr, stream);
 }
 
@@ -722,8 +723,16 @@
                                            const float* rstd, const float* w, int64_t rows, int E, float* dx, int64_t lddx,
                                            int add_into_dx, void* dx_bf16, int want_dw, int want_db, int want_colsum,
                                            float* workspace, int64_t workspace_floats, int* blocks_out, void* stream) {
+    return mmvid_layernorm_bwd_partial_src(dy, dy_is_bf16, lddy, x, ldx, mean, rstd, w, rows, E, nullptr, dx, lddx, add_into_dx, dx_bf16,
+                                           want_dw, want_db, want_colsum, workspace, workspace_floats, blocks_out, stream);
+}
+
+extern "C" int mmvid_layernorm_bwd_partial_src(const void* dy, int dy_is_bf16, int64_t lddy, const float* x, int64_t ldx, const float* mean,
+                                               const float* rstd, const float* w, int64_t rows, int E, const float* dx_src, float* dx,
+                                               int64_t lddx, int add_into_dx, void* dx_bf16, int want_dw, int want_db, int want_colsum,
+                                               float* workspace, int64_t workspace_floats, int* blocks_out, void* stream) {
     MMVID_REQUIRE(workspace && blocks_out, "layernorm_bwd_partial: null workspace / blocks_out");
-    return layernorm_bwd_impl(dy, dy_is_bf16, lddy, x, ldx, mean, rstd, w, rows, E, dx, lddx, add_into_dx, dx_bf16,
+    return layernorm_bwd_impl(dy, dy_is_bf16, lddy, x, ldx, mean, rstd, w, rows, E, dx_src, dx, lddx, add_into_dx, dx_bf16,
                               want_dw ? workspace : nullptr, want_db ? workspace : nullptr, want_colsum ? workspace : nullptr, workspace,
                               workspace_floats, blocks_out, stream);
 }
diff --git a/mmvid_amd/csrc/optim.hip b/mmvid_amd/csrc/optim.hip
--- a/mmvid_amd/csrc/optim.hip
+++ b/mmvid_amd/csrc/optim.hip
@@ -97,6 +97,18 @@
     }
 }
 
+__global__ __launch_bounds__(256) void zero_ranges_kernel(float* __restrict__ g, long n, const long* __restrict__ table) {
+    const long off = table[2 * (long)blockIdx.x], len = table[2 * (long)blockIdx.x + 1];
+    if (off < 0 || len <= 0 || off > n || len > n - off) return;
+    const long end = off + len;
+    long a = (off + 3) & ~3l;
+    if (a > end) a = end;
+    const long b = a + ((end - a) & ~3l);
+    for (long i = off + threadIdx.x; i < a; i += 256) g[i] = 0.f;
+    for (long i = a + 4 * (long)threadIdx.x; i < b; i += 1024) *reinterpret_cast<float4*>(g + i) = make_float4(0.f, 0.f, 0.f, 0.f);
+    for (long i = b + threadIdx.x; i < end; i += 256) g[i] = 0.f;
+}
+
 static int grid_for(long n) {
     long b = (n + 1023) / 1024;
     if (b > 2048) b = 2048;
@@ -224,3 +236,12 @@
     MMVID_LAUNCH_CHECK("cast_f32_to_bf16");
     return MMVID_OK;
 }
+
+extern "C" int mmvid_zero_ranges(float* g, int64_t n, const int64_t* table, int n_ranges, void* stream) {
+    MMVID_REQUIRE(g && n >= 0 && n_ranges >= 0 && (table || n_ranges == 0), "zero_ranges: bad arguments");
+    MMVID_REQUIRE(((uintptr_t)g & 15) == 0 && ((uintptr_t)table & 7) == 0, "zero_ranges: alignment");
+    if (n_ranges == 0) return MMVID_OK;
+    hipLaunchKernelGGL(zero_ranges_kernel, dim3(n_ranges), dim3(256), 0, (hipStream_t)stream, g, (long)n, (const long*)table);
+    MMVID_LAUNCH_CHECK("zero_ranges");
+    return MMVID_OK;
+}
diff --git a/mmvid_amd/csrc/tower.hip b/mmvid_amd/csrc/tower.hip
--- a/mmvid_amd/csrc/tower.hip
+++ b/mmvid_amd/csrc/tower.hip
@@ -104,10 +104,10 @@
     return mmvid_gemm_bf16(0, 1, (int)M, K, N, dY, N, W, K, 1, 0, 0, 0, 1, 1.0f, nullptr, nullptr, 0, dact_pre, nullptr, K,
                            0, 0, out_f32, out_bf16, K, out_colsum, st);
 }
-int linear_dw(int64_t M, int N, int K, const void* dY, const void* X, float* dW, float* db, float* ws, void* st) {
+int linear_dw(int64_t M, int N, int K, const void* dY, const void* X, float* dW, float* db, float* ws, int accumulate, void* st) {
     if (dW) {
         const int sk = mmvid_gemm_dw_pick_splitk(M, N, K);
-        TRY(mmvid_gemm_bf16_dw(M, N, K, dY, N, X, K, sk, ws, dW, 1, st));
+        TRY(mmvid_gemm_bf16_dw(M, N, K, dY, N, X, K, sk, ws, dW, accumulate, st));
     }
     if (db) TRY(mmvid_colsum_bf16(dY, N, M, N, db, st));
     return 0;
@@ -126,8 +126,8 @@
 static int tower_forward_enqueue(const mmvid_tower_cfg_t* cfg, const mmvid_tower_layer_t* layers, const float* x_in,
                                  float* x_out, void* saved, void* scratch, void* stream, void* kv_cache = nullptr,
                                  int kv_lmax = 0);
-static int tower_backward_enqueue(const mmvid_tower_cfg_t* cfg, const mmvid_tower_layer_t* layers, float* g,
-                                  void* saved, void* scratch, void* stream);
+static int tower_backward_enqueue(const mmvid_tower_cfg_t* cfg, const mmvid_tower_layer_t* layers, const float* g_in, float* g,
+                                  void* saved, void* scratch, unsigned flags, void* stream);
 
 static uint64_t tower_key(uint64_t seed, const mmvid_tower_cfg_t* cfg, const mmvid_tower_layer_t* layers, const void* a,
                           const void* b, const void* c, const void* d, const void* stream) {
@@ -194,17 +194,31 @@
 
 extern "C" int mmvid_tower_backward(const mmvid_tower_cfg_t* cfg, const mmvid_tower_layer_t* layers, float* g,
                                     void* saved, void* scratch, void* stream) {
+    return mmvid_tower_backward_ex(cfg, layers, nullptr, g, saved, scratch, 0u, stream);
+}
+
+extern "C" int mmvid_tower_backward_ex(const mmvid_tower_cfg_t* cfg, const mmvid_tower_layer_t* layers, const float* g_in, float* g,
+                                       void* saved, void* scratch, unsigned flags, void* stream) {
     TRY(check_cfg(cfg));
     MMVID_REQUIRE(layers && g && saved && scratch, "tower_backward: null pointer");
-    const uint64_t key = tower_key(mmvid_option(MMVID_OPT_DETERMINISTIC) ? 5 : 3, cfg, layers, g, saved, scratch, nullptr, stream);
+    MMVID_REQUIRE((flags & ~(unsigned)MMVID_TOWER_DW_FIRST_WRITE) == 0, "tower_backward_ex: unknown flag bits 0x%x", flags);
+    if (g_in == g) g_in = nullptr;
+    if (g_in) {
+        const char *a = (const char*)g_in, *b = (const char*)g;
+        const int64_t bytes = (int64_t)cfg->B * cfg->L * cfg->E * 4;
+        MMVID_REQUIRE(a + bytes <= b || b + bytes <= a, "tower_backward_ex: g_in overlaps g");
+    }
+    const uint64_t key = tower_key((mmvid_option(MMVID_OPT_DETERMINISTIC) ? 5 : 3) + 16 * (uint64_t)flags, cfg, layers, g, saved, scratch,
+                                   g_in, stream);
     return mmvid_run_cached(key, (hipStream_t)stream, [=](hipStream_t s) {
-        return tower_backward_enqueue(cfg, layers, g, saved, scratch, (void*)s);
+        return tower_backward_enqueue(cfg, layers, g_in, g, saved, scratch, flags, (void*)s);
     });
 }
 
-static int tower_backward_enqueue(const mmvid_tower_cfg_t* cfg, const mmvid_tower_layer_t* layers, float* g, void* saved,
-                                  void* scratch, void* stream) {
+static int tower_backward_enqueue(const mmvid_tower_cfg_t* cfg, const mmvid_tower_layer_t* layers, const float* g_in, float* g,
+                                  void* saved, void* scratch, unsigned flags, void* stream) {
     const Dims d = dims_of(*cfg);
+    const int dw_accumulate = (flags & MMVID_TOWER_DW_FIRST_WRITE) ? 0 : 1;
     const SavedLayer sl = saved_layout(d);
     const Scratch sc = scratch_layout(d);
     char* scr = (char*)scratch;
@@ -228,7 +242,7 @@
         char* kp = keep + (int64_t)i * kl.total;
         void* g_pj = kp + kl.g_pj;
         if (i == d.layers - 1) {
-            TRY(mmvid_cast_f32_to_bf16(g, g_pj, d.M * d.E, stream));
+            TRY(mmvid_cast_f32_to_bf16(g_in ? g_in : g, g_pj, d.M * d.E, stream));
             if (ly.g_pj_b && det_ws) TRY(mmvid_colsum_bf16_det(g_pj, d.E, d.M, d.E, ly.g_pj_b, det_ws, det_bytes, stream));
             if (ly.g_pj_b && !det_ws) TRY(mmvid_colsum_bf16(g_pj, d.E, d.M, d.E, ly.g_pj_b, stream));
         }
@@ -237,9 +251,10 @@
         {
             mmvid_ln_reduce_t r = {(const float*)(kp + sl.k_ln2), ly.g_ln2_w, ly.g_ln2_b, ly.g_out_b};
             int nb = 0;
-            TRY(mmvid_layernorm_bwd_partial(d_h, 1, d.E, (const float*)(sv + sl.x_mid), d.E, (const float*)(sv + sl.mean2),
-                                            (const float*)(sv + sl.rstd2), ly.ln2_w, d.M, d.E, g, d.E, 1, kp + kl.g_out, r.dw != nullptr,
-                                            r.db != nullptr, r.dx_colsum != nullptr, (float*)(kp + sl.k_ln2), ln_ws_floats, &nb, stream));
+            TRY(mmvid_layernorm_bwd_partial_src(d_h, 1, d.E, (const float*)(sv + sl.x_mid), d.E, (const float*)(sv + sl.mean2),
+                                                (const float*)(sv + sl.rstd2), ly.ln2_w, d.M, d.E, i == d.layers - 1 ? g_in : nullptr, g,
+                                                d.E, 1, kp + kl.g_out, r.dw != nullptr, r.db != nullptr, r.dx_colsum != nullptr,
+                                                (float*)(kp + sl.k_ln2), ln_ws_floats, &nb, stream));
             if (r.dw || r.db || r.dx_colsum) ln_items.push_back(r), ln_blocks = nb;
         }
         TRY(linear_dx(d.M, d.E, d.E, kp + kl.g_out, ly.out_w, nullptr, nullptr, scr + sc.d_o, stream));
@@ -287,11 +302,11 @@
         ++nk;
     }
     if (nk == 0) return MMVID_OK;
-    if (mmvid_gemm_dw_multi_fill(nk, kd, d.layers) >= 0.7) return mmvid_gemm_bf16_dw_multi(d.M, nk, kd, d.layers, 1, stream);
+    if (mmvid_gemm_dw_multi_fill(nk, kd, d.layers) >= 0.7) return mmvid_gemm_bf16_dw_multi(d.M, nk, kd, d.layers, dw_accumulate, stream);
     for (int k = 0; k < nk; ++k)
         for (int i = d.layers - 1; i >= 0; --i)
             TRY(linear_dw(d.M, kd[k].N, kd[k].K, (const char*)kd[k].dY + (int64_t)i * kl.total, (const char*)kd[k].X + (int64_t)i * sl.total,
-                          kd[k].dW_list[i], nullptr, ws, stream));
+                          kd[k].dW_list[i], nullptr, ws, dw_accumulate, stream));
     return MMVID_OK;
 }
 
diff --git a/mmvid_amd/engine.py b/mmvid_amd/engine.py
--- a/mmvid_amd/engine.py
+++ b/mmvid_amd/engine.py
@@ -8,8 +8,46 @@
 ALIGN = 128
 
 
+ZERO_CHUNK = 16384
+
+
 def _round_up(x, m):
     return (x + m - 1) // m * m
+
+
+def flat_layout(numels):
+    offs, tot = [], 0
+    for n in numels:
+        offs.append(tot)
+        tot += _round_up(n, ALIGN)
+    return offs, tot
+
+
+def zero_ranges_table(segments, skip=(), chunk=ZERO_CHUNK):
+    rows, at = [], None
+    skip = sorted((int(a), int(b)) for a, b in skip if b > a)
+    for lo, hi in sorted((int(a), int(b)) for a, b in segments if b > a):
+        lo = lo if at is None else max(lo, at)
+        pieces, cur = [], lo
+        for a, b in skip:
+            if b <= cur or a >= hi:
+                continue
+            if a > cur:
+                pieces.append((cur, a))
+            cur = max(cur, b)
+        if cur < hi:
+            pieces.append((cur, hi))
+        for a, b in pieces:
+            for o in range(a, b, chunk):
+                rows.append((o, min(chunk, b - o)))
+        at = hi if at is None else max(at, hi)
+    return rows
+
+
+def first_write_plan(offsets, numels, total, first_write, lazy=None):
+    dense = [(0, total)] if lazy is None else [(0, lazy[0]), (lazy[1], total)]
+    fw = [(offsets[i], offsets[i] + numels[i]) for i in sorted(first_write)]
+    return zero_ranges_table(dense, fw), zero_ranges_table(fw)
 
 
 class WarmupLR:
@@ -32,7 +70,7 @@
 class FlatTrainer:
     def __init__(self, model, lr=1e-4, betas=(0.9, 0.999), eps=1e-8, weight_decay=0.0, max_grad_norm=1.0,
                  process_group=None, bucket_mb=64, order=None, lr_schedule=None, force_exchange=False, sparse_tables=True,
-                 lazy_rows=True, exchange=None):
+                 lazy_rows=True, exchange=None, first_write=True):
         self.model = model
         self.exchange = os.environ.get('MMVID_EXCHANGE', exchange or 'allreduce')
         assert self.exchange in ('allreduce', 'direct'), self.exchange
@@ -47,13 +85,10 @@
         self.names = [n for n, _ in params]
         self.params = [p for _, p in params]
         dev = self.params[0].device
-        offs, tot = [], 0
-        for p in self.params:
-            offs.append(tot)
-            tot += _round_up(p.numel(), ALIGN)
+        offs, tot = flat_layout([p.numel() for p in self.params])
         self.offsets, self.numel = offs, tot
         self.P = torch.zeros(tot, device=dev, dtype=torch.float32)
-        self.G = torch.zeros(tot, device=dev, dtype=torch.float32)
+        self._G = torch.zeros(tot, device=dev, dtype=torch.float32)
         self.M = torch.zeros(tot, device=dev, dtype=torch.float32)
         self.V = torch.zeros(tot, device=dev, dtype=torch.float32)
         self.S = torch.zeros(tot, device=dev, dtype=torch.bfloat16) if dev.type == 'cuda' else None
@@ -61,7 +96,7 @@
             n = p.numel()
             self.P[o:o + n].copy_(p.detach().reshape(-1))
             p.data = self.P[o:o + n].view(p.shape)
-            p.grad = self.G[o:o + n].view(p.shape)
+            p.grad = self._G[o:o + n].view(p.shape)
         if self.S is not None:
             ops.cast_bf16(self.P, self.S)
             self._attach_shadows()
@@ -86,6 +121,38 @@
         if tw is not None and hasattr(tw, 'on_layers_done') and self._layer_start and (self.world > 1 or self.force_exchange):
             tw.on_layers_done = self.layers_done
         self._init_lazy_rows(lazy_rows and os.environ.get('MMVID_LAZY_ROWS', '1') != '0')
+        self._init_first_write(first_write and os.environ.get('MMVID_DW_FIRST_WRITE', '1') != '0')
+
+    @property
+    def G(self):
+        self._settle_first_write()
+        return self._G
+
+    def _init_first_write(self, enabled):
+        self._fw = None
+        tw = getattr(self.model, 'transformer', None)
+        if not enabled or self.S is None or tw is None or not hasattr(tw, 'expect_first_write'):
+            return
+        if 'mmvid_zero_ranges' in _lib.load()._mmvid_missing or 'mmvid_tower_backward_ex' in _lib.load()._mmvid_missing:
+            return
+        at = {id(p): i for i, p in enumerate(self.params)}
+        idx = [at.get(id(p)) for p in tw.first_write_params()]
+        live = [i for i in idx if i is not None]
+        if not live:
+            return
+        z = self._lazy
+        lazy = None if z is None else (z['lo'], z['lo'] + z['rows'] * z['rowlen'])
+        clear, own = first_write_plan(self.offsets, [p.numel() for p in self.params], self.numel, live, lazy)
+        dev = self._G.device
+        table = lambda rows: torch.tensor(rows, dtype=torch.int64, device=dev).view(-1, 2)
+        self._fw = {'tower': tw, 'clear': table(clear), 'own': table(own),
+                    'ptrs': [None if i is None else self._G.data_ptr() + 4 * self.offsets[i] for i in idx]}
+
+    def _settle_first_write(self):
+        fw = getattr(self, '_fw', None)
+        if fw is not None and fw['tower'].first_write_pending():
+            fw['tower'].expect_first_write(None)
+            ops.zero_ranges(self._G, fw['own'])
 
     def _init_lazy_rows(self, enabled):
         self._lazy = None
@@ -152,9 +219,9 @@
             if p.data_ptr() != self.P.data_ptr() + 4 * o:
                 raise RuntimeError('a parameter no longer lives in FlatTrainer.P (moved by .to() / load_state_dict(assign=True)); '
                                    'rebuild the trainer after moving the model')
-            if p.grad is None or p.grad.data_ptr() != self.G.data_ptr() + 4 * o:
+            if p.grad is None or p.grad.data_ptr() != self._G.data_ptr() + 4 * o:
                 stray = p.grad
-                p.grad = self.G[o:o + p.numel()].view(p.shape)
+                p.grad = self._G[o:o + p.numel()].view(p.shape)
                 if stray is not None:
                     p.grad.add_(stray)
                     if self._lazy is not None and o == self._lazy['lo']:
@@ -230,14 +297,24 @@
             if pending or getattr(self.model, '_text_id_overflow', False):
                 z['all_dirty'] = True
         self._stepped_since_zero = False
-        if z is None or z['all_dirty']:
-            self.G.zero_()
+        fw = self._fw
+        if fw is not None:
+            ops.zero_ranges(self._G, fw['clear'])
+            if z is not None:
+                lo, hi = z['lo'], z['lo'] + z['rows'] * z['rowlen']
+                if z['all_dirty']:
+                    self._G[lo:hi].zero_()
+                elif z['dirty_n']:
+                    self._G[lo:hi].view(z['rows'], z['rowlen']).index_fill_(0, z['dirty'][:z['dirty_n']], 0.0)
+            fw['tower'].expect_first_write(fw['ptrs'])
+        elif z is None or z['all_dirty']:
+            self._G.zero_()
         else:
             lo, hi = z['lo'], z['lo'] + z['rows'] * z['rowlen']
-            self.G[:lo].zero_()
-            self.G[hi:].zero_()
+            self._G[:lo].zero_()
+            self._G[hi:].zero_()
             if z['dirty_n']:
-                self.G[lo:hi].view(z['rows'], z['rowlen']).index_fill_(0, z['dirty'][:z['dirty_n']], 0.0)
+                self._G[lo:hi].view(z['rows'], z['rowlen']).index_fill_(0, z['dirty'][:z['dirty_n']], 0.0)
         if z is not None:
             z['all_dirty'], z['dirty_n'] = False, 0
             if hasattr(self.model, 'table_grad_pending'):
@@ -282,14 +359,14 @@
 
     def _reduce_message(self, s, e):
         if self.exchange == 'allreduce' or self.world == 1 or (e - s) % self.world != 0:
-            self._works.append(dist.all_reduce(self.G[s:e], op=dist.ReduceOp.SUM, group=self.pg, async_op=True))
+            self._works.append(dist.all_reduce(self._G[s:e], op=dist.ReduceOp.SUM, group=self.pg, async_op=True))
             return
         n, w = e - s, self.world
         if self._direct_buf is None or self._direct_buf.numel() < n + n // w:
-            self._direct_buf = torch.empty(self.bucket_elems + self.bucket_elems // w + w, device=self.G.device, dtype=torch.float32)
+            self._direct_buf = torch.empty(self.bucket_elems + self.bucket_elems // w + w, device=self._G.device, dtype=torch.float32)
         recv = self._direct_buf[:n].view(w, n // w)
         shard = self._direct_buf[n:n + n // w]
-        msg = self.G[s:e]
+        msg = self._G[s:e]
         nccl = dist.get_backend(self.pg) == 'nccl'
         if nccl:
             dist.all_to_all_single(recv.view(-1), msg, group=self.pg)
@@ -370,11 +447,12 @@
 
     def after_failed_capture(self):
         if self._comm_stream is not None:
-            self._comm_stream = torch.cuda.Stream(device=self.G.device)
+            self._comm_stream = torch.cuda.Stream(device=self._G.device)
         self._works = []
         self._sent_from = self.numel
 
     def allreduce_grads(self):
+        self._settle_first_write()
         if self.world > 1 or self.force_exchange:
             self._send(0, self._sent_from)
             if self._comm_stream is not None:
@@ -390,6 +468,7 @@
         self._sent_from = self.numel
 
     def step(self):
+        self._settle_first_write()
         self._check_bindings()
         self.allreduce_grads()
         if self._lazy is not None:
@@ -409,8 +488,8 @@
                 ops.lr_schedule(self._step_dev, 1, sc.min_lr, sc.max_lr, sc.warmup, sc.every, self._lr_dev)
                 lr_dev = self._lr_dev
             ops.counter_add(self._step_dev, 1.0)
-        ops.grad_sqnorm(self.G, self._sq, partials=self._sq_partials, lazy=self._lazy_arg())
-        ops.adam_step(self.P, self.G, self.M, self.V, self.S, self.step_count, self.lr, self.betas, self.eps, self.wd,
+        ops.grad_sqnorm(self._G, self._sq, partials=self._sq_partials, lazy=self._lazy_arg())
+        ops.adam_step(self.P, self._G, self.M, self.V, self.S, self.step_count, self.lr, self.betas, self.eps, self.wd,
                       self.max_norm, self._sq, gscale, step_dev=self._step_dev, lr_dev=lr_dev, lazy=self._lazy_arg())
         tw = getattr(self.model, 'transformer', None)
         if tw is not None and hasattr(tw, 'mark_shadow_fresh') and getattr(self, '_tower_shadow_attached', False):
diff --git a/mmvid_amd/ops.py b/mmvid_amd/ops.py
--- a/mmvid_amd/ops.py
+++ b/mmvid_amd/ops.py
@@ -416,6 +416,12 @@
          _stream())
 
 
+def zero_ranges(g, table):
+    _chk(g, f32, 'g'), _chk(table, torch.int64, 'table')
+    assert table.dim() == 2 and table.shape[1] == 2
+    call('mmvid_zero_ranges', _p(g), g.numel(), _p(table), table.shape[0], _stream())
+
+
 def counter_add(counter, value=1.0):
     call('mmvid_counter_add', _p(counter), float(value), _stream())
 
```

New measurement: 214,000 (median of 6 runs). About the same (+1.0%).
